# mpkuse/solve_keyframe_pose_graph

Hardware: AMD Instinct MI355X
Metric: LM iters/sec + final chi2 vs Ceres, 100k-pose/300k-edge SE(3) graph (higher is better)
Workload: dtype f64

## Files before the change

### solve_keyframe_pose_graph_amd/csrc/pgo_handle.hpp

```cpp
#pragma once
#include <hip/hip_runtime.h>

#include <chrono>
#include <cstdlib>
#include <cstring>
#include <memory>
#include <string>
#include <thread>
#include <vector>

#include "pgo.h"
#include "pgo_internal.hpp"
#include "pgo_comm.hpp"
#include "pgo_mg_host.hpp"

#pragma GCC visibility push(hidden)
namespace pgo {

inline double now_s() { return std::chrono::duration<double>(std::chrono::steady_clock::now().time_since_epoch()).count(); }

inline bool debug_hooks_enabled() { static const bool on = []() { const char* e = std::getenv("PGO_ENABLE_DEBUG_HOOKS"); return e && e[0] == '1' && e[1] == 0; }(); return on; }
inline bool debug_poison() { static const bool on = []() { const char* e = std::getenv("PGO_DEBUG_POISON"); return debug_hooks_enabled() && e && e[0] == '1' && e[1] == 0; }(); return on; }
inline bool debug_break_coarse() { if (!debug_hooks_enabled()) return false; const char* e = std::getenv("PGO_DEBUG_BREAK_COARSE"); return e && e[0] == '1' && e[1] == 0; }

inline int debug_graph_after() {
    static const int v = []() {
        const char* e = std::getenv("PGO_DEBUG_GRAPH_AFTER");
        if (!debug_hooks_enabled() || !e) return 192;
        char* end = nullptr; const long n = std::strtol(e, &end, 10);
        return (end && *end == 0 && n >= 2 && n <= 1000000 && (n & 1) == 0) ? (int)n : 192;
    }();
    return v;
}

template <class T>
struct DBuf {
    T* p = nullptr;
    size_t cap = 0;
    DBuf() = default;
    DBuf(const DBuf&) = delete;
    DBuf& operator=(const DBuf&) = delete;
    ~DBuf() { if (p) (void)hipFree(p); }
    hipError_t ensure(size_t n) {
        if (n <= cap) return hipSuccess;
        if (p) { (void)hipFree(p); p = nullptr; cap = 0; }
        const size_t want = n + n / 8 + 64;
        hipError_t e = hipMalloc((void**)&p, want * sizeof(T));
        if (e == hipSuccess) cap = want;
        if (e == hipSuccess && debug_poison()) { e = hipMemset(p, 0xFF, want * sizeof(T)); if (e == hipSuccess) e = hipDeviceSynchronize(); }
        return e;
    }
};

struct EventPair {
    hipEvent_t e0 = nullptr, e1 = nullptr;
    hipError_t create() { hipError_t e = hipEventCreate(&e0); if (e == hipSuccess) e = hipEventCreate(&e1); return e; }
    ~EventPair() { if (e0) (void)hipEventDestroy(e0); if (e1) (void)hipEventDestroy(e1); }
};

struct HostClass {
    std::vector<int32_t> c1, c2, sw;
    std::vector<double> meas;
    int64_t size() const { return (int64_t)c1.size(); }
};

struct MgPrepared;
struct MgPreparedFree { void operator()(MgPrepared* Q) const; };
using MgImage = std::unique_ptr<MgPrepared, MgPreparedFree>;

struct LevelPlanDev { const int32_t* send_idx = nullptr; const int32_t* recv_idx = nullptr; const pgo_mg::ExchangePlan* plan = nullptr; };
struct SetupPlanDev { const int32_t* val_send = nullptr; const int32_t* val_dst = nullptr; const int32_t* val_sum_ptr = nullptr; const int32_t* val_sum_src = nullptr;
                      const int32_t* ps_send = nullptr; const int32_t* ps_recv = nullptr; const int32_t* rv_send = nullptr; const int32_t* rv_recv = nullptr; };
struct OwnRange { int64_t row0 = 0, row1 = 0, blk0 = 0, blk1 = 0, ps0 = 0, ps1 = 0, w0 = 0, w1 = 0, rT0 = 0, rT1 = 0; };

struct MgJob {
    enum Kind { none, fresh, regroup };
    Kind kind = none;
    std::thread thread;
    MgImage out;
    int rc = 0;
    MgImage old;
};

struct MgState {
    DBuf<double> f64; DBuf<int32_t> i32; DBuf<int64_t> i64;
    MgDev M{}; MgLevelDev levels[MG_MAX_LEVELS];
    bool fine = false; MgLevelDev fineF{}, fineT{};
    int fine_auto = -1;
    bool built = false, active = false;
    pgo_mg::BuildCache cache;
    std::vector<double> sw_built;
    int regroups = 0;
    uint64_t geometry_epoch = 0;
    MgJob job;
    std::vector<LevelPlanDev> lvl_plan;
    std::vector<pgo_mg::ExchangePlan> plans;
    std::vector<uint8_t> dist;
    pgo_mg::SetupPlans setup; int first_whole = 0;
    int32_t fw_row0 = 0, fw_row1 = 0; int64_t fw_blk0 = 0, fw_blk1 = 0;
    std::vector<SetupPlanDev> su_plan;
    std::vector<OwnRange> own;
    int levels_distributed = 0; int64_t rows_total = 0, rows_own = 0, blocks_total = 0, blocks_own = 0;
    bool fresh_pending() const { return job.kind == MgJob::fresh; }
};

struct CoarseState {
    DBuf<double> d_ccen, d_cd, d_cAc, d_crc, d_cscr;
    DBuf<float> d_cAcf;
    DBuf<int64_t> d_cblk_ptr, d_ccontrib;
    DBuf<int32_t> d_cblk_ab, d_cagg_free, d_cinfo;
    CoarseDev K{};
    bool built = false, active = false;
    int mode = 0;
    int retests = 0; bool skip_all = false; double drop_radius = 0.0;
    int backoff = 0, skip = 0;
    int keep_streak = 0;
    uint64_t geometry_epoch = 0;
};

struct OwnedStream {
    hipStream_t s = nullptr;
    OwnedStream() = default;
    OwnedStream(const OwnedStream&) = delete;
    OwnedStream& operator=(const OwnedStream&) = delete;
    ~OwnedStream() { if (s) (void)hipStreamDestroy(s); }
    operator hipStream_t() const { return s; }
};

struct PcgState {
    struct Poll { int32_t flags[4]; double scal[4]; };
    Poll* poll = nullptr; hipEvent_t poll_ev[2] = {nullptr, nullptr};
    struct CapturedChunk { hipGraphExec_t exec = nullptr; int len = 0; uint64_t epoch = 0; double scale = 0.0; bool sr = false; };
    CapturedChunk cg_chunk[3];
    hipGraphExec_t cg_graph = nullptr;
    uint64_t build_epoch = 1; bool cg_graph_failed = false;
    double cg_predicted = 0.0;
    double cg_prev_equiv = 0.0, cg_prev_radius = 0.0;
    int mg_switch_at = 400;
    int cg_extra = 0;
    bool mg_failed = false;
    bool mg_start_deferred = false;
    PcgState() = default;
    PcgState(const PcgState&) = delete;
    PcgState& operator=(const PcgState&) = delete;
    hipError_t create() {
        hipError_t e = hipHostMalloc((void**)&poll, 3 * sizeof(Poll), hipHostMallocDefault);
        if (e == hipSuccess) e = hipEventCreateWithFlags(&poll_ev[0], hipEventDisableTiming);
        if (e == hipSuccess) e = hipEventCreateWithFlags(&poll_ev[1], hipEventDisableTiming);
        if (e == hipSuccess) std::memset(poll, 0, 3 * sizeof(Poll));
        return e;
    }
    ~PcgState() {
        for (CapturedChunk& cc : cg_chunk) if (cc.exec) (void)hipGraphExecDestroy(cc.exec);
        if (poll) (void)hipHostFree(poll);
        for (hipEvent_t e : poll_ev) if (e) (void)hipEventDestroy(e);
    }
};

}
#pragma GCC visibility pop

using namespace pgo;

struct pgo_problem {
    pgo_options opt;
    int device = 0;
    std::string err;

    HostClass rel, swe;
    std::vector<PriorDev> priors;
    std::vector<int32_t> constant_nodes;
    bool graph_dirty = true, priors_dirty = true;

    int64_t N = 0, S = 0, N_global = 0;
    bool local_ids = false;
    std::vector<int32_t> l2g, g2l;
    std::vector<uint8_t> h_touched_any;
    std::vector<double> h_own;
    std::vector<double> h_init_q, h_init_t;
    std::vector<uint64_t> h_touch_mask;
    std::vector<int32_t> h_owner;
    pgo_mg::FinePlan fine_plan;
    DBuf<int32_t> d_l2g, d_fp_send, d_fp_shloc, d_fp_sumptr, d_fp_sumsrc;
    DBuf<double> d_own, d_xsend[2], d_xrecv, d_xscal;
    int64_t n_sh_mine = 0, n_sh_global = 0;
    int64_t st_exchanges = 0, st_allreduces = 0, st_pcg_iterations = 0; double st_bytes_neighbour = 0.0, st_bytes_allreduce = 0.0;
    DBuf<int32_t> d_rc1, d_rc2, d_sc1, d_sc2, d_sidx, d_bsr_col;
    DBuf<double> d_rmeas, d_smeas;
    DBuf<int4> d_rwin, d_swin;
    DBuf<PriorDev> d_prior;
    DBuf<int64_t> d_inc_rowptr, d_inc, d_bsr_rowptr;
    DBuf<uint8_t> d_node_free;
    DBuf<double> d_Jr, d_Js, d_Jp;
    DBuf<double> d_Hd_g;
    DBuf<double> d_Hoff, d_c, d_hss, d_gs;
    DBuf<double> d_scale_p, d_scale_s, d_diag_p, d_diag_s, d_a_inv;
    DBuf<double> d_val, d_Dtot_b;
    DBuf<float> d_Lf;
    DBuf<double> d_cgvec;
    DBuf<double> d_part;
    DBuf<double> d_cgpart;
    DBuf<int32_t> d_flags;
    DBuf<double> d_scal;
    DBuf<double> d_pose[2], d_swv[2], d_delta_s, d_io;
    DBuf<double> d_tmp;
    DBuf<double> d_vio;
    DBuf<int32_t> d_vio_idx; DBuf<double> d_vio_meas;
    CoarseState coarse;
    uint64_t lin_epoch = 0;
    MgState mg;
    uint64_t hoff_epoch = 0;
    int64_t n_vio = 0;
    DBuf<uint32_t> d_einc;
    DBuf<uint32_t> d_einc_slot;
    DBuf<ushort4> d_node_rng;
    DBuf<int64_t> d_tile_inc0;
    DBuf<int32_t> d_einc_other, d_tile_node0, d_tile_sw0, d_node_prior;
    DBuf<double2> d_rec;
    DBuf<double> d_lam;
    MfDev F{};
    bool built_mf = false;
    int64_t mf_pair_lanes = 0, mf_rel_side_lanes = 0, mf_sw_lanes = 0;
    int cur = 0;
    int64_t n_part = MAX_PARTIALS;
    std::vector<uint8_t> h_node_free, h_sw_used;
    int64_t nnzb = 0;

    GraphDev G{};
    LinDev L{};
    ScaleDev Sc{};
    CgDev C{};

    bool in_solve = false, scale_ready = false, terminated = false, have_prev_step = false;
    double radius = 0, decrease_factor = 2, x_cost = 0, x_norm = 0, gmax = 0;
    bool reuse_diagonal = false;
    int iteration = 0, invalid = 0;
    double t_begin = 0, t_device0 = 0;
    pgo_summary sum;

    std::unique_ptr<pgo_comm::Comm> comm;
    int rank() const { return comm ? comm->rank() : 0; }
    int world() const { return comm ? comm->world() : 1; }

    OwnedStream st;
    PcgState pcg;
    double last_rho = 1.0;
};


#define HIPCHK(p, expr) PGO_HIPCHK((p)->err, expr)

#pragma GCC visibility push(hidden)
namespace pgo {

int allreduce(pgo_problem* p, double* buf, size_t n, int op );
int host_allreduce(pgo_problem* p, std::vector<double>& v, int op);
int exchange_rows(pgo_problem* p, double* a1, int k1, double* a2, int k2, const int32_t* stop = nullptr);
int exchange_level(pgo_problem* p, int l, double* v1, double* v2, const int32_t* stop, const double* dinv);
int exchange_blocks_copy(pgo_problem* p, const pgo_mg::ExchangePlan& X, const int32_t* send_idx, const int32_t* recv_idx, double* arr, int K);
int exchange_blocks_sum(pgo_problem* p, const pgo_mg::BlockPlan& B, const SetupPlanDev& D, double* arr);
int ensure_exchange_buffers(pgo_problem* p);

int build_two_level_aggregates(pgo_problem* p);
void two_level_solve_begin(pgo_problem* p);
void two_level_solve_end(pgo_problem* p);
int build_system(pgo_problem* p, bool* ok);
bool single_reduction(const pgo_problem* p);
struct PcgForm {
    enum Rec { ranks, sr, sr_coarse, classic_mf, classic_csr, classic_coarse };
    enum Post { none, mg_cycle, mg_restricted, two_level };
    Rec rec; Post post;
    int fused_parts;
    bool single_red() const { return rec == sr || rec == sr_coarse; }
    bool fused_coarse() const { return rec == sr_coarse || rec == classic_coarse; }
    bool mg() const { return post == mg_cycle || post == mg_restricted; }
    int precond() const { return mg() ? 2 : (fused_coarse() || post == two_level) ? 1 : 0; }
};
PcgForm choose_form(const pgo_problem* p, bool this_rank_only = false);
void pcg_matvec(pgo_problem* p, const PcgForm& f, int k, double tol2);
int pcg_update(pgo_problem* p, const PcgForm& f, int k);
int pcg_precond(pgo_problem* p, const PcgForm& f, int k);
int pcg_iteration(pgo_problem* p, const PcgForm& f, int k, double tol2);
int pcg_start(pgo_problem* p, const PcgForm& f, bool warm, double tol2);
struct CgResult { int iterations; bool breakdown; double rel_residual; bool converged; };
struct PcgPhase { double tol; int resume = -1; bool warm = false; bool switch_now = false; int max_iterations = 0; };
int run_pcg(pgo_problem* p, CgResult* res, const PcgPhase& ph);
int finish_system(pgo_problem* p, CgResult* cg, bool evaluated, int* precond_used);

bool wants_multigrid(const pgo_problem* p);
void mg_drop_pending(pgo_problem* p);
bool mg_start_fresh(pgo_problem* p, const double* sw_now);
int build_multigrid(pgo_problem* p, const double* sw_now);
int mg_fresh_install(pgo_problem* p);
int regroup_if_moved(pgo_problem* p, const double* sv, bool in_solve);
int regroup_start(pgo_problem* p);
int build_mg(pgo_problem* p);
int mg_operators(pgo_problem* p, int32_t* fail, bool hoff_valid, bool kernels_only, double t_build0);
bool mg_exchange_at(pgo_problem* p, int point, int lv, int* plan, double** v1, double** v2, const double** dinv);
int mg_apply_ranks(pgo_problem* p, bool inside_iteration);
double mg_cs(const pgo_problem* p);
double mg_scale(const pgo_problem* p);
const MgLevelDev* mg_fine_view(const pgo_problem* p);

}
#pragma GCC visibility pop
```

### solve_keyframe_pose_graph_amd/csrc/pgo_internal.hpp

```cpp
#pragma once
#include <hip/hip_runtime.h>
#include <stdint.h>

#include "pgo_device_math.hpp"

#define PGO_HIPCHK(err, expr)                                                                      \
    do {                                                                                           \
        hipError_t e__ = (expr);                                                                   \
        if (e__ != hipSuccess) {                                                                   \
            (err) = std::string(#expr) + ": " + hipGetErrorString(e__);                            \
            return e__ == hipErrorOutOfMemory ? PGO_ERR_OUT_OF_MEMORY : PGO_ERR_HIP;               \
        }                                                                                          \
    } while (0)

namespace pgo {

constexpr int TILE = 64;
constexpr int REL_DOUBLES = 78;
constexpr int SW_DOUBLES = 86;
constexpr int K1_WAVES = 4;
constexpr int WIN_MAX = 72;
constexpr int WIN_STRIDE = 80;
constexpr int MAX_PARTIALS = 1024;
constexpr int CG_MAX_GRID = 1024;
constexpr int RZ_STRIDE = CG_MAX_GRID + MAX_PARTIALS;
constexpr int PQ_SLOTS = CG_MAX_GRID;
constexpr int PRIOR_DOUBLES = 42;
constexpr int MF_BLOCK = 256;
constexpr int MF_MAX_NODES = 42;
constexpr int MF_SLOTS = 384;
constexpr int MF_MAX_GRID = 1024;
constexpr int MF_PLANES = 8;

struct PriorDev {
    double Rf[9];
    double tf[3];
    double qf[4];
    double w;
    int32_t node;
    int32_t pad_;
};

struct EdgeClassDev {
    const int32_t* c1;
    const int32_t* c2;
    const double* meas;
    const int32_t* swidx;
    const int4* win;
    double* J;
    int64_t E, Epad;
    int32_t tiles;
};

struct GraphDev {
    int64_t N, S;
    EdgeClassDev rel, sw;
    const PriorDev* prior; int32_t n_prior; double* Jp;
    const int64_t* inc_rowptr; const int64_t* inc;
    const uint8_t* node_free;
    const double* own;
    const int64_t* bsr_rowptr; const int32_t* bsr_col; int64_t nnzb;
};

struct MfDev {
    const uint32_t* einc;
    const int32_t* einc_other;
    const uint32_t* einc_slot;
    const int64_t* tile_inc0;
    const int32_t* tile_sw0;
    const int32_t* tile_node0;
    const ushort4* node_rng;
    const int32_t* node_prior;
    double2* rec;
    double* lam;
    int64_t ninc, ninc_pad;
    int32_t tiles;
};

struct LinDev {
    double* Hd; double* g; double* Hoff; double* c; double* hss; double* gs;
};

struct ScaleDev {
    double* scale_p;
    double* scale_s;
    double* diag_p;
    double* diag_s;
    double* a_inv;
};

struct CoarseDev {
    int32_t n_agg, nc;
    int32_t m;
    int32_t n_blk;
    double* cen;
    double* d;
    double* Ac;
    double* rc;
    double* yc;
    const int64_t* blk_ptr;
    const int32_t* blk_ab;
    const int64_t* contrib;
    const int32_t* agg_free;
    float* Acf;
};

constexpr int MG_MAX_LEVELS = 12;
constexpr int MG_TILE_ROWS = 32;
struct MgLevelDev {
    int32_t n, n_next, tiles, n_ps;
    int64_t nnzb;
    const int64_t* rowptr; const int32_t* col; double* val;
    const int64_t* g_ptr; const int64_t* g_ent;
    double* Dinv;
    double* pos; double* d;
    const int32_t* parent; const int32_t* agg_ptr; const int4* tile_info; const int2* tile_rows;
    double* r; double* x; double* xt; double* xf;
    float* valf;
    int32_t smoothed, n_w;
    int32_t seg_shift, pad3_;
    const int32_t* ps_rowptr; const int32_t* ps_col; const int32_t* w_rowptr; const int32_t* w_col; const int64_t* psT_ptr; const int64_t* psT_ent;
    double* ps_val; double* w_val;
    double* t; double* u; double* y; const double* zero;
    double* dlump;
    const int32_t* row_of; const int32_t* tr_of;
    const int32_t* ps_row; const int32_t* w_row;
    float* rt_valf; float* r_valf;
    const int2* rt_rows; const int2* rT_rows; const int32_t* rT_col; const int32_t* rT_of_w; const int32_t* ps_of_w;
    int32_t rT_tiles, rT_seg_shift;
    int32_t tile0, tiles_own, rT_row0, rT_row1;
    int32_t su_row0, su_row1, su_ps0, su_ps1, su_w0, su_w1, n_su_prod, pad4_;
    int64_t su_blk0, su_blk1;
    const int32_t* su_prod;
};
struct MgDev {
    int32_t n_levels;
    int32_t n1;
    const int32_t* agg0;
    const int32_t* mem0_ptr; const int32_t* mem0;
    double* d0;
    const int4* blk_tab;
    const double* inv_cnt;
    int32_t a0, a1;
    const int32_t* g0_slots; int32_t n_g0, pad_;
};
constexpr int MG_BLOCK0 = 64;

struct CgDev {
    double* val; float* Lf; double* Dtot; double* b;
    double* x; double* r; double* r2; double* z; double* p; double* p2; double* q;
    double* part_pq;
    double* part_rz;
    int32_t extra_rz;
    int32_t pad_;
    double* scal;
    int32_t* flags;
};

void launch_k1(const GraphDev& G, const double* pose8, const double* sw, bool want_jacobian, double* partials , int* n_partials, hipStream_t st);
void launch_prior(const GraphDev& G, const double* pose8, bool want_jacobian, double* partial_cost , hipStream_t st);
void launch_k2(const GraphDev& G, const LinDev& L, bool want_offdiag, hipStream_t st, const MfDev* F = nullptr );
void launch_scale_init(const GraphDev& G, const LinDev& L, const ScaleDev& Sc, int jacobi_scaling, hipStream_t st);
void launch_lm_diag(const GraphDev& G, const LinDev& L, const ScaleDev& Sc, double min_diag, double max_diag, hipStream_t st);
void launch_build_rows(const GraphDev& G, const LinDev& L, const ScaleDev& Sc, const CgDev& C, double radius, int add_lambda, double* lam_out , hipStream_t st);
void launch_mf_compact(const GraphDev& G, const MfDev& F, const double* pose8, const double* sw, hipStream_t st);
void launch_mf_spmv(const GraphDev& G, const MfDev& F, const ScaleDev& Sc, const CgDev& C, int k, double tol2, hipStream_t st);
void launch_mf_apply(const GraphDev& G, const MfDev& F, const ScaleDev& Sc, const CgDev& C, const double* x, double* y, hipStream_t st);
void launch_mf_apply_dot(const GraphDev& G, const MfDev& F, const ScaleDev& Sc, const CgDev& C, const double* x, double* y, hipStream_t st);
void launch_invert_rows(const GraphDev& G, const CgDev& C, int32_t* fail_flag, hipStream_t st);
void launch_cg_init(const GraphDev& G, const CgDev& C, int warm , double tol2, hipStream_t st);
int launch_cg_init_vectors(const GraphDev& G, const CgDev& C, int warm, hipStream_t st);
void launch_cg_init_scalars(const CgDev& C, int nparts, int nparts_bb, double tol2, hipStream_t st);
void launch_cg_set_tolerance(const CgDev& C, double tol2, hipStream_t st);
void launch_cg_poll(const CgDev& C, int32_t* host_flags, double* host_scal, hipStream_t st);
void launch_cg_spmv(const GraphDev& G, const CgDev& C, int k, double tol2, hipStream_t st);
void launch_cg_update(const GraphDev& G, const CgDev& C, int k, int n_pq_partials, hipStream_t st);
void launch_mf_apply_dot_live(const GraphDev& G, const MfDev& F, const ScaleDev& Sc, const CgDev& C, hipStream_t st);
void launch_cg_update_sr(const GraphDev& G, const CgDev& C, int k, int first, int n_pq_partials, hipStream_t st);
void launch_mf_apply_dot_live_coarse(const GraphDev& G, const MfDev& F, const ScaleDev& Sc, const CgDev& C, const CoarseDev& K, int pending, hipStream_t st);
void launch_cg_update_restrict_sr(const GraphDev& G, const CgDev& C, const CoarseDev& K, int k, int first, int pending, int n_pq_partials, hipStream_t st);
int cg_grid_size(const GraphDev& G);
int mf_grid_size(const MfDev& F);
void launch_apply_operator(const GraphDev& G, const CgDev& C, const double* x, double* y, hipStream_t st);
void launch_model_change(const GraphDev& G, const LinDev& L, const ScaleDev& Sc, const double* delta_p, double* delta_s, double* partials, int* n_partials, hipStream_t st);
void launch_plus(const GraphDev& G, const double* pose8, const double* sw, const double* delta_p, const double* delta_s,
                 double* pose8_out, double* sw_out, double* part_step2, double* part_sw_step2, int* n_partials, hipStream_t st);
void launch_state_norms(const GraphDev& G, const LinDev& L, const double* pose8, const double* sw,
                        double* part_xnorm2, double* part_sw_xnorm2, double* part_gmax, int* n_partials, hipStream_t st);
void launch_reduce(const double* partials, int n, int op , double* out, hipStream_t st);
void launch_manifold_plus(int64_t n, const double* quat, const double* t, const double* delta, double* quat_out, double* t_out, hipStream_t st);
void launch_pack_pose(const double* quat, const double* t, double* pose8, int64_t N, hipStream_t st);
void launch_unpack_pose(const double* pose8, double* quat, double* t, int64_t N, hipStream_t st);
void launch_unpack_k1(const GraphDev& G, int kind, int64_t first, int64_t count, double* r, double* J1, double* J2, double* Js, hipStream_t st);
void launch_gather_rows(double* buf, const double* a1, int k1, const double* a2, int k2, int64_t n, const int32_t* idx, const int32_t* stop, hipStream_t st);
void launch_scatter_rows(const double* buf, double* a1, int k1, double* a2, int k2, int64_t n, const int32_t* idx, const int32_t* stop, hipStream_t st);
void launch_scatter_rows_dinv(const double* buf, double* r, double* x, const double* Dinv, int64_t n, const int32_t* idx, const int32_t* stop, hipStream_t st);
void launch_sum_rows(const double* buf, double* a1, int k1, double* a2, int k2, int64_t n_sh, const int32_t* sh_loc, const int32_t* sum_ptr, const int32_t* sum_src, const int32_t* stop, hipStream_t st);
struct LocalPeers { const double* src[16]; int64_t off[16]; int64_t cnt[16]; int n; };
void launch_local_reduce(double* out, const LocalPeers& P, int64_t n, int op, hipStream_t st);
void launch_local_copy(double* recv, const LocalPeers& P, hipStream_t st);
void launch_coarse_geometry(const GraphDev& G, const CoarseDev& K, const double* pose8, hipStream_t st);
void launch_coarse_assemble(const GraphDev& G, const LinDev& L, const ScaleDev& Sc, const CgDev& C, const CoarseDev& K, hipStream_t st);
void launch_coarse_symmetrize(const CoarseDev& K, hipStream_t st);
void launch_coarse_shift(const CoarseDev& K, double eps, hipStream_t st);
void launch_coarse_invert(const CoarseDev& K, double* scratch , int32_t* fail, hipStream_t st);
void launch_coarse_negate(const CoarseDev& K, hipStream_t st);
void launch_coarse_apply(const GraphDev& G, const CgDev& C, const CoarseDev& K, const double* r, double* z, double* part_rz, bool inside_iteration, hipStream_t st);
int coarse_group_keyframes(const CoarseDev& K);
int coarse_update_grid(const GraphDev& G, const CoarseDev& K);
int coarse_solve_grid(const CoarseDev& K);
void launch_mf_spmv_coarse(const GraphDev& G, const MfDev& F, const ScaleDev& Sc, const CgDev& C, const CoarseDev& K, int k, double tol2, int nparts, int pending, hipStream_t st);
void launch_cg_update_restrict(const GraphDev& G, const CgDev& C, const CoarseDev& K, int k, int n_pq_partials, hipStream_t st);
void launch_coarse_solve_dot(const CoarseDev& K, const int32_t* stop, double* part, hipStream_t st);
void launch_cgcg_dots(const GraphDev& G, const CgDev& C, hipStream_t st);
void launch_cg_reduce2_live(const CgDev& C, const double* pa, int na, const double* pb, int nb, double* out, hipStream_t st);
void launch_cgcg_update(const GraphDev& G, const CgDev& C, int k, int first, hipStream_t st, const double* xq = nullptr, const int32_t* sh_of = nullptr, const double* two = nullptr);
void launch_cgcg_scalars_init(const CgDev& C, const double* bb_src, double tol2, hipStream_t st);
void launch_scatter_owned_pose(const double* quat, const double* t, int64_t n, const int32_t* l2g, const double* own, double* gquat, double* gt, hipStream_t st);
void launch_vio_odometry(int64_t n, const int32_t* c1, const int32_t* c2, const double* vio, int yaw_weight, double* meas8, hipStream_t st);
void launch_vio_initial_guess(int64_t u_begin, int64_t count, const double* left, const int32_t* left_of_node, const double* vio, double* quat, double* t, hipStream_t st);

void launch_mg_geometry(const GraphDev& G, const MgDev& M, const MgLevelDev* levels, const double* pose8, hipStream_t st);
void launch_mg_geometry0_sum(const GraphDev& G, const MgDev& M, const MgLevelDev* levels, const double* pose8, hipStream_t st);
void launch_mg_geometry_finish(const GraphDev& G, const MgDev& M, const MgLevelDev* levels, const double* pose8, hipStream_t st);
void launch_mg_assemble(const GraphDev& G, const LinDev& L, const ScaleDev& Sc, const CgDev& C, const MgDev& M, const MgLevelDev* levels, const CoarseDev& K, double omega, int32_t* fail, hipStream_t st, double prolong_scale = 0.0, bool hoff_valid = false);
void launch_mg_galerkin0(const GraphDev& G, const LinDev& L, const ScaleDev& Sc, const CgDev& C, const MgDev& M, const MgLevelDev* levels, hipStream_t st, bool hoff_valid = false);
void launch_k2_offdiag(const GraphDev& G, const LinDev& L, hipStream_t st);
void launch_mg_assemble_fine(const GraphDev& G, const LinDev& L, const ScaleDev& Sc, const CgDev& C, const MgLevelDev& F, const MgLevelDev& T, const MgLevelDev& L1, double omega, int32_t* fail, hipStream_t st,
                             double prolong_scale, bool hoff_valid, const double* pose8 = nullptr );
void launch_mg_assemble_rest(const MgDev& M, const MgLevelDev* levels, const CoarseDev& K, double omega, int32_t* fail, hipStream_t st, double prolong_scale = 0.0 ,
                             int first_level = 0 );
void launch_mg_level_inverses(const MgLevelDev& A, double omega, int32_t* fail, hipStream_t st);
void launch_mg_level_power(const MgLevelDev& A, double omega, hipStream_t st);
void launch_mg_power_init(const MgLevelDev& A, hipStream_t st);
void launch_mg_power_step(const MgLevelDev& A, const double* v, double* w, double omega, hipStream_t st);
void launch_mg_power_sums(const MgLevelDev& A, const double* a, const double* b, const int32_t* fail, double* out3, hipStream_t st);
void launch_mg_power_finish(const double* in3, int32_t* fail, double* lam, hipStream_t st);
void launch_mg_level_rescale(const MgLevelDev& A, const double* lam, double omega, hipStream_t st);
void launch_mg_transition_ps(const MgLevelDev& A, double prolong_scale, hipStream_t st);
void launch_mg_transition_w(const MgLevelDev& A, hipStream_t st);
void launch_mg_transition_product(const MgLevelDev& A, const MgLevelDev& B, hipStream_t st);
void launch_mg_level_galerkin(const MgLevelDev& A, const MgLevelDev& B, hipStream_t st);
void launch_mg_dense_top(const MgDev& M, const MgLevelDev* levels, const CoarseDev& K, hipStream_t st);
struct MgExchangeHook { void* ctx; int (*fn)(void* ctx, int point, int level); };
void launch_mg_apply(const GraphDev& G, const CgDev& C, const MgDev& M, const MgLevelDev* levels, const CoarseDev& K, const double* r, double* z, double* part_rz, double scale, bool inside_iteration, hipStream_t st,
                     bool restricted = false , double prolong_scale = 0.0 ,
                     const MgLevelDev* fine = nullptr ,
                     const MgExchangeHook* hook = nullptr , int* hook_rc = nullptr);
void launch_cg_update_mg(const GraphDev& G, const CgDev& C, const MgDev& M, const MgLevelDev* levels, const CoarseDev& K, int k, int n_pq_partials, hipStream_t st);
void launch_cg_update_mg_sr(const GraphDev& G, const CgDev& C, const MgDev& M, const MgLevelDev* levels, const CoarseDev& K, int k, int first, int n_pq_partials, hipStream_t st);

double k1_algorithmic_bytes(const GraphDev& G, bool want_jacobian);

}
```

### solve_keyframe_pose_graph_amd/csrc/pgo_mg_kernels.hpp

```cpp

__device__ __forceinline__ int bsr_idx(int row, int col) { return (row >> 1) * 12 + col * 2 + (row & 1); }

__device__ __forceinline__ void mg_row_accumulate(int64_t b, int64_t e, const int32_t* __restrict__ col, const double* __restrict__ val,
                                                  const double* __restrict__ x, int c, double* acc) {
    int64_t k = b;
    for (; k + 4 <= e; k += 4) spmv_chunk<4, false>(col + k, val + (size_t)k * 36, c, x, nullptr, 0.0, acc);
    if (k + 2 <= e) { spmv_chunk<2, false>(col + k, val + (size_t)k * 36, c, x, nullptr, 0.0, acc); k += 2; }
    if (k < e) spmv_chunk<1, false>(col + k, val + (size_t)k * 36, c, x, nullptr, 0.0, acc);
}

template <int U>
__device__ __forceinline__ void mg_chunk_f32(const int32_t* __restrict__ colp, const float* __restrict__ valp, int c, const double* __restrict__ x, double* acc) {
    int32_t col[U];
    float2 v[U][3];
    double xx[U];
#pragma unroll
    for (int u = 0; u < U; ++u) col[u] = colp[u];
#pragma unroll
    for (int u = 0; u < U; ++u) {
        const float2* vp = reinterpret_cast<const float2*>(valp + (size_t)u * 36) + c;
        v[u][0] = vp[0]; v[u][1] = vp[6]; v[u][2] = vp[12];
    }
#pragma unroll
    for (int u = 0; u < U; ++u) xx[u] = x[(size_t)col[u] * 6 + c];
// ... 186 lines not shown
#pragma unroll
            for (int u = 0; u < CH; ++u) if (u < n) acc += coarse_entry(Hs[wv][u], ds[wv][u], ds[wv][u] + 3, r, c);
        }
        __builtin_amdgcn_wave_barrier();
    }
    if (own) A.val[(size_t)slot * 36 + bsr_idx(r, c)] = acc;
}
__global__ __launch_bounds__(256) void mg_galerkin_kernel(MgLevelDev A, MgLevelDev B) {
    constexpr int CH = 8;
    __shared__ double Hs[4][CH][36];
    __shared__ double ds[4][CH][6];
    const int wv = wave_in_block(), lane = threadIdx.x & 63;
    const int64_t slot = wave_in_grid() + B.su_blk0;
    if (slot >= B.su_blk1) return;
    const int r = lane / 6, c = lane - r * 6;
    const bool own = lane < 36;
    const int srow = 2 * (lane / 12) + (lane & 1), scol = (lane % 12) >> 1;
    const int du = lane / 6, dm = lane - du * 6;
    double acc = 0.0;
    const int64_t kend = B.g_ptr[slot + 1];
    for (int64_t k0 = B.g_ptr[slot]; k0 < kend; k0 += CH) {
        const int n = (int)(kend - k0 < CH ? kend - k0 : CH);
        if (du < n) {
            const int64_t e = B.g_ent[k0 + du];
            const int64_t node = dm < 3 ? (e >> 32) : (int64_t)A.col[e & 0xffffffffll];
            ds[wv][du][dm] = A.d[(size_t)node * 3 + (dm < 3 ? dm : dm - 3)];
        }
        double h[CH];
#pragma unroll
        for (int u = 0; u < CH; ++u) {
            const int64_t fs = B.g_ent[k0 + u < kend ? k0 + u : kend - 1] & 0xffffffffll;
            h[u] = own ? A.val[(size_t)fs * 36 + lane] : 0.0;
        }
        if (own) {
#pragma unroll
            for (int u = 0; u < CH; ++u) Hs[wv][u][srow * 6 + scol] = h[u];
        }
        __builtin_amdgcn_wave_barrier();
        if (own) {
#pragma unroll
            for (int u = 0; u < CH; ++u) if (u < n) acc += coarse_entry(Hs[wv][u], ds[wv][u], ds[wv][u] + 3, r, c);
        }
        __builtin_amdgcn_wave_barrier();
    }
    if (own) B.val[(size_t)slot * 36 + bsr_idx(r, c)] = acc;
}
__global__ __launch_bounds__(256) void mg_dinv_kernel(MgLevelDev A, double omega, int32_t* __restrict__ fail, int skip_orphans ,
                                                      const double* __restrict__ diag = nullptr) {
    const int i = blockIdx.x * blockDim.x + threadIdx.x + A.su_row0;
    if (i >= A.su_row1) return;
    if (skip_orphans && A.parent[i] < 0) { double* out = A.Dinv + (size_t)i * 36; for (int e = 0; e < 36; ++e) out[e] = 0.0; return; }
    const double* v = diag ? diag + (size_t)i * 36 : A.val + (size_t)A.rowptr[i] * 36;
    double Lm[36];
    bool ok = true;
    for (int attempt = 0; attempt < 2; ++attempt) {
    ok = true;
#pragma unroll
    for (int j = 0; j < 6; ++j) {
        double d = v[bsr_idx(j, j)];
#pragma unroll
        for (int k = 0; k < 6; ++k) if (k < j) d -= Lm[j * 6 + k] * Lm[j * 6 + k];
        ok = ok && (d > 0.0);
        d = sqrt(d);
        Lm[j * 6 + j] = 1.0 / d;
#pragma unroll
        for (int r = 0; r < 6; ++r) if (r > j) {
            double s = v[bsr_idx(r, j)];
#pragma unroll
            for (int k = 0; k < 6; ++k) if (k < j) s -= Lm[r * 6 + k] * Lm[j * 6 + k];
            Lm[r * 6 + j] = s * Lm[j * 6 + j];
        }
    }
    if (ok || !diag || attempt == 1) break;
    v = A.val + (size_t)A.rowptr[i] * 36;
    }
    if (!ok) atomicOr(fail, 1);
    double* out = A.Dinv + (size_t)i * 36;
#pragma unroll
    for (int e = 0; e < 6; ++e) {
        double y[6], z[6];
#pragma unroll
        for (int r = 0; r < 6; ++r) {
            double s = r == e ? 1.0 : 0.0;
#pragma unroll
            for (int k = 0; k < 6; ++k) if (k < r) s -= Lm[r * 6 + k] * y[k];
            y[r] = s * Lm[r * 6 + r];
        }
#pragma unroll
        for (int r = 5; r >= 0; --r) {
            double s = y[r];
#pragma unroll
            for (int k = 0; k < 6; ++k) if (k > r) s -= Lm[k * 6 + r] * z[k];
            z[r] = s * Lm[r * 6 + r];
        }
#pragma unroll
        for (int r = 0; r < 6; ++r) out[r * 6 + e] = omega * z[r];
    }
}
__global__ __launch_bounds__(256) void mg_dense_scatter_kernel(MgLevelDev A, CoarseDev K) {
    const int64_t t = (int64_t)blockIdx.x * blockDim.x + threadIdx.x;
    if (t >= (int64_t)A.n * 36) return;
    const int i = (int)(t / 36), l = (int)(t - (int64_t)i * 36);
    const int row = 2 * (l / 12) + (l & 1), col = (l % 12) >> 1;
    for (int64_t k = A.rowptr[i]; k < A.rowptr[i + 1]; ++k)
        K.Ac[(size_t)(i * 6 + row) * K.nc + (size_t)A.col[k] * 6 + col] = A.val[(size_t)k * 36 + l];
}
__device__ __forceinline__ double mg_pblock(const double* __restrict__ d, int r, int c) {
    if (r < 3 || c >= 3) return r == c ? 1.0 : 0.0;
    const int a = r - 3;
    if (a == c) return 0.0;
    const int o = 3 - a - c;
    const double sgn = ((a + 1) % 3 == c) ? 1.0 : -1.0;
    return sgn * 2.0 * d[o];
}
template <bool FILT>
__global__ __launch_bounds__(256) void mg_ps_kernel(MgLevelDev A, double cs) {
    __shared__ double acc_s[4][36];
    const int wv = wave_in_block(), lane = threadIdx.x & 63;
    const int64_t slot = wave_in_grid() + A.su_ps0;
    if (slot >= A.su_ps1) return;
    const bool own = lane < 36;
    const int r = own ? lane / 6 : 0, c = own ? lane % 6 : 0;
    const int i = A.ps_row[slot], a = A.ps_col[slot];
    double acc = 0.0;
    for (int64_t k = A.rowptr[i]; k < A.rowptr[i + 1]; ++k) {
        const int j = A.col[k];
        if (A.parent[j] != a) continue;
        if (FILT && (A.g_ent[k] & 7) >= 3) continue;
        if (own) {
            const double* dj = A.d + (size_t)j * 3;
            const double* blk = (FILT && k == A.rowptr[i]) ? A.dlump + (size_t)i * 36 : A.val + (size_t)k * 36;
#pragma unroll
            for (int m = 0; m < 6; ++m) acc += blk[bsr_idx(r, m)] * mg_pblock(dj, m, c);
        }
    }
    if (own) acc_s[wv][lane] = acc;
    __builtin_amdgcn_wave_barrier();
    if (own) {
        double v = A.parent[i] == a ? mg_pblock(A.d + (size_t)i * 3, r, c) : 0.0;
        const double* Dk = A.Dinv + (size_t)i * 36 + r * 6;
#pragma unroll
        for (int m = 0; m < 6; ++m) v -= cs * Dk[m] * acc_s[wv][m * 6 + c];
        A.ps_val[(size_t)slot * 36 + lane] = v;
    }
}
constexpr int MG_SETUP_CHUNK = 8;
__global__ __launch_bounds__(256) void mg_w_kernel(MgLevelDev A) {
    __shared__ double pb[4][MG_SETUP_CHUNK][36], ab[4][MG_SETUP_CHUNK][36];
    const int wv = wave_in_block(), lane = threadIdx.x & 63;
    const int64_t slot = wave_in_grid() + A.su_w0;
    if (slot >= A.su_w1) return;
    const bool own = lane < 36;
    const int r = own ? lane / 6 : 0, c = own ? lane % 6 : 0;
    const int i = A.w_row[slot], b = A.w_col[slot];
    double acc = 0.0;
    const int64_t kend = A.rowptr[i + 1];
    for (int64_t k0 = A.rowptr[i]; k0 < kend; k0 += MG_SETUP_CHUNK) {
        const int n = (int)(kend - k0 < MG_SETUP_CHUNK ? kend - k0 : MG_SETUP_CHUNK);
        int j[MG_SETUP_CHUNK], p0[MG_SETUP_CHUNK], p1[MG_SETUP_CHUNK], ps[MG_SETUP_CHUNK];
#pragma unroll
        for (int u = 0; u < MG_SETUP_CHUNK; ++u) j[u] = u < n ? A.col[k0 + u] : 0;
#pragma unroll
        for (int u = 0; u < MG_SETUP_CHUNK; ++u) { p0[u] = u < n ? A.ps_rowptr[j[u]] : 0; p1[u] = u < n ? A.ps_rowptr[j[u] + 1] : 0; }
        int cand[MG_SETUP_CHUNK];
#pragma unroll
        for (int u = 0; u < MG_SETUP_CHUNK; ++u) cand[u] = (p0[u] + lane < p1[u]) ? A.ps_col[p0[u] + lane] : -1;
#pragma unroll
        for (int u = 0; u < MG_SETUP_CHUNK; ++u) {
            unsigned long long hit = __ballot(cand[u] == b);
            ps[u] = hit ? p0[u] + __ffsll((long long)hit) - 1 : -1;
            for (int base = p0[u] + 64; ps[u] < 0 && base < p1[u]; base += 64) {
                hit = __ballot(base + lane < p1[u] && A.ps_col[base + lane] == b);
                if (hit) ps[u] = base + __ffsll((long long)hit) - 1;
            }
        }
#pragma unroll
        for (int u = 0; u < MG_SETUP_CHUNK; ++u) if (ps[u] >= 0 && own) pb[wv][u][lane] = A.ps_val[(size_t)ps[u] * 36 + lane];
#pragma unroll
        for (int u = 0; u < MG_SETUP_CHUNK; ++u) if (ps[u] >= 0 && own) ab[wv][u][lane] = A.val[(size_t)(k0 + u) * 36 + lane];
        __builtin_amdgcn_wave_barrier();
#pragma unroll
        for (int u = 0; u < MG_SETUP_CHUNK; ++u) {
            if (ps[u] >= 0 && own) {
#pragma unroll
                for (int m = 0; m < 6; ++m) acc += ab[wv][u][bsr_idx(r, m)] * pb[wv][u][m * 6 + c];
            }
        }
        __builtin_amdgcn_wave_barrier();
    }
    if (own) A.w_val[(size_t)slot * 36 + lane] = acc;
}
__global__ __launch_bounds__(256) void mg_rt_kernel(MgLevelDev A) {
    const int lane = threadIdx.x & 63;
    const int64_t k = wave_in_grid() + A.su_w0;
    if (k >= A.su_w1 || lane >= 36) return;
    const int r = lane / 6, c = lane % 6;
    const int i = A.w_row[k];
    const int32_t ps = A.ps_of_w[k];
    const int32_t tr = A.rT_of_w[k];
    double v = ps >= 0 ? A.ps_val[(size_t)ps * 36 + lane] : 0.0;
    const double* Dk = A.Dinv + (size_t)i * 36 + r * 6;
    const double* W = A.w_val + (size_t)k * 36;
#pragma unroll
    for (int m = 0; m < 6; ++m) v -= Dk[m] * W[m * 6 + c];
    const float f = (float)v;
    A.rt_valf[(size_t)k * 36 + bsr_idx(r, c)] = f;
    A.r_valf[(size_t)tr * 36 + bsr_idx(c, r)] = f;
}
__global__ __launch_bounds__(256) void mg_psTw_kernel(MgLevelDev A, MgLevelDev B) {
    __shared__ double pa[4][MG_SETUP_CHUNK][36], wb[4][MG_SETUP_CHUNK][36];
    const int wv = wave_in_block(), lane = threadIdx.x & 63;
    int64_t slot = wave_in_grid();
    if (slot >= (A.su_prod ? (int64_t)A.n_su_prod : B.nnzb)) return;
    if (A.su_prod) slot = A.su_prod[slot];
    const bool own = lane < 36;
    const int r = own ? lane / 6 : 0, c = own ? lane % 6 : 0;
    const int a = B.row_of[slot], b = B.col[slot];
    double acc = 0.0;
    const int64_t eend = A.psT_ptr[a + 1];
    for (int64_t e0 = A.psT_ptr[a]; e0 < eend; e0 += MG_SETUP_CHUNK) {
        const int n = (int)(eend - e0 < MG_SETUP_CHUNK ? eend - e0 : MG_SETUP_CHUNK);
        int64_t ent[MG_SETUP_CHUNK];
        int w0[MG_SETUP_CHUNK], w1[MG_SETUP_CHUNK], ws[MG_SETUP_CHUNK], cand[MG_SETUP_CHUNK];
#pragma unroll
        for (int u = 0; u < MG_SETUP_CHUNK; ++u) ent[u] = u < n ? A.psT_ent[e0 + u] : 0;
#pragma unroll
        for (int u = 0; u < MG_SETUP_CHUNK; ++u) { const int i = (int)(ent[u] >> 32); const bool in = u < n && i >= A.su_row0 && i < A.su_row1; w0[u] = in ? A.w_rowptr[i] : 0; w1[u] = in ? A.w_rowptr[i + 1] : 0; }
#pragma unroll
        for (int u = 0; u < MG_SETUP_CHUNK; ++u) cand[u] = (w0[u] + lane < w1[u]) ? A.w_col[w0[u] + lane] : -1;
#pragma unroll
        for (int u = 0; u < MG_SETUP_CHUNK; ++u) {
            unsigned long long hit = __ballot(cand[u] == b);
            ws[u] = hit ? w0[u] + __ffsll((long long)hit) - 1 : -1;
            for (int base = w0[u] + 64; ws[u] < 0 && base < w1[u]; base += 64) {
                hit = __ballot(base + lane < w1[u] && A.w_col[base + lane] == b);
                if (hit) ws[u] = base + __ffsll((long long)hit) - 1;
            }
        }
#pragma unroll
        for (int u = 0; u < MG_SETUP_CHUNK; ++u)
            if (ws[u] >= 0 && own) { pa[wv][u][lane] = A.ps_val[(size_t)(ent[u] & 0xffffffffll) * 36 + lane]; wb[wv][u][lane] = A.w_val[(size_t)ws[u] * 36 + lane]; }
        __builtin_amdgcn_wave_barrier();
#pragma unroll
        for (int u = 0; u < MG_SETUP_CHUNK; ++u) {
            if (ws[u] >= 0 && own) {
#pragma unroll
                for (int m = 0; m < 6; ++m) acc += pa[wv][u][m * 6 + r] * wb[wv][u][m * 6 + c];
            }
        }
        __builtin_amdgcn_wave_barrier();
    }
    if (own) B.val[(size_t)slot * 36 + bsr_idx(r, c)] = acc;
}
__device__ __forceinline__ void mg_smooth_step_tile(const MgLevelDev& A, int tile, const double* __restrict__ in_r, const double* __restrict__ in_x, double* __restrict__ out_w,
                                                    const double* __restrict__ add1, const double* __restrict__ add2, double* __restrict__ out, double cs, const int32_t* __restrict__ stop,
                                                    double* xch , double* tb ) {
    const int stopped = stop ? *stop : 0;
    const int q6 = threadIdx.x / 6, c = threadIdx.x % 6;
    const int li = q6 & ((MG_TILE_ROWS >> A.seg_shift) - 1), sg = q6 >> (5 - A.seg_shift);
    const int4 ti = A.tile_info[tile];
    const int2 rb = A.tile_rows[tile * MG_TILE_ROWS + li];
    if (stopped) return;
    const int i0 = ti.z, i1 = ti.w;
    const int row = i0 + li;
    const bool rowlive = row < i1;
    const bool live = rowlive && sg == 0;
    double rv = 0.0, av = 0.0;
    double Dk[6] = {0.0, 0.0, 0.0, 0.0, 0.0, 0.0};
    if (live) {
        if (in_r) rv = in_r[(size_t)row * 6 + c];
        if (add1) av += add1[(size_t)row * 6 + c];
        if (add2) av += add2[(size_t)row * 6 + c];
        const double2* Dp = reinterpret_cast<const double2*>(A.Dinv + (size_t)row * 36 + c * 6);
        const double2 u0 = Dp[0], u1 = Dp[1], u2 = Dp[2];
        Dk[0] = u0.x; Dk[1] = u0.y; Dk[2] = u1.x; Dk[3] = u1.y; Dk[4] = u2.x; Dk[5] = u2.y;
    }
    double acc[6] = {0.0, 0.0, 0.0, 0.0, 0.0, 0.0};
    MG_ROW_PRODUCT(tile, in_x);
    double* mine = xch + (size_t)threadIdx.x * 7;
#pragma unroll
    for (int q = 0; q < 6; ++q) mine[q] = acc[q];
    __syncthreads();
    double w = 0.0;
    if (live) {
        w = rv - mg_gather_row(xch, li, c, A.seg_shift);
        tb[threadIdx.x] = w;
        if (out_w) out_w[(size_t)row * 6 + c] = w;
    }
    __syncthreads();
    if (live) {
        const double* ta = tb + (threadIdx.x - c);
        double x = 0.0;
#pragma unroll
        for (int j = 0; j < 6; ++j) x += Dk[j] * ta[j];
        out[(size_t)row * 6 + c] = av + cs * x;
    }
}
__global__ __launch_bounds__(CG_BLOCK) void mg_smooth_step_kernel(MgLevelDev A, const double* __restrict__ in_r, const double* __restrict__ in_x, double* __restrict__ out_w,
                                                                   const double* __restrict__ add1, const double* __restrict__ add2, double* __restrict__ out, double cs, const int32_t* __restrict__ stop) {
    __shared__ double xch[CG_BLOCK * 7];
    __shared__ double tb[CG_BLOCK];
    mg_smooth_step_tile(A, (int)blockIdx.x + A.tile0, in_r, in_x, out_w, add1, add2, out, cs, stop, xch, tb);
}
__global__ __launch_bounds__(CG_BLOCK) void mg_sdown_kernel(MgLevelDev A, double* __restrict__ r_next, double* __restrict__ x_next, const double* __restrict__ Dinv_next, const int32_t* __restrict__ stop) {
    __shared__ double xch[CG_BLOCK * 7];
    __shared__ double tb[CG_BLOCK];
    if ((int)blockIdx.x < A.tiles_own) { mg_smooth_step_tile(A, (int)blockIdx.x + A.tile0, A.r, A.x, nullptr, A.x, nullptr, A.y, 1.0, stop, xch, tb); return; }
    const int stopped = stop ? *stop : 0;
    const int tile = (int)blockIdx.x - A.tiles_own;
    const int ss = A.rT_seg_shift, rpt = MG_TILE_ROWS >> ss;
    const int q6 = threadIdx.x / 6, c = threadIdx.x % 6;
    const int li = q6 & (rpt - 1), sg = q6 >> (5 - ss);
    const int2 rb = A.rT_rows[tile * MG_TILE_ROWS + li];
    const int row = A.rT_row0 + tile * rpt + li;
    const bool live = row < A.rT_row1 && sg == 0;
    double Dk[6] = {0.0, 0.0, 0.0, 0.0, 0.0, 0.0};
    if (live && x_next) {
        const double2* Dp = reinterpret_cast<const double2*>(Dinv_next + (size_t)row * 36 + c * 6);
        const double2 u0 = Dp[0], u1 = Dp[1], u2 = Dp[2];
        Dk[0] = u0.x; Dk[1] = u0.y; Dk[2] = u1.x; Dk[3] = u1.y; Dk[4] = u2.x; Dk[5] = u2.y;
    }
    if (stopped) return;
    double acc[6] = {0.0, 0.0, 0.0, 0.0, 0.0, 0.0};
    if (row < A.rT_row1) { int kb, ke; mg_split_row(rb, sg, ss, kb, ke); mg_row_accumulate_f32(kb, ke, A.rT_col, A.r_valf, A.r, c, acc); }
    double* mine = xch + (size_t)threadIdx.x * 7;
#pragma unroll
    for (int q = 0; q < 6; ++q) mine[q] = acc[q];
    __syncthreads();
    double sum = 0.0;
    if (live) { sum = mg_gather_row(xch, li, c, ss); r_next[(size_t)row * 6 + c] = sum; }
    if (!x_next) return;
    tb[threadIdx.x] = sum;
    __syncthreads();
    if (live) {
        const double* ra = tb + (threadIdx.x - c);
        double x = 0.0;
#pragma unroll
        for (int j = 0; j < 6; ++j) x += Dk[j] * ra[j];
        x_next[(size_t)row * 6 + c] = x;
    }
}

template <bool HOFF>
__global__ __launch_bounds__(256) void mg_fine_blocks_kernel(GraphDev G, LinDev L, ScaleDev Sc, CgDev C, MgLevelDev F) {
    const int lane = threadIdx.x & 63;
    const int64_t k = wave_in_grid();
    if (k >= F.nnzb) return;
    const int r = lane / 6, c = lane - r * 6;
    const bool own = lane < 36;
    const double h = fine_block_value<HOFF>(G, L, Sc, C, F.g_ent[k], lane, r, c, own);
    if (own) F.val[(size_t)k * 36 + bsr_idx(r, c)] = h;
}
__global__ __launch_bounds__(256) void mg_fine_lump_kernel(MgLevelDev F, const double* __restrict__ pose8) {
    __shared__ double cs_[4][36];
    const int wv = wave_in_block(), lane = threadIdx.x & 63;
    const int64_t i = wave_in_grid();
    if (i >= F.n) return;
    const bool own = lane < 36;
    const int r = own ? lane / 6 : 0, c = own ? lane % 6 : 0;
    const int64_t k0 = F.rowptr[i], k1 = F.rowptr[i + 1];
    double acc = 0.0;
    if (F.parent[i] >= 0) {
        const double* ti = pose8 + (size_t)i * 8 + 4;
        for (int64_t k = k0 + 1; k < k1; ++k) {
            if ((F.g_ent[k] & 7) < 3) continue;
            const int j = F.col[k];
            if (F.parent[j] < 0 || j == (int)i) continue;
            if (own) {
                const double* tj = pose8 + (size_t)j * 8 + 4;
                const double d[3] = {tj[0] - ti[0], tj[1] - ti[1], tj[2] - ti[2]};
#pragma unroll
                for (int m = 0; m < 6; ++m) acc += F.val[(size_t)k * 36 + bsr_idx(r, m)] * mg_pblock(d, m, c);
            }
        }
    }
    if (own) cs_[wv][lane] = acc;
    __builtin_amdgcn_wave_barrier();
    if (own) F.dlump[(size_t)i * 36 + bsr_idx(r, c)] = F.val[(size_t)k0 * 36 + bsr_idx(r, c)] + 0.5 * (cs_[wv][r * 6 + c] + cs_[wv][c * 6 + r]);
}
__global__ __launch_bounds__(256) void mg_ps_f32_kernel(MgLevelDev T) {
    const int lane = threadIdx.x & 63;
    const int64_t k = wave_in_grid();
    if (k >= T.n_ps || lane >= 36) return;
    const int r = lane / 6, c = lane % 6;
    const float f = (float)T.ps_val[(size_t)k * 36 + lane];
    T.rt_valf[(size_t)k * 36 + bsr_idx(r, c)] = f;
    T.r_valf[(size_t)T.rT_of_w[k] * 36 + bsr_idx(c, r)] = f;
}
__global__ __launch_bounds__(CG_BLOCK) void mg_prolong0s_kernel(GraphDev G, MgLevelDev T, const double* __restrict__ x1, const double* __restrict__ rv, double* __restrict__ zv,
                                                                 double* __restrict__ part_rz, double scale, const int32_t* __restrict__ stop) {
    __shared__ double red[CG_BLOCK / 64];
    if (stop && *stop) return;
    const int64_t pairs = G.N * 3;
    double acc = 0.0;
    for (int64_t i = (int64_t)blockIdx.x * CG_BLOCK + threadIdx.x; i < pairs; i += (int64_t)gridDim.x * CG_BLOCK) {
        const int64_t n = i / 3;
        const int j = (int)(i - n * 3);
        const int k0 = T.ps_rowptr[n], k1 = T.ps_rowptr[n + 1];
        if (k1 <= k0) continue;
        double a0 = 0.0, a1 = 0.0;
        for (int k = k0; k < k1; ++k) {
            const float4* vp = reinterpret_cast<const float4*>(T.rt_valf + (size_t)k * 36 + j * 12);
            const float4 v0 = vp[0], v1 = vp[1], v2 = vp[2];
            const double2* xp = reinterpret_cast<const double2*>(x1 + (size_t)T.ps_col[k] * 6);
            const double2 xa = xp[0], xb = xp[1], xc = xp[2];
            a0 += (double)v0.x * xa.x + (double)v0.z * xa.y + (double)v1.x * xb.x + (double)v1.z * xb.y + (double)v2.x * xc.x + (double)v2.z * xc.y;
            a1 += (double)v0.y * xa.x + (double)v0.w * xa.y + (double)v1.y * xb.x + (double)v1.w * xb.y + (double)v2.y * xc.x + (double)v2.w * xc.y;
        }
        a0 *= scale; a1 *= scale;
        double2* zp = reinterpret_cast<double2*>(zv) + i;
        const double2 r = reinterpret_cast<const double2*>(rv)[i];
        double2 z = *zp;
        z.x += a0; z.y += a1;
        *zp = z;
        acc += r.x * a0 + r.y * a1;
    }
    const double s = block_sum(acc, red);
    if (threadIdx.x == 0) part_rz[blockIdx.x] += s;
}

__global__ void mg_power_init_kernel(double* __restrict__ v, double* __restrict__ w, int n6, int lo6, int hi6) {
    const int i = blockIdx.x * blockDim.x + threadIdx.x;
    if (i >= n6) return;
    v[i] = (i >= lo6 && i < hi6) ? 1.0 + 0.5 * sin(0.7 * (double)i) : 0.0;
    w[i] = 0.0;
}
__global__ __launch_bounds__(1024) void mg_power_ratio_kernel(const double* __restrict__ a, const double* __restrict__ b, int lo6, int hi6, double* __restrict__ lam) {
    __shared__ double red[32];
    double sa = 0.0, sb = 0.0;
    for (int i = lo6 + threadIdx.x; i < hi6; i += blockDim.x) { sa += a[i] * a[i]; sb += b[i] * b[i]; }
    sa = wave_sum(sa); sb = wave_sum(sb);
    if ((threadIdx.x & 63) == 0) { red[threadIdx.x >> 6] = sa; red[16 + (threadIdx.x >> 6)] = sb; }
    __syncthreads();
    if (threadIdx.x == 0) {
        double ta = 0.0, tb = 0.0;
        for (int k = 0; k < 16; ++k) { ta += red[k]; tb += red[16 + k]; }
        *lam = ta > 0.0 ? sqrt(tb / ta) : 0.0;
    }
}
__global__ __launch_bounds__(256) void mg_rescale_dinv_kernel(MgLevelDev A, const double* __restrict__ lam, double omega, double limit, double target) {
    const double wl = omega * lam[0];
    if (!(wl > limit)) return;
    const double f = target / wl;
    const int64_t i = (int64_t)blockIdx.x * blockDim.x + threadIdx.x + (int64_t)A.su_row0 * 36;
    if (i < (int64_t)A.su_row1 * 36) A.Dinv[i] *= f;
}
void launch_mg_level_power(const MgLevelDev& A, double omega, hipStream_t st) {
    const int n6 = A.n * 6;
    double* v = A.x; double* w = A.xt; double* lam = A.xf;
    MgLevelDev S = A;
    const bool part = A.su_row0 != 0 || A.su_row1 != A.n;
    if (!part) { S.tile0 = 0; S.tiles_own = A.tiles; }
    hipLaunchKernelGGL(mg_power_init_kernel, dim3((unsigned)((n6 + 255) / 256)), dim3(256), 0, st, v, w, n6, A.su_row0 * 6, A.su_row1 * 6);
    for (int it = 0; it < 8; ++it) {
        if (S.tiles_own > 0) hipLaunchKernelGGL(mg_smooth_step_kernel, dim3((unsigned)S.tiles_own), dim3(CG_BLOCK), 0, st, S, (const double*)nullptr, (const double*)v, (double*)nullptr, (const double*)nullptr, (const double*)nullptr, w, -1.0 / omega, (const int32_t*)nullptr);
        double* tmp = v; v = w; w = tmp;
    }
    hipLaunchKernelGGL(mg_power_ratio_kernel, dim3(1), dim3(1024), 0, st, (const double*)w, (const double*)v, A.su_row0 * 6, A.su_row1 * 6, lam);
}
void launch_mg_level_rescale(const MgLevelDev& A, const double* lam, double omega, hipStream_t st) {
    const int64_t cnt = (int64_t)(A.su_row1 - A.su_row0) * 36;
    if (cnt > 0) hipLaunchKernelGGL(mg_rescale_dinv_kernel, dim3((unsigned)((cnt + 255) / 256)), dim3(256), 0, st, A, lam, omega, 1.75, 1.5);
}
void launch_mg_level_inverses(const MgLevelDev& A, double omega, int32_t* fail, hipStream_t st) {
    const int rows = A.su_row1 - A.su_row0;
    const int64_t blocks = A.su_blk1 - A.su_blk0;
    if (rows > 0) hipLaunchKernelGGL(mg_dinv_kernel, dim3((unsigned)((rows + 255) / 256)), dim3(256), 0, st, A, omega, fail, 0, (const double*)nullptr);
    if (blocks > 0) hipLaunchKernelGGL(mg_val_f32_kernel, dim3((unsigned)((blocks + 3) / 4)), dim3(256), 0, st, A);
}
void launch_mg_transition_ps(const MgLevelDev& A, double prolong_scale, hipStream_t st) {
    const int cnt = A.su_ps1 - A.su_ps0;
    if (cnt > 0) hipLaunchKernelGGL(mg_ps_kernel<false>, dim3((unsigned)((cnt + 3) / 4)), dim3(256), 0, st, A, prolong_scale);
}
void launch_mg_transition_w(const MgLevelDev& A, hipStream_t st) {
    const int cnt = A.su_w1 - A.su_w0;
    if (cnt <= 0) return;
    hipLaunchKernelGGL(mg_w_kernel, dim3((unsigned)((cnt + 3) / 4)), dim3(256), 0, st, A);
    if (A.rt_valf) hipLaunchKernelGGL(mg_rt_kernel, dim3((unsigned)((cnt + 3) / 4)), dim3(256), 0, st, A);
}
void launch_mg_transition_product(const MgLevelDev& A, const MgLevelDev& B, hipStream_t st) {
    const int64_t cnt = A.su_prod ? (int64_t)A.n_su_prod : B.nnzb;
    if (cnt > 0) hipLaunchKernelGGL(mg_psTw_kernel, dim3((unsigned)((cnt + 3) / 4)), dim3(256), 0, st, A, B);
}
void launch_mg_level_galerkin(const MgLevelDev& A, const MgLevelDev& B, hipStream_t st) {
    const int64_t cnt = B.su_blk1 - B.su_blk0;
    if (cnt > 0) hipLaunchKernelGGL(mg_galerkin_kernel, dim3((unsigned)((cnt + 3) / 4)), dim3(256), 0, st, A, B);
}
void launch_mg_power_init(const MgLevelDev& A, hipStream_t st) {
    const int n6 = A.n * 6;
    hipLaunchKernelGGL(mg_power_init_kernel, dim3((unsigned)((n6 + 255) / 256)), dim3(256), 0, st, A.x, A.xt, n6, A.su_row0 * 6, A.su_row1 * 6);
}
void launch_mg_power_step(const MgLevelDev& A, const double* v, double* w, double omega, hipStream_t st) {
    if (A.tiles_own > 0) hipLaunchKernelGGL(mg_smooth_step_kernel, dim3((unsigned)A.tiles_own), dim3(CG_BLOCK), 0, st, A, (const double*)nullptr, v, (double*)nullptr, (const double*)nullptr, (const double*)nullptr, w, -1.0 / omega, (const int32_t*)nullptr);
}
__global__ __launch_bounds__(1024) void mg_power_sums_kernel(const double* __restrict__ a, const double* __restrict__ b, int lo6, int hi6, const int32_t* __restrict__ fail, double* __restrict__ out3) {
    __shared__ double red[32];
    double sa = 0.0, sb = 0.0;
    for (int i = lo6 + threadIdx.x; i < hi6; i += blockDim.x) { sa += a[i] * a[i]; sb += b[i] * b[i]; }
    sa = wave_sum(sa); sb = wave_sum(sb);
    if ((threadIdx.x & 63) == 0) { red[threadIdx.x >> 6] = sa; red[16 + (threadIdx.x >> 6)] = sb; }
    __syncthreads();
    if (threadIdx.x == 0) {
        double ta = 0.0, tb = 0.0;
        for (int k = 0; k < 16; ++k) { ta += red[k]; tb += red[16 + k]; }
        out3[0] = ta; out3[1] = tb; out3[2] = *fail != 0 ? 1.0 : 0.0;
    }
}
__global__ void mg_power_finish_kernel(const double* __restrict__ in3, int32_t* __restrict__ fail, double* __restrict__ lam) { if (in3[2] != 0.0) *fail = 1; *lam = in3[0] > 0.0 ? sqrt(in3[1] / in3[0]) : 0.0; }
void launch_mg_power_sums(const MgLevelDev& A, const double* a, const double* b, const int32_t* fail, double* out3, hipStream_t st) {
    hipLaunchKernelGGL(mg_power_sums_kernel, dim3(1), dim3(1024), 0, st, a, b, A.su_row0 * 6, A.su_row1 * 6, fail, out3);
}
void launch_mg_power_finish(const double* in3, int32_t* fail, double* lam, hipStream_t st) { hipLaunchKernelGGL(mg_power_finish_kernel, dim3(1), dim3(1), 0, st, in3, fail, lam); }

void launch_mg_galerkin0(const GraphDev& G, const LinDev& L, const ScaleDev& Sc, const CgDev& C, const MgDev& M, const MgLevelDev* levels, hipStream_t st, bool hoff_valid) {
    const int64_t cnt = M.g0_slots ? (int64_t)M.n_g0 : levels[0].nnzb;
    if (cnt <= 0) return;
    if (hoff_valid) hipLaunchKernelGGL((mg_galerkin0_kernel<true>), dim3((unsigned)((cnt + 3) / 4)), dim3(256), 0, st, G, L, Sc, C, M, levels[0]);
    else hipLaunchKernelGGL((mg_galerkin0_kernel<false>), dim3((unsigned)((cnt + 3) / 4)), dim3(256), 0, st, G, L, Sc, C, M, levels[0]);
}
void launch_mg_assemble(const GraphDev& G, const LinDev& L, const ScaleDev& Sc, const CgDev& C, const MgDev& M, const MgLevelDev* levels, const CoarseDev& K, double omega, int32_t* fail, hipStream_t st, double prolong_scale, bool hoff_valid) {
    launch_mg_galerkin0(G, L, Sc, C, M, levels, st, hoff_valid);
    launch_mg_assemble_rest(M, levels, K, omega, fail, st, prolong_scale);
}
void launch_mg_dense_top(const MgDev& M, const MgLevelDev* levels, const CoarseDev& K, hipStream_t st) {
    const MgLevelDev& T = levels[M.n_levels - 1];
    (void)hipMemsetAsync(K.Ac, 0, (size_t)K.nc * K.nc * sizeof(double), st);
    if (K.nc > 6 * K.n_agg) hipLaunchKernelGGL(coarse_pad_identity_kernel, dim3((unsigned)((K.nc - 6 * K.n_agg + 63) / 64)), dim3(64), 0, st, K);
    hipLaunchKernelGGL(mg_dense_scatter_kernel, dim3((unsigned)(((int64_t)T.n * 36 + 255) / 256)), dim3(256), 0, st, T, K);
}
void launch_mg_assemble_rest(const MgDev& M, const MgLevelDev* levels, const CoarseDev& K, double omega, int32_t* fail, hipStream_t st, double prolong_scale, int first_level) {
    for (int l = first_level; l < M.n_levels; ++l) {
        if (l > first_level) {
            const MgLevelDev& A = levels[l - 1];
            if (A.smoothed) { launch_mg_transition_ps(A, prolong_scale, st); launch_mg_transition_w(A, st); launch_mg_transition_product(A, levels[l], st); }
            else launch_mg_level_galerkin(A, levels[l], st);
        }
        if (l + 1 < M.n_levels) {
            launch_mg_level_inverses(levels[l], omega, fail, st);
            launch_mg_level_power(levels[l], omega, st);
            launch_mg_level_rescale(levels[l], levels[l].xf, omega, st);
        }
    }
    launch_mg_dense_top(M, levels, K, st);
}
void launch_mg_assemble_fine(const GraphDev& G, const LinDev& L, const ScaleDev& Sc, const CgDev& C, const MgLevelDev& F, const MgLevelDev& T, const MgLevelDev& L1, double omega, int32_t* fail, hipStream_t st,
                             double prolong_scale, bool hoff_valid, const double* pose8) {
    if (hoff_valid) hipLaunchKernelGGL((mg_fine_blocks_kernel<true>), dim3((unsigned)((F.nnzb + 3) / 4)), dim3(256), 0, st, G, L, Sc, C, F);
    else hipLaunchKernelGGL((mg_fine_blocks_kernel<false>), dim3((unsigned)((F.nnzb + 3) / 4)), dim3(256), 0, st, G, L, Sc, C, F);
    if (F.dlump && pose8) {
        hipLaunchKernelGGL(mg_fine_lump_kernel, dim3((unsigned)((F.n + 3) / 4)), dim3(256), 0, st, F, pose8);
        hipLaunchKernelGGL(mg_dinv_kernel, dim3((unsigned)((F.n + 255) / 256)), dim3(256), 0, st, F, omega, fail, 1, (const double*)F.dlump);
        hipLaunchKernelGGL(mg_ps_kernel<true>, dim3((unsigned)((F.n_ps + 3) / 4)), dim3(256), 0, st, F, prolong_scale);
    } else {
        hipLaunchKernelGGL(mg_dinv_kernel, dim3((unsigned)((F.n + 255) / 256)), dim3(256), 0, st, F, omega, fail, 1, (const double*)nullptr);
        hipLaunchKernelGGL(mg_ps_kernel<false>, dim3((unsigned)((F.n_ps + 3) / 4)), dim3(256), 0, st, F, prolong_scale);
    }
    hipLaunchKernelGGL(mg_w_kernel, dim3((unsigned)((F.n_w + 3) / 4)), dim3(256), 0, st, F);
    hipLaunchKernelGGL(mg_psTw_kernel, dim3((unsigned)((L1.nnzb + 3) / 4)), dim3(256), 0, st, F, L1);
    hipLaunchKernelGGL(mg_ps_f32_kernel, dim3((unsigned)((T.n_ps + 3) / 4)), dim3(256), 0, st, T);
}

__global__ __launch_bounds__(CG_BLOCK) void mg_restrict0_kernel(MgDev M, const double* __restrict__ rv, double* __restrict__ r_out, double* __restrict__ x_out,
                                                                 const double* __restrict__ Dinv, const int32_t* __restrict__ stop, const double* __restrict__ own = nullptr ) {
    __shared__ double rb[CG_BLOCK];
    const int stopped = stop ? *stop : 0;
    const int a = M.a0 + blockIdx.x * MG_TILE_ROWS + threadIdx.x / 6, k = threadIdx.x % 6;
    const bool live = a < M.a1;
    int m0 = 0, m1 = 0;
    if (live) { m0 = M.mem0_ptr[a]; m1 = M.mem0_ptr[a + 1]; }
    if (stopped) return;
    double s = 0.0;
    if (live) {
        if (own) for (int m = m0; m < m1; ++m) { const int i = M.mem0[m]; s += own[i] * mg_restrict_comp(rv + (size_t)i * 6, M.d0 + (size_t)i * 3, k); }
        else for (int m = m0; m < m1; ++m) { const int i = M.mem0[m]; s += mg_restrict_comp(rv + (size_t)i * 6, M.d0 + (size_t)i * 3, k); }
        r_out[(size_t)a * 6 + k] = s;
    }
    if (!x_out) return;
    rb[threadIdx.x] = s;
    __syncthreads();
    if (live) {
        const double* Dk = Dinv + (size_t)a * 36 + k * 6;
        const double* ra = rb + (threadIdx.x - k);
        double x = 0.0;
#pragma unroll
        for (int j = 0; j < 6; ++j) x += Dk[j] * ra[j];
        x_out[(size_t)a * 6 + k] = x;
    }
}
#ifdef PGO_MG_TIMELINE
__device__ unsigned long long pgo_mg_tl[4 * 1024 * 8];
#define MG_TL(slot) do { __builtin_amdgcn_s_waitcnt(0); if (threadIdx.x == 0 && A.pad3_ < 4 && blockIdx.x < 1024) pgo_mg_tl[((size_t)A.pad3_ * 1024 + blockIdx.x) * 8 + (slot)] = wall_clock64(); } while (0)
extern "C" int pgo_debug_mg_timeline(unsigned long long* out, int n) {
    return (int)hipMemcpyFromSymbol(out, HIP_SYMBOL(pgo_mg_tl), (size_t)n * sizeof(unsigned long long), 0, hipMemcpyDeviceToHost);
}
#else
#define MG_TL(slot) do {} while (0)
#endif
__global__ __launch_bounds__(CG_BLOCK) void mg_down_kernel(MgLevelDev A, double* __restrict__ r_next, double* __restrict__ x_next, const double* __restrict__ Dinv_next,
                                                            const int32_t* __restrict__ stop) {
    __shared__ double xch[CG_BLOCK * 7];
    __shared__ double tb[CG_BLOCK];
    __shared__ double cb[CG_BLOCK];
    MG_TL(0);
    const int stopped = stop ? *stop : 0;
    const int q6 = threadIdx.x / 6, c = threadIdx.x % 6;
    const int li = q6 & ((MG_TILE_ROWS >> A.seg_shift) - 1), sg = q6 >> (5 - A.seg_shift);
    const int tile_d = (int)blockIdx.x + A.tile0;
    const int4 ti = A.tile_info[tile_d];
    const int2 rb = A.tile_rows[tile_d * MG_TILE_ROWS + li];
    MG_TL(1);
    if (stopped) return;
    const int a0 = ti.x, na = ti.y - ti.x, i0 = ti.z, i1 = ti.w;
    const int row = i0 + li;
    const bool rowlive = row < i1;
    const bool live = rowlive && sg == 0;
    const bool lagg = threadIdx.x < na * 6;
    const int a = a0 + li;
    double rv = 0.0, d0 = 0.0, d1 = 0.0, d2 = 0.0;
    int m0 = 0, m1 = 0;
    double Dk[6] = {0.0, 0.0, 0.0, 0.0, 0.0, 0.0};
    if (live) { rv = A.r[(size_t)row * 6 + c]; d0 = A.d[(size_t)row * 3]; d1 = A.d[(size_t)row * 3 + 1]; d2 = A.d[(size_t)row * 3 + 2]; }
    if (lagg) {
        m0 = A.agg_ptr[a]; m1 = A.agg_ptr[a + 1];
        if (x_next) {
            const double2* Dp = reinterpret_cast<const double2*>(Dinv_next + (size_t)a * 36 + c * 6);
            const double2 u0 = Dp[0], u1 = Dp[1], u2 = Dp[2];
            Dk[0] = u0.x; Dk[1] = u0.y; Dk[2] = u1.x; Dk[3] = u1.y; Dk[4] = u2.x; Dk[5] = u2.y;
        }
    }
    MG_TL(2);
    double acc[6] = {0.0, 0.0, 0.0, 0.0, 0.0, 0.0};
    MG_ROW_PRODUCT(blockIdx.x, A.x);
    MG_TL(3);
    double* mine = xch + (size_t)threadIdx.x * 7;
#pragma unroll
    for (int q = 0; q < 6; ++q) mine[q] = acc[q];
    __syncthreads();
    if (live) tb[threadIdx.x] = rv - mg_gather_row(xch, li, c, A.seg_shift);
    __syncthreads();
    MG_TL(4);
    if (live) {
        const double d[3] = {d0, d1, d2};
        cb[threadIdx.x] = mg_restrict_comp(tb + (size_t)li * 6, d, c);
    }
    __syncthreads();
    double s = 0.0;
    if (lagg) {
        for (int m = m0; m < m1; ++m) s += cb[(m - i0) * 6 + c];
        r_next[(size_t)a * 6 + c] = s;
    }
    MG_TL(5);
    if (!x_next) return;
    tb[threadIdx.x] = s;
    __syncthreads();
    if (lagg) {
        const double* ra = tb + (threadIdx.x - c);
        double x = 0.0;
#pragma unroll
        for (int j = 0; j < 6; ++j) x += Dk[j] * ra[j];
        x_next[(size_t)a * 6 + c] = x;
    }
    MG_TL(6);
}
__global__ __launch_bounds__(384) void mg_dense_solve_kernel(CoarseDev K, MgLevelDev Below, int has_below, double scale, const int32_t* __restrict__ stop) {
    __shared__ double ys[6];
    const int stopped = stop ? *stop : 0;
    const int a = blockIdx.x;
    const int q = threadIdx.x >> 6, lane = threadIdx.x & 63;
    const double2* __restrict__ x = reinterpret_cast<const double2*>(K.rc);
    const float4* __restrict__ Ar = reinterpret_cast<const float4*>(K.Acf + (size_t)(a * 6 + q) * K.nc);
    const int n4 = K.nc >> 2;
    double s = 0.0;
    if (lane < n4) { const float4 u = Ar[lane]; const double2 v = x[2 * lane], w = x[2 * lane + 1]; s = (double)u.x * v.x + (double)u.y * v.y + (double)u.z * w.x + (double)u.w * w.y; }
    if (stopped) return;
#pragma unroll 4
    for (int j = lane + 64; j < n4; j += 64) { const float4 u = Ar[j]; const double2 v = x[2 * j], w = x[2 * j + 1]; s += (double)u.x * v.x + (double)u.y * v.y + (double)u.z * w.x + (double)u.w * w.y; }
    s = wave_sum(s);
    if (lane == 0) { ys[q] = s; K.yc[a * 6 + q] = s; }
    if (!has_below) return;
    __syncthreads();
    double y[6];
#pragma unroll
    for (int k = 0; k < 6; ++k) y[k] = ys[k];
    const int c0 = Below.agg_ptr[a], c1 = Below.agg_ptr[a + 1];
    for (int idx = threadIdx.x; idx < (c1 - c0) * 6; idx += 384) {
        const int i = c0 + idx / 6, k = idx % 6;
        Below.xt[(size_t)i * 6 + k] = Below.x[(size_t)i * 6 + k] + scale * mg_prolong_comp(y, Below.d + (size_t)i * 3, k);
    }
}
template <bool FINE>
__global__ __launch_bounds__(CG_BLOCK) void mg_up_kernel(MgLevelDev A, MgLevelDev Below, int has_below, double scale, const int32_t* __restrict__ stop,
                                                          MgDev M, const double* __restrict__ rfine, double* __restrict__ zfine, double* __restrict__ part_extra,
                                                          const double* __restrict__ xnext = nullptr) {
    __shared__ double xch[CG_BLOCK * 7];
    __shared__ double tb[CG_BLOCK];
    __shared__ double xb[CG_BLOCK];
    const int stopped = stop ? *stop : 0;
    const int q6 = threadIdx.x / 6, c = threadIdx.x % 6;
    const int li = q6 & ((MG_TILE_ROWS >> A.seg_shift) - 1), sg = q6 >> (5 - A.seg_shift);
    double acc2 = 0.0;
    for (int tile = A.tile0 + (int)blockIdx.x; tile < A.tile0 + A.tiles_own; tile += gridDim.x) {
    const int4 ti = A.tile_info[tile];
    const bool expl = xnext != nullptr;
    const int2 rb = expl ? A.rt_rows[tile * MG_TILE_ROWS + li] : A.tile_rows[tile * MG_TILE_ROWS + li];
    if (stopped) return;
    const int i0 = ti.z, i1 = ti.w;
    const int row = i0 + li;
    const bool rowlive = row < i1;
    const bool live = rowlive && sg == 0;
    double rv = 0.0, xv = 0.0;
    double Dk[6] = {0.0, 0.0, 0.0, 0.0, 0.0, 0.0};
    int c0 = 0, c1 = 0;
    if (live) {
        rv = A.r[(size_t)row * 6 + c]; xv = expl ? A.y[(size_t)row * 6 + c] : A.xt[(size_t)row * 6 + c];
        if (!expl) {
            const double2* Dp = reinterpret_cast<const double2*>(A.Dinv + (size_t)row * 36 + c * 6);
            const double2 u0 = Dp[0], u1 = Dp[1], u2 = Dp[2];
            Dk[0] = u0.x; Dk[1] = u0.y; Dk[2] = u1.x; Dk[3] = u1.y; Dk[4] = u2.x; Dk[5] = u2.y;
        }
    }
    if (has_below) { c0 = Below.agg_ptr[i0]; c1 = Below.agg_ptr[i1]; }
    const int idx0 = threadIdx.x;
    int ch = 0, chk = 0, chp = 0; double chx = 0.0, chd[3] = {0.0, 0.0, 0.0};
    const bool first = has_below && idx0 < (c1 - c0) * 6;
    if (first) {
        ch = c0 + idx0 / 6; chk = idx0 % 6;
        chp = Below.parent[ch]; chx = Below.x[(size_t)ch * 6 + chk];
        chd[0] = Below.d[(size_t)ch * 3]; chd[1] = Below.d[(size_t)ch * 3 + 1]; chd[2] = Below.d[(size_t)ch * 3 + 2];
    }
    constexpr int FT = FINE ? (MG_TILE_ROWS * 8 * 3 + CG_BLOCK - 1) / CG_BLOCK : 1;
    int fn[FT], fa[FT]; double fd[FT][3]; double2 fz[FT];
    int fcnt = 0;
    if (FINE) {
        const int e0 = M.mem0_ptr[i0];
        fcnt = (M.mem0_ptr[i1] - e0) * 3;
#pragma unroll
        for (int tt = 0; tt < FT; ++tt) {
            const int idx = threadIdx.x + tt * CG_BLOCK;
            fn[tt] = -1;
            if (idx < fcnt) {
                const int n = M.mem0[e0 + idx / 3], j = idx % 3;
                fn[tt] = n * 3 + j; fa[tt] = M.agg0[n] - i0;
                fd[tt][0] = M.d0[(size_t)n * 3]; fd[tt][1] = M.d0[(size_t)n * 3 + 1]; fd[tt][2] = M.d0[(size_t)n * 3 + 2];
                fz[tt] = reinterpret_cast<const double2*>(zfine)[(size_t)n * 3 + j];
            }
        }
    }
    double acc[6] = {0.0, 0.0, 0.0, 0.0, 0.0, 0.0};
    if (expl) { if (rowlive) { int kb, ke; mg_split_row(rb, sg, A.seg_shift, kb, ke); mg_row_accumulate_f32(kb, ke, A.w_col, A.rt_valf, xnext, c, acc); } }
    else MG_ROW_PRODUCT(tile, A.xt);
    double* mine = xch + (size_t)threadIdx.x * 7;
#pragma unroll
    for (int q = 0; q < 6; ++q) mine[q] = acc[q];
    __syncthreads();
    if (expl) {
        if (live) {
            const double x = xv + scale * mg_gather_row(xch, li, c, A.seg_shift);
            A.xf[(size_t)row * 6 + c] = x;
            xb[threadIdx.x] = x;
        }
    } else {
        if (live) tb[threadIdx.x] = rv - mg_gather_row(xch, li, c, A.seg_shift);
        __syncthreads();
        if (live) {
            const double* ta = tb + (threadIdx.x - c);
            double x = xv;
#pragma unroll
            for (int j = 0; j < 6; ++j) x += Dk[j] * ta[j];
            A.xf[(size_t)row * 6 + c] = x;
            xb[threadIdx.x] = x;
        }
    }
    if (FINE) {
        __syncthreads();
        if (live) acc2 += scale * rv * xb[threadIdx.x];
#pragma unroll
        for (int tt = 0; tt < FT; ++tt) {
            if (fn[tt] < 0) continue;
            const int j = fn[tt] % 3;
            const double* y = xb + (size_t)fa[tt] * 6;
            const double b0 = scale * mg_prolong_comp(y, fd[tt], 2 * j), b1 = scale * mg_prolong_comp(y, fd[tt], 2 * j + 1);
            reinterpret_cast<double2*>(zfine)[fn[tt]] = make_double2(fz[tt].x + b0, fz[tt].y + b1);
        }
        __syncthreads();
        continue;
    }
    if (!has_below) return;
    __syncthreads();
    if (first) Below.xt[(size_t)ch * 6 + chk] = chx + scale * mg_prolong_comp(xb + (size_t)(chp - i0) * 6, chd, chk);
    for (int idx = threadIdx.x + CG_BLOCK; idx < (c1 - c0) * 6; idx += CG_BLOCK) {
        const int i = c0 + idx / 6, k = idx % 6;
        const double* y = xb + (size_t)(Below.parent[i] - i0) * 6;
        Below.xt[(size_t)i * 6 + k] = Below.x[(size_t)i * 6 + k] + scale * mg_prolong_comp(y, Below.d + (size_t)i * 3, k);
    }
    }
    if (FINE) {
        __shared__ double red[CG_BLOCK / 64];
        const double s2 = block_sum(acc2, red);
        if (threadIdx.x == 0) part_extra[blockIdx.x] = s2;
    }
}
__global__ __launch_bounds__(CG_BLOCK) void mg_prolong0_kernel(GraphDev G, MgDev M, const double* __restrict__ y1, const double* __restrict__ rv, double* __restrict__ zv,
                                                                double* __restrict__ part_rz, double scale, const int32_t* __restrict__ stop) {
    __shared__ double red[CG_BLOCK / 64];
    if (stop && *stop) return;
    const int64_t pairs = G.N * 3;
    double acc = 0.0;
    for (int64_t i = (int64_t)blockIdx.x * CG_BLOCK + threadIdx.x; i < pairs; i += (int64_t)gridDim.x * CG_BLOCK) {
        const int64_t n = i / 3;
        const int j = (int)(i - n * 3);
        const int a = M.agg0[n];
        if (a < 0) continue;
        const double* y = y1 + (size_t)a * 6;
        const double* d = M.d0 + (size_t)n * 3;
        const double a0 = scale * mg_prolong_comp(y, d, 2 * j), a1 = scale * mg_prolong_comp(y, d, 2 * j + 1);
        double2* zp = reinterpret_cast<double2*>(zv) + i;
        const double2 r = reinterpret_cast<const double2*>(rv)[i];
        double2 z = *zp;
        z.x += a0; z.y += a1;
        *zp = z;
        const double w = G.own ? G.own[n] : 1.0;
        acc += w * (r.x * a0 + r.y * a1);
    }
    const double s = block_sum(acc, red);
    if (threadIdx.x == 0) part_rz[blockIdx.x] += s;
}

#ifdef PGO_SR_MG_NO_BOUNDS
#define PGO_SR_MG_WAVES 1
#else
#define PGO_SR_MG_WAVES 3
#endif
template <bool SR>
__global__ __launch_bounds__(CG_BLOCK, SR ? PGO_SR_MG_WAVES : 1) void cg_update_mg_kernel(GraphDev G, CgDev C, MgDev M, double* __restrict__ r1_out, double* __restrict__ x1_out, const double* __restrict__ Dinv1,
                                                                 int parity, int nparts_pq, int nparts, int first) {
    static_assert(CG_BLOCK / 3 == MG_BLOCK0, "one workgroup trip of the vector update = one run of the slot table");
    __shared__ double red[2 * (CG_BLOCK / 64) + 1];
    const double2* __restrict__ rin = reinterpret_cast<const double2*>(SR ? C.r : (parity ? C.r2 : C.r));
    double2* __restrict__ rout = reinterpret_cast<double2*>(SR ? C.r : (parity ? C.r : C.r2));
    const double2* __restrict__ pcur = reinterpret_cast<const double2*>(SR ? C.p : (parity ? C.p2 : C.p));
    const double2* __restrict__ qv = reinterpret_cast<const double2*>(C.q);
    double2* __restrict__ xv = reinterpret_cast<double2*>(C.x);
    double2* __restrict__ zv = reinterpret_cast<double2*>(C.z);
    double2* __restrict__ pout = reinterpret_cast<double2*>(C.p);
    double2* __restrict__ sv = reinterpret_cast<double2*>(C.p2);
    double2 u0 = make_double2(0.0, 0.0), s0 = u0;
    constexpr int KF = CG_BLOCK / 3;
    const int t = threadIdx.x;
    const int64_t pairs = G.N * 3;
    const int64_t stride = (int64_t)gridDim.x * CG_BLOCK;
    const int64_t trips = (pairs + stride - 1) / stride;
    const int c6 = t % 6;
    double2 r0, q0, p0, x0; double d0, d1, d2; float4 lf0, lf1; int4 tab0, tab1; double Dk0[6], Dk1[6];
    auto load_trip = [&](int64_t run) {
        const int64_t base = run * CG_BLOCK, i = base + t;
        r0 = make_double2(0.0, 0.0); q0 = r0; p0 = r0; x0 = r0; d0 = d1 = d2 = 0.0;
        if (SR) { u0 = r0; s0 = r0; }
        lf0 = make_float4(0.f, 0.f, 0.f, 0.f); lf1 = lf0; tab0 = make_int4(-1, -1, -1, 0); tab1 = tab0;
        if (base < pairs) {
            tab0 = M.blk_tab[(size_t)run * MG_BLOCK0 + t / 6];
            tab1 = M.blk_tab[(size_t)run * MG_BLOCK0 + (t + CG_BLOCK) / 6];
        }
        if (i < pairs) {
            r0 = rin[i]; q0 = qv[i]; p0 = pcur[i]; x0 = xv[i];
            if (SR) { u0 = zv[i]; s0 = sv[i]; }
            const double* d = M.d0 + (size_t)(i / 3) * 3; d0 = d[0]; d1 = d[1]; d2 = d[2];
        }
        const int64_t first_node = base / 3;
        const float4* lp = reinterpret_cast<const float4*>(C.Lf + (size_t)first_node * LF_STRIDE);
        if (first_node + t / 6 < G.N) lf0 = lp[t];
        if (first_node + (t + CG_BLOCK) / 6 < G.N) lf1 = lp[t + CG_BLOCK];
#pragma unroll
        for (int jj = 0; jj < 6; ++jj) { Dk0[jj] = 0.0; Dk1[jj] = 0.0; }
        if (x1_out) {
            if (tab0.x >= 0) { const double2* Dp = reinterpret_cast<const double2*>(Dinv1 + (size_t)tab0.x * 36 + c6 * 6); const double2 u0 = Dp[0], u1 = Dp[1], u2 = Dp[2]; Dk0[0] = u0.x; Dk0[1] = u0.y; Dk0[2] = u1.x; Dk0[3] = u1.y; Dk0[4] = u2.x; Dk0[5] = u2.y; }
            if (tab1.x >= 0) { const double2* Dp = reinterpret_cast<const double2*>(Dinv1 + (size_t)tab1.x * 36 + c6 * 6); const double2 u0 = Dp[0], u1 = Dp[1], u2 = Dp[2]; Dk1[0] = u0.x; Dk1[1] = u0.y; Dk1[2] = u1.x; Dk1[3] = u1.y; Dk1[4] = u2.x; Dk1[5] = u2.y; }
        }
    };
    load_trip((int64_t)blockIdx.x);
    double alpha = 0.0, beta = 0.0;
    if (SR) { if (!sr_head(C, parity, first, nparts_pq, nparts, red, alpha, beta)) return; }
    else {
        double pq, rz;
        if (block_total2_done(C.flags, C.part_pq, nparts_pq, C.part_rz + parity * RZ_STRIDE, nparts + C.extra_rz, red, pq, rz)) return;
        if (!(pq > 0.0)) {
            if (blockIdx.x == 0 && threadIdx.x == 0) C.flags[1] = 1;
            if (threadIdx.x == 0) C.part_rz[(parity ^ 1) * RZ_STRIDE + blockIdx.x] = 0.0;
            return;
        }
        alpha = rz / pq;
    }
    __shared__ double2 rnew[CG_BLOCK];
    __shared__ double2 btr[CG_BLOCK];
    __shared__ double rs[2 * CG_BLOCK];
    __shared__ __attribute__((aligned(16))) float lfs[KF * LF_STRIDE];
    static_assert(KF * LF_STRIDE / 4 == 2 * CG_BLOCK, "two 16-B loads per lane stage a trip's factors");
    double acc = 0.0;
    for (int64_t it = 0; it < trips; ++it) {
        const int64_t run = it * gridDim.x + blockIdx.x;
        const int64_t base = run * CG_BLOCK;
        const int64_t i = base + t;
        const bool live = i < pairs;
        double2 rr = make_double2(0.0, 0.0);
        if (live) {
            if (SR) {
                p0.x = u0.x + beta * p0.x; p0.y = u0.y + beta * p0.y;
                s0.x = q0.x + beta * s0.x; s0.y = q0.y + beta * s0.y;
                rr = make_double2(r0.x - alpha * s0.x, r0.y - alpha * s0.y);
                x0.x += alpha * p0.x; x0.y += alpha * p0.y;
                pout[i] = p0; sv[i] = s0;
            } else {
                rr = make_double2(r0.x - alpha * q0.x, r0.y - alpha * q0.y);
                x0.x += alpha * p0.x; x0.y += alpha * p0.y;
            }
            rout[i] = rr; xv[i] = x0;
        }
        reinterpret_cast<float4*>(lfs)[t] = lf0; reinterpret_cast<float4*>(lfs)[t + CG_BLOCK] = lf1;
        rnew[t] = rr;
        const double e0 = d0, e1 = d1, e2 = d2;
        const int4 tb0 = tab0, tb1 = tab1;
        __syncthreads();
        {
            const int j = t % 3;
            const double* r6 = reinterpret_cast<const double*>(rnew + (t - j));
            double2 b;
            if (j == 0) b = make_double2(r6[0] + 2.0 * (e1 * r6[5] - e2 * r6[4]), r6[1] + 2.0 * (e2 * r6[3] - e0 * r6[5]));
            else if (j == 1) b = make_double2(r6[2] + 2.0 * (e0 * r6[4] - e1 * r6[3]), r6[3]);
            else b = make_double2(r6[4], r6[5]);
            btr[t] = b;
            if (live) {
                const double2 z = lf_apply_pair(lfs + (t / 3) * LF_STRIDE, r6, j);
                zv[i] = z;
                acc += rr.x * z.x + rr.y * z.y;
            }
        }
        __syncthreads();
        double sum2[2];
#pragma unroll
        for (int round = 0; round < 2; ++round) {
            const int4 tb = round ? tb1 : tb0;
            double sum = 0.0;
            if (tb.x >= 0) {
                const double* col = reinterpret_cast<const double*>(btr) + c6;
                const uint32_t lo = (uint32_t)tb.y, hi = (uint32_t)tb.z;
#pragma unroll
                for (int m = 0; m < 8; ++m) {
                    const uint32_t kf = ((m < 4 ? lo >> (8 * m) : hi >> (8 * (m - 4))) & 0xffu);
                    if (kf != 0xffu) sum += col[kf * 6];
                }
                r1_out[(size_t)tb.x * 6 + c6] = sum;
            }
            sum2[round] = sum;
            rs[round * CG_BLOCK + t] = sum;
        }
        if (x1_out) {
            __syncthreads();
#pragma unroll
            for (int round = 0; round < 2; ++round) {
                const int4 tb = round ? tb1 : tb0;
                if (tb.x >= 0) {
                    const double* ra = rs + round * CG_BLOCK + (t - c6);
                    double x = 0.0;
#pragma unroll
                    for (int jj = 0; jj < 6; ++jj) x += (round ? Dk1[jj] : Dk0[jj]) * ra[jj];
                    x1_out[(size_t)tb.x * 6 + c6] = x;
                }
            }
        }
        (void)sum2;
        if (it + 1 < trips) { load_trip(run + gridDim.x); __syncthreads(); }
    }
    const double s = block_sum(acc, red);
    if (threadIdx.x == 0) C.part_rz[(parity ^ 1) * RZ_STRIDE + blockIdx.x] = s;
}
void launch_cg_update_mg(const GraphDev& G, const CgDev& C, const MgDev& M, const MgLevelDev* levels, const CoarseDev& K, int k, int n_pq_partials, hipStream_t st) {
    const int g = cg_grid(G);
    if (M.n_levels == 1) hipLaunchKernelGGL(cg_update_mg_kernel<false>, dim3(g), dim3(CG_BLOCK), 0, st, G, C, M, K.rc, (double*)nullptr, (const double*)nullptr, k & 1, n_pq_partials, g, 0);
    else hipLaunchKernelGGL(cg_update_mg_kernel<false>, dim3(g), dim3(CG_BLOCK), 0, st, G, C, M, levels[0].r, levels[0].x, (const double*)levels[0].Dinv, k & 1, n_pq_partials, g, 0);
}
void launch_cg_update_mg_sr(const GraphDev& G, const CgDev& C, const MgDev& M, const MgLevelDev* levels, const CoarseDev& K, int k, int first, int n_pq_partials, hipStream_t st) {
    const int g = cg_grid(G);
    if (M.n_levels == 1) hipLaunchKernelGGL(cg_update_mg_kernel<true>, dim3(g), dim3(CG_BLOCK), 0, st, G, C, M, K.rc, (double*)nullptr, (const double*)nullptr, k & 1, n_pq_partials, g, first);
    else hipLaunchKernelGGL(cg_update_mg_kernel<true>, dim3(g), dim3(CG_BLOCK), 0, st, G, C, M, levels[0].r, levels[0].x, (const double*)levels[0].Dinv, k & 1, n_pq_partials, g, first);
}
void launch_mg_apply(const GraphDev& G, const CgDev& C, const MgDev& M, const MgLevelDev* levels, const CoarseDev& K, const double* r, double* z, double* part_rz, double scale, bool inside_iteration, hipStream_t st,
                     bool restricted, double prolong_scale, const MgLevelDev* fine ,
                     const MgExchangeHook* hook, int* hook_rc) {
    const int32_t* stop = inside_iteration ? C.flags : nullptr;
    const int nl = M.n_levels;
    const unsigned g1 = (unsigned)((std::max(M.a1 - M.a0, 0) + MG_TILE_ROWS - 1) / MG_TILE_ROWS);
    bool hook_failed = false;
    auto xchg = [&](int point, int level) { if (hook && !hook_failed) { const int rc = hook->fn(hook->ctx, point, level); if (rc != 0) { hook_failed = true; if (hook_rc) *hook_rc = rc; } } };
    if (restricted) {}
    else if (fine) {
        MgLevelDev T = *fine; T.tiles = 0; T.tiles_own = 0; T.r = const_cast<double*>(r);
        if (nl == 1) hipLaunchKernelGGL(mg_sdown_kernel, dim3((unsigned)T.rT_tiles), dim3(CG_BLOCK), 0, st, T, K.rc, (double*)nullptr, (const double*)nullptr, stop);
        else hipLaunchKernelGGL(mg_sdown_kernel, dim3((unsigned)T.rT_tiles), dim3(CG_BLOCK), 0, st, T, levels[0].r, levels[0].x, (const double*)levels[0].Dinv, stop);
    }
    else if (g1 == 0) {}
    else if (nl == 1) hipLaunchKernelGGL(mg_restrict0_kernel, dim3(g1), dim3(CG_BLOCK), 0, st, M, r, K.rc, (double*)nullptr, (const double*)nullptr, stop);
    else hipLaunchKernelGGL(mg_restrict0_kernel, dim3(g1), dim3(CG_BLOCK), 0, st, M, r, levels[0].r, levels[0].x, (const double*)levels[0].Dinv, stop);
    for (int l = 1; l < nl; ++l) {
        MgLevelDev A = levels[l - 1];
        xchg(0, l);
        if (hook_failed) return;
        if (A.smoothed && A.rt_valf) {
            const unsigned g = (unsigned)(A.tiles_own + A.rT_tiles);
            if (g == 0) continue;
            if (l + 1 == nl) hipLaunchKernelGGL(mg_sdown_kernel, dim3(g), dim3(CG_BLOCK), 0, st, A, K.rc, (double*)nullptr, (const double*)nullptr, stop);
            else hipLaunchKernelGGL(mg_sdown_kernel, dim3(g), dim3(CG_BLOCK), 0, st, A, levels[l].r, levels[l].x, (const double*)levels[l].Dinv, stop);
            continue;
        }
        if (A.tiles_own == 0) continue;
        if (A.smoothed) {
            hipLaunchKernelGGL(mg_smooth_step_kernel, dim3((unsigned)A.tiles_own), dim3(CG_BLOCK), 0, st, A, (const double*)A.r, (const double*)A.x, A.t, (const double*)nullptr, (const double*)nullptr, A.u, prolong_scale, stop);
            A.r = A.t; A.x = A.u;
        }
        if (l + 1 == nl) hipLaunchKernelGGL(mg_down_kernel, dim3((unsigned)A.tiles_own), dim3(CG_BLOCK), 0, st, A, K.rc, (double*)nullptr, (const double*)nullptr, stop);
        else hipLaunchKernelGGL(mg_down_kernel, dim3((unsigned)A.tiles_own), dim3(CG_BLOCK), 0, st, A, levels[l].r, levels[l].x, (const double*)levels[l].Dinv, stop);
    }
    auto below_of = [&](int idx) { MgLevelDev B = levels[idx]; if (B.smoothed) B.x = const_cast<double*>(B.zero); return B; };
    auto expl_at = [&](int idx) { return idx >= 0 && levels[idx].smoothed && levels[idx].rt_valf != nullptr; };
    xchg(0, nl);
    if (hook_failed) return;
    hipLaunchKernelGGL(mg_dense_solve_kernel, dim3((unsigned)K.n_agg), dim3(384), 0, st, K, nl >= 2 ? below_of(nl - 2) : levels[0], nl >= 2 && !expl_at(nl - 2) ? 1 : 0, scale, stop);
    const bool fused = C.extra_rz > 0;
    const unsigned g0 = (unsigned)cg_grid(G);
    for (int l = nl - 1; l >= 1; --l) {
        MgLevelDev A = levels[l - 1];
        xchg(1, l);
        if (hook_failed) return;
        if (A.tiles_own == 0) continue;
        if (expl_at(l - 1)) {
            const double* xn = l + 1 == nl ? (const double*)K.yc : (const double*)levels[l].xf;
            if (l == 1 && fused) hipLaunchKernelGGL(mg_up_kernel<true>, dim3((unsigned)(A.tiles_own < MAX_PARTIALS ? A.tiles_own : MAX_PARTIALS)), dim3(CG_BLOCK), 0, st, A, A, 0, scale, stop, M, r, z, part_rz + g0, xn);
            else hipLaunchKernelGGL(mg_up_kernel<false>, dim3((unsigned)A.tiles_own), dim3(CG_BLOCK), 0, st, A, l >= 2 ? below_of(l - 2) : levels[0], l >= 2 && !expl_at(l - 2) ? 1 : 0, scale, stop, M, r, z, part_rz, xn);
            continue;
        }
        if (A.smoothed) {
            hipLaunchKernelGGL(mg_smooth_step_kernel, dim3((unsigned)A.tiles_own), dim3(CG_BLOCK), 0, st, A, (const double*)nullptr, (const double*)A.xt, (double*)nullptr, (const double*)A.x, (const double*)A.xt, A.y, prolong_scale, stop);
            A.xt = A.y;
        }
        if (l == 1 && fused) hipLaunchKernelGGL(mg_up_kernel<true>, dim3((unsigned)(A.tiles_own < MAX_PARTIALS ? A.tiles_own : MAX_PARTIALS)), dim3(CG_BLOCK), 0, st, A, A, 0, scale, stop, M, r, z, part_rz + g0, (const double*)nullptr);
        else hipLaunchKernelGGL(mg_up_kernel<false>, dim3((unsigned)A.tiles_own), dim3(CG_BLOCK), 0, st, A, l >= 2 ? below_of(l - 2) : levels[0], l >= 2 && !expl_at(l - 2) ? 1 : 0, scale, stop, M, r, z, part_rz, (const double*)nullptr);
    }
    xchg(2, 1);
    if (hook_failed) return;
    if (fine) hipLaunchKernelGGL(mg_prolong0s_kernel, dim3(g0), dim3(CG_BLOCK), 0, st, G, *fine, (const double*)(nl == 1 ? K.yc : levels[0].xf), r, z, part_rz, scale, stop);
    else if (!fused) hipLaunchKernelGGL(mg_prolong0_kernel, dim3(g0), dim3(CG_BLOCK), 0, st, G, M, (const double*)(nl == 1 ? K.yc : levels[0].xf), r, z, part_rz, scale, stop);
}
```

### solve_keyframe_pose_graph_amd/csrc/pgo_pcg.hip

```cpp
#include <algorithm>
#include <cmath>
#include <cstdio>
#include <cstdlib>
#include <cstring>
#include <vector>

#include "pgo_handle.hpp"

namespace pgo {

int build_two_level_aggregates(pgo_problem* p) {
    CoarseState& c = p->coarse;
    const int64_t N = p->N, Er = p->rel.size(), Es = p->swe.size();
    const int32_t* g2l = p->local_ids ? p->g2l.data() : nullptr;
    auto L = [g2l](int32_t g) -> int32_t { return g2l ? g2l[g] : g; };
    int n_agg = p->opt.coarse_aggregates;
    const int half = std::min(n_agg / 2, 256);
    if (N <= half) n_agg = (int)N;
    else n_agg = (int)std::min<int64_t>(n_agg, std::max<int64_t>(N / 8, half));
    if (n_agg >= 2 && !p->local_ids && (N + n_agg - 1) / n_agg <= 1024) {
        const int m = (int)((N + n_agg - 1) / n_agg);
        n_agg = (int)((N + m - 1) / m);
        std::vector<int32_t> agg_free((size_t)n_agg, 0);
        for (int64_t n = 0; n < N; ++n) if (p->h_node_free[n]) agg_free[n / m]++;
        std::vector<std::pair<int64_t, int64_t>> ent;
        ent.reserve((size_t)N + 2 * (size_t)(Er + Es));
        for (int64_t n = 0; n < N; ++n) if (p->h_node_free[n]) ent.push_back({(int64_t)(n / m) * n_agg + n / m, (n << 3) | 0});
        auto edge = [&](int64_t e, int32_t c1, int32_t c2, int kind_fwd) {
            if (!p->h_node_free[c1] || !p->h_node_free[c2]) return;
            const int64_t a = c1 / m, b = c2 / m;
            if (a < b) ent.push_back({a * n_agg + b, (e << 3) | kind_fwd});
            else if (a > b) ent.push_back({b * n_agg + a, (e << 3) | (kind_fwd + 1)});
            else { ent.push_back({a * n_agg + a, (e << 3) | kind_fwd}); ent.push_back({a * n_agg + a, (e << 3) | (kind_fwd + 1)}); }
        };
        for (int64_t e = 0; e < Er; ++e) edge(e, L(p->rel.c1[e]), L(p->rel.c2[e]), 1);
        for (int64_t e = 0; e < Es; ++e) edge(e, L(p->swe.c1[e]), L(p->swe.c2[e]), 3);
        for (int a = 0; a < n_agg; ++a) if (agg_free[a] == 0) ent.push_back({(int64_t)a * n_agg + a, -1});
        std::stable_sort(ent.begin(), ent.end(), [](const std::pair<int64_t, int64_t>& x, const std::pair<int64_t, int64_t>& y) { return x.first < y.first; });
        std::vector<int64_t> blk_ptr, contrib;
        std::vector<int32_t> blk_ab;
        int64_t prev = -1;
        for (const auto& kv : ent) {
            if (kv.first != prev) { blk_ptr.push_back((int64_t)contrib.size()); blk_ab.push_back((int32_t)(kv.first / n_agg)); blk_ab.push_back((int32_t)(kv.first % n_agg)); prev = kv.first; }
            if (kv.second >= 0) contrib.push_back(kv.second);
        }
        blk_ptr.push_back((int64_t)contrib.size());
        const int n_blk = (int)blk_ab.size() / 2;
        const int nc = (6 * n_agg + 63) / 64 * 64;
        HIPCHK(p, c.d_ccen.ensure((size_t)n_agg * 3)); HIPCHK(p, c.d_cd.ensure((size_t)N * 3)); HIPCHK(p, c.d_cAc.ensure((size_t)nc * nc)); HIPCHK(p, c.d_cAcf.ensure((size_t)nc * nc));
        HIPCHK(p, c.d_crc.ensure((size_t)nc * 2)); HIPCHK(p, c.d_cscr.ensure((size_t)nc * 64 + 4096)); HIPCHK(p, hipMemsetAsync(c.d_crc.p, 0, (size_t)nc * 2 * sizeof(double), p->st)); HIPCHK(p, c.d_cblk_ptr.ensure(blk_ptr.size())); HIPCHK(p, c.d_ccontrib.ensure(std::max<size_t>(contrib.size(), 1)));
        HIPCHK(p, c.d_cblk_ab.ensure(blk_ab.size())); HIPCHK(p, c.d_cagg_free.ensure(n_agg)); HIPCHK(p, c.d_cinfo.ensure(4));
        HIPCHK(p, hipMemcpyAsync(c.d_cblk_ptr.p, blk_ptr.data(), blk_ptr.size() * sizeof(int64_t), hipMemcpyHostToDevice, p->st));
        if (!contrib.empty()) HIPCHK(p, hipMemcpyAsync(c.d_ccontrib.p, contrib.data(), contrib.size() * sizeof(int64_t), hipMemcpyHostToDevice, p->st));
        HIPCHK(p, hipMemcpyAsync(c.d_cblk_ab.p, blk_ab.data(), blk_ab.size() * sizeof(int32_t), hipMemcpyHostToDevice, p->st));
        HIPCHK(p, hipMemcpyAsync(c.d_cagg_free.p, agg_free.data(), n_agg * sizeof(int32_t), hipMemcpyHostToDevice, p->st));
        HIPCHK(p, hipStreamSynchronize(p->st));
        c.K = CoarseDev{n_agg, nc, m, n_blk, c.d_ccen.p, c.d_cd.p, c.d_cAc.p, c.d_crc.p, c.d_crc.p + nc, c.d_cblk_ptr.p, c.d_cblk_ab.p, c.d_ccontrib.p, c.d_cagg_free.p, c.d_cAcf.p};
        c.built = true;
    }
    return PGO_OK;
}

static int build_coarse(pgo_problem* p) {
    CoarseState& c = p->coarse;
    c.active = false;
    const double t_coarse0 = now_s();
    if (!c.built || p->opt.coarse_aggregates <= 0) return PGO_OK;
    if (c.mode == 2) {
        if (c.retests >= 2 || c.skip_all || !(p->radius >= 9.0 * c.drop_radius)) return PGO_OK;
        ++c.retests; c.mode = 0;
    }
    if (!(c.K.m <= 64 || (p->radius >= p->opt.coarse_min_radius && c.K.m <= 1024))) return PGO_OK;
    if (c.geometry_epoch != p->lin_epoch) {
        launch_coarse_geometry(p->G, c.K, p->d_pose[p->cur].p, p->st);
        c.geometry_epoch = p->lin_epoch;
    }
    launch_coarse_assemble(p->G, p->L, p->Sc, p->C, c.K, p->st);
    int32_t* fail = c.d_cinfo.p;
    HIPCHK(p, hipMemsetAsync(fail, 0, sizeof(int32_t), p->st));
    launch_coarse_invert(c.K, c.d_cscr.p, fail, p->st);
    if (debug_break_coarse()) launch_coarse_negate(c.K, p->st);
    int32_t h = 1;
    HIPCHK(p, hipMemcpyAsync(&h, fail, sizeof(h), hipMemcpyDeviceToHost, p->st));
    HIPCHK(p, hipStreamSynchronize(p->st));
    c.active = h == 0;
    if (p->opt.verbosity > 1) std::fprintf(stderr, "[pgo] coarse operator assembled and inverted in %.3f ms (since the start of build_coarse)\n", (now_s() - t_coarse0) * 1e3);
    if (p->opt.verbosity > 0) std::fprintf(stderr, "[pgo] coarse space: %d aggregates of %d keyframes, %d blocks, radius %.1e: %s\n", c.K.n_agg, c.K.m, c.K.n_blk, p->radius, h == 0 ? "on" : "coarse operator not positive definite -> off");
    return PGO_OK;
}
void two_level_solve_begin(pgo_problem* p) {
    CoarseState& c = p->coarse;
    c.retests = 0; c.drop_radius = 0.0;
    if (c.skip > 0) { c.mode = 2; c.skip_all = true; --c.skip; }
    else { c.mode = (c.keep_streak % 4 != 0) ? 1 : 0; c.skip_all = false; }
}
void two_level_solve_end(pgo_problem* p) {
    CoarseState& c = p->coarse;
    if (c.mode == 2 && !c.skip_all) { c.backoff = std::min(2 * c.backoff + 1, 15); c.skip = c.backoff; }
    if (c.mode == 1) ++c.keep_streak; else if (c.mode == 2 && !c.skip_all) c.keep_streak = 0;
}

int build_system(pgo_problem* p, bool* ok) {
    PcgState& s = p->pcg;
    int rc;
    HIPCHK(p, hipMemsetAsync(p->d_flags.p + 4, 0, sizeof(int32_t), p->st));
    launch_build_rows(p->G, p->L, p->Sc, p->C, p->radius, 1 , p->built_mf ? p->d_lam.p : nullptr, p->st);
    if ((rc = exchange_rows(p, p->C.Dtot, 36, p->C.b, 6)) != PGO_OK) return rc;
    launch_invert_rows(p->G, p->C, p->d_flags.p + 4, p->st);
    int32_t fail = 0;
    HIPCHK(p, hipMemcpyAsync(&fail, p->d_flags.p + 4, sizeof(int32_t), hipMemcpyDeviceToHost, p->st));
    HIPCHK(p, hipStreamSynchronize(p->st));
    if (p->local_ids) {
        std::vector<double> f(1, fail ? 1.0 : 0.0);
        if ((rc = host_allreduce(p, f, 2)) != PGO_OK) return rc;
        fail = f[0] != 0.0;
    }
    *ok = fail == 0;
    p->mg.active = false; s.mg_failed = false; p->C.extra_rz = 0; s.mg_start_deferred = false;
    s.cg_predicted = (s.cg_prev_radius > 0.0 && p->radius > 0.0) ? s.cg_prev_equiv * std::sqrt(p->radius / s.cg_prev_radius) : 0.0;
    if (*ok && p->mg.built) {
        const double predicted = s.cg_predicted;
        const double start_factor = 1.75, wait_factor = 2.0;
        s.mg_switch_at = p->opt.mg_switch_iterations;
        if (predicted > 0.0 && predicted < start_factor * (double)p->opt.mg_switch_iterations) s.mg_switch_at = std::max(p->opt.mg_switch_iterations, (int)(wait_factor * predicted));
        const bool hard = p->opt.mg_switch_iterations <= 0 || predicted >= start_factor * (double)p->opt.mg_switch_iterations;
        const bool rejection_likely = p->reuse_diagonal || p->last_rho < 0.8;
        s.mg_start_deferred = hard && rejection_likely && p->opt.mg_switch_iterations > 0 && p->opt.cg_early_tolerance > p->opt.cg_rel_tolerance;
        if (s.mg_start_deferred) {
            const int prelude = 72;
            s.mg_switch_at = std::min(s.mg_switch_at, prelude);
        }
        if (hard && !s.mg_start_deferred && (rc = build_mg(p)) != PGO_OK) return rc;
    }
    else if (*ok && (rc = build_coarse(p)) != PGO_OK) return rc;
    return PGO_OK;
}
bool single_reduction(const pgo_problem* p) {
    const bool two_level = p->coarse.active && !p->mg.active;
    constexpr int64_t SINGLE_REDUCTION_MAX_KEYFRAMES = 150000;
    return p->opt.cg_single_reduction != 0 && !p->local_ids && p->built_mf && p->opt.cg_rel_tolerance >= 1e-11 && p->N_global <= SINGLE_REDUCTION_MAX_KEYFRAMES &&
           (!two_level || coarse_group_keyframes(p->coarse.K) > 0);
}
PcgForm choose_form(const pgo_problem* p, bool this_rank_only) {
    PcgForm f{PcgForm::classic_csr, PcgForm::none, 0};
    const bool mg = p->mg.active, two_level = p->coarse.active && !mg;
    const bool fused_coarse = !p->local_ids && two_level && p->built_mf && coarse_group_keyframes(p->coarse.K) > 0;
    if (p->local_ids && !this_rank_only) f.rec = PcgForm::ranks;
    else if (fused_coarse) f.rec = single_reduction(p) ? PcgForm::sr_coarse : PcgForm::classic_coarse;
    else if (single_reduction(p)) f.rec = PcgForm::sr;
    else if (p->built_mf) f.rec = PcgForm::classic_mf;
    if (fused_coarse) f.fused_parts = coarse_update_grid(p->G, p->coarse.K);
    else if (mg) f.post = f.rec != PcgForm::ranks && p->mg.M.blk_tab != nullptr ? PcgForm::mg_restricted : PcgForm::mg_cycle;
    else if (two_level) f.post = PcgForm::two_level;
    return f;
}
void pcg_matvec(pgo_problem* p, const PcgForm& f, int k, double tol2) {
    if (f.rec == PcgForm::ranks && p->built_mf) launch_mf_apply_dot(p->G, p->F, p->Sc, p->C, p->C.z, p->C.q, p->st);
    else if (f.rec == PcgForm::ranks) { launch_apply_operator(p->G, p->C, p->C.z, p->C.q, p->st); launch_cgcg_dots(p->G, p->C, p->st); }
    else if (f.rec == PcgForm::sr) launch_mf_apply_dot_live(p->G, p->F, p->Sc, p->C, p->st);
    else if (f.rec == PcgForm::sr_coarse) launch_mf_apply_dot_live_coarse(p->G, p->F, p->Sc, p->C, p->coarse.K, k > 0 ? 1 : 0, p->st);
    else if (f.rec == PcgForm::classic_coarse) launch_mf_spmv_coarse(p->G, p->F, p->Sc, p->C, p->coarse.K, k, tol2, f.fused_parts, k > 0 ? 1 : 0, p->st);
    else if (f.rec == PcgForm::classic_mf) launch_mf_spmv(p->G, p->F, p->Sc, p->C, k, tol2, p->st);
    else launch_cg_spmv(p->G, p->C, k, tol2, p->st);
}
int pcg_update(pgo_problem* p, const PcgForm& f, int k) {
    const int first = k == 0 ? 1 : 0, n_pq = p->built_mf ? mf_grid_size(p->F) : cg_grid_size(p->G);
    const bool restricted = f.post == PcgForm::mg_restricted;
    const MgState& m = p->mg;
    if (f.rec == PcgForm::ranks) {
        int rc;
        launch_cg_reduce2_live(p->C, p->C.part_pq, n_pq, p->C.part_rz, cg_grid_size(p->G), p->d_xscal.p, p->st);
        if ((rc = exchange_rows(p, p->C.q, 6, nullptr, 0, p->C.flags)) != PGO_OK || (rc = allreduce(p, p->d_xscal.p, 2, 0)) != PGO_OK) return rc;
        launch_cgcg_update(p->G, p->C, k, first, p->st, nullptr, nullptr, p->d_xscal.p);
        ++p->st_pcg_iterations;
    } else if (f.rec == PcgForm::sr_coarse) launch_cg_update_restrict_sr(p->G, p->C, p->coarse.K, k, first, k > 0 ? 1 : 0, n_pq, p->st);
    else if (f.rec == PcgForm::classic_coarse) launch_cg_update_restrict(p->G, p->C, p->coarse.K, k, n_pq, p->st);
    else if (f.rec == PcgForm::sr && restricted) launch_cg_update_mg_sr(p->G, p->C, m.M, m.levels, p->coarse.K, k, first, n_pq, p->st);
    else if (f.rec == PcgForm::sr) launch_cg_update_sr(p->G, p->C, k, first, n_pq, p->st);
    else if (restricted) launch_cg_update_mg(p->G, p->C, m.M, m.levels, p->coarse.K, k, n_pq, p->st);
    else launch_cg_update(p->G, p->C, k, n_pq, p->st);
    return PGO_OK;
}
int pcg_precond(pgo_problem* p, const PcgForm& f, int k) {
    double* const part_rz = p->C.part_rz + (size_t)((k & 1) ^ 1) * RZ_STRIDE;
    const double* const r = f.single_red() || (k & 1) ? p->C.r : p->C.r2;
    if (f.fused_coarse()) launch_coarse_solve_dot(p->coarse.K, p->C.flags, part_rz + f.fused_parts, p->st);
    else if (f.mg() && f.rec == PcgForm::ranks) return mg_apply_ranks(p, true);
    else if (f.mg()) launch_mg_apply(p->G, p->C, p->mg.M, p->mg.levels, p->coarse.K, r, p->C.z, part_rz, mg_scale(p), true, p->st, f.post == PcgForm::mg_restricted, mg_cs(p), mg_fine_view(p));
    else if (f.post == PcgForm::two_level) launch_coarse_apply(p->G, p->C, p->coarse.K, r, p->C.z, part_rz, true, p->st);
    return PGO_OK;
}
int pcg_start(pgo_problem* p, const PcgForm& f, bool warm, double tol2) {
    int rc;
    if (warm) {
        if (p->built_mf) launch_mf_apply(p->G, p->F, p->Sc, p->C, p->C.x, p->C.q, p->st);
        else launch_apply_operator(p->G, p->C, p->C.x, p->C.q, p->st);
        if ((rc = exchange_rows(p, p->C.q, 6, nullptr, 0)) != PGO_OK) return rc;
    }
    if (f.rec == PcgForm::ranks) {
        const int g = launch_cg_init_vectors(p->G, p->C, warm ? 1 : 0, p->st);
        if (f.mg() && (rc = mg_apply_ranks(p, false)) != PGO_OK) return rc;
        double* bb = p->C.scal + 12;
        launch_reduce(p->C.part_pq, g, 0, bb, p->st);
        if ((rc = allreduce(p, bb, 1, 0)) != PGO_OK) return rc;
        launch_cgcg_scalars_init(p->C, bb, tol2, p->st);
    } else if (f.precond() == 0) {
        launch_cg_init(p->G, p->C, warm ? 1 : 0, tol2, p->st);
    } else {
        int g = launch_cg_init_vectors(p->G, p->C, warm ? 1 : 0, p->st);
        const int g_bb = g;
        if (f.mg()) launch_mg_apply(p->G, p->C, p->mg.M, p->mg.levels, p->coarse.K, p->C.r, p->C.z, p->C.part_rz, mg_scale(p), false, p->st, false, mg_cs(p), mg_fine_view(p));
        else launch_coarse_apply(p->G, p->C, p->coarse.K, p->C.r, p->C.z, p->C.part_rz, false, p->st);
        if (f.fused_coarse()) {
            HIPCHK(p, hipMemsetAsync(p->C.part_rz + g, 0, (size_t)(f.fused_parts + p->C.extra_rz - g) * sizeof(double), p->st));
            g = f.fused_parts;
        }
        launch_cg_init_scalars(p->C, g, g_bb, tol2, p->st);
    }
    return PGO_OK;
}
int pcg_iteration(pgo_problem* p, const PcgForm& f, int k, double tol2) {
    int rc;
    pcg_matvec(p, f, k, tol2);
    if ((rc = pcg_update(p, f, k)) != PGO_OK) return rc;
    return pcg_precond(p, f, k);
}

namespace {

int chunk_length(const pgo_problem* p, const PcgForm& f) {
    int e = std::max(2, p->opt.cg_check_every) & ~1;
    if (f.precond() == 1) e = std::min(e, f.fused_coarse() ? 24 : 12);
    if (!f.mg()) return e;
    const MgState& m = p->mg;
    int n_sm = 0;
    for (int l = 0; l < m.M.n_levels; ++l) n_sm += (m.levels[l].smoothed && !m.levels[l].rt_valf) ? 1 : 0;
    if (f.rec == PcgForm::ranks) return std::min(e, std::max(2, (72 / (6 * m.M.n_levels + 12)) & ~1));
    return std::max(2, (72 / (2 * m.M.n_levels + 3 + 2 * n_sm)) & ~1);
}
struct EndGame {
    bool on = false, tight = false, have = false; int next = 0, k0 = 0; double rz0 = 0.0;
    void snapshot(pgo_problem* p) { if (on) launch_cg_poll(p->C, p->pcg.poll[2].flags, p->pcg.poll[2].scal, p->st); have = false; }
    void update(const pgo_problem* p, int slot, int k, int every, double tol2) {
        if (!on) return;
        const PcgState::Poll* poll = p->pcg.poll;
        const int kk = poll[slot].flags[2]; const double rz = poll[slot].scal[1], bb = poll[slot].scal[0];
        if (!have) { k0 = poll[2].flags[2]; rz0 = poll[2].scal[1]; have = true; }
        tight = false; next = every;
        if (rz > 0.0 && bb > 0.0 && rz0 > 0.0 && kk > k0 && rz < rz0) {
            const double lr = std::log(rz / rz0) / (double)(kk - k0);
            const double need = std::log(tol2 * bb / rz);
            const double left = need < 0.0 ? need / lr - (double)(k - kk) : 0.0;
            if (left < 2.0 * (double)every) {
                tight = true;
                const int want = (int)std::ceil(std::max(left, 0.0) * 1.15 + 4.0);
                next = std::max(2, std::min(every, (want + 1) & ~1));
            }
        }
        if (kk > k0) { k0 = kk; rz0 = rz; }
    }
};
struct PcgRun {
    PcgForm f; double tol2; int cap; bool want_graph; int every = 2, k = 0, n_chunks = 0, waited = -1; EndGame eg;
    int ex_k0 = -1; double ex_rz0 = 0.0;
};
void ensure_graph(pgo_problem* p, const PcgRun& R, bool may_capture) {
    PcgState& s = p->pcg;
    PcgState::CapturedChunk& cc = s.cg_chunk[R.f.precond()];
    const bool sr = R.f.single_red();
    if (!R.want_graph || s.cg_graph_failed || (cc.exec != nullptr && cc.epoch == s.build_epoch && cc.len == R.every && cc.scale == mg_scale(p) && cc.sr == sr)) { s.cg_graph = R.want_graph && !s.cg_graph_failed ? cc.exec : nullptr; return; }
    if (!may_capture) { s.cg_graph = nullptr; return; }
    if (cc.exec) { (void)hipGraphExecDestroy(cc.exec); cc.exec = nullptr; }
    hipGraph_t gr = nullptr;
    bool ok = hipStreamBeginCapture(p->st, hipStreamCaptureModeThreadLocal) == hipSuccess;
    if (ok) {
        for (int j = 0; j < R.every; ++j) (void)pcg_iteration(p, R.f, 2 + j, R.tol2);
        ok = hipStreamEndCapture(p->st, &gr) == hipSuccess && gr != nullptr;
    }
    const double t_inst = now_s();
    if (ok) ok = hipGraphInstantiate(&cc.exec, gr, nullptr, nullptr, 0) == hipSuccess;
    if (p->opt.verbosity > 1) std::fprintf(stderr, "[pgo] PCG chunk of %d iterations (preconditioner %d) captured, instantiated in %.2f ms\n", R.every, R.f.precond(), (now_s() - t_inst) * 1e3);
    if (gr) (void)hipGraphDestroy(gr);
    if (!ok) { cc.exec = nullptr; s.cg_graph_failed = true; (void)hipGetLastError(); }
    else { cc.epoch = s.build_epoch; cc.len = R.every; cc.scale = mg_scale(p); cc.sr = sr; }
    s.cg_graph = cc.exec;
}
int enqueue_poll(pgo_problem* p, int slot) {
    PcgState& s = p->pcg;
#ifdef PGO_POLL_BY_COPY
    HIPCHK(p, hipMemcpyAsync(s.poll[slot].flags, p->C.flags, 3 * sizeof(int32_t), hipMemcpyDeviceToHost, p->st));
    HIPCHK(p, hipMemcpyAsync(s.poll[slot].scal, p->C.scal, 3 * sizeof(double), hipMemcpyDeviceToHost, p->st));
#else
    launch_cg_poll(p->C, s.poll[slot].flags, s.poll[slot].scal, p->st);
#endif
    HIPCHK(p, hipEventRecord(s.poll_ev[slot], p->st));
    return PGO_OK;
}
bool may_switch_to_mg(const pgo_problem* p) { return p->mg.built && !p->mg.active && !p->pcg.mg_failed; }

void switch_estimate(pgo_problem* p, PcgRun& R, int slot) {
    const pgo_options& o = p->opt;
    PcgState& s = p->pcg;
    if (!may_switch_to_mg(p) || s.mg_start_deferred || o.mg_switch_iterations <= 0 || R.k >= s.mg_switch_at) return;
    const int kk = s.poll[slot].flags[2]; const double rz = s.poll[slot].scal[1], bb = s.poll[slot].scal[0];
    if (!(rz > 0.0 && bb > 0.0)) return;
    if (R.ex_k0 < 0) { if (kk >= 24) { R.ex_k0 = kk; R.ex_rz0 = rz; } }
    else if (kk >= 96 && kk > R.ex_k0) {
        const double lr = std::log(rz / R.ex_rz0) / (double)(kk - R.ex_k0);
        const double need = std::log(o.cg_rel_tolerance * o.cg_rel_tolerance * bb / rz);
        const double total = lr < 0.0 ? (double)kk + need / lr : 1e30;
        if (total >= 1.75 * (double)o.mg_switch_iterations && total >= 2.0 * (double)kk) s.mg_switch_at = std::min(s.mg_switch_at, R.k);
    }
}
int switch_to_mg(pgo_problem* p, PcgRun& R, int so_far) {
    int rc = build_mg(p);
    if (rc != PGO_OK) return rc;
    if (!p->mg.active) { p->pcg.mg_failed = true; return PGO_OK; }
    p->pcg.cg_extra += so_far;
    R.f = choose_form(p);
    if ((rc = pcg_start(p, R.f, true, R.tol2)) != PGO_OK) return rc;
    R.k = 0; R.n_chunks = 0; R.waited = -1; R.every = chunk_length(p, R.f);
    R.eg.tight = false; R.eg.next = R.every; R.eg.have = false; R.eg.snapshot(p);
    ensure_graph(p, R, true);
    return PGO_OK;
}

}

int run_pcg(pgo_problem* p, CgResult* res, const PcgPhase& ph) {
    const pgo_options& o = p->opt;
    PcgState& s = p->pcg;
    PcgRun R{choose_form(p), ph.tol * ph.tol, ph.max_iterations > 0 ? ph.max_iterations : o.cg_max_iterations};
    const bool multi = R.f.rec == PcgForm::ranks;
    int rc;
    if (R.f.fused_coarse()) p->C.extra_rz = coarse_solve_grid(p->coarse.K);
    else if (!p->mg.active) p->C.extra_rz = 0;
    if (ph.resume >= 0) launch_cg_set_tolerance(p->C, R.tol2, p->st);
    else if ((rc = pcg_start(p, R.f, ph.warm, R.tol2)) != PGO_OK) return rc;
    R.k = ph.resume >= 0 ? ph.resume : 0;
    R.every = chunk_length(p, R.f);
    R.want_graph = o.cg_use_graph && !s.cg_graph_failed && (!p->local_ids || (p->comm && p->comm->graph_capturable()));
    const int graph_after = debug_graph_after();
    ensure_graph(p, R, R.k >= graph_after);
    bool done = false;
    R.eg.on = o.cg_end_game != 0 && !multi;
    if (ph.switch_now && ph.resume >= 0 && may_switch_to_mg(p) && (rc = switch_to_mg(p, R, ph.resume)) != PGO_OK) return rc;
    R.eg.next = R.every;
    if (ph.resume >= 0 || R.k == 0) R.eg.snapshot(p);
    while (R.k < R.cap && !done) {
        if (R.eg.tight && R.n_chunks > 0 && R.waited < R.n_chunks - 1) {
            HIPCHK(p, hipEventSynchronize(s.poll_ev[(R.n_chunks - 1) & 1]));
            R.waited = R.n_chunks - 1;
            if (s.poll[R.waited & 1].flags[0]) { done = true; break; }
            R.eg.update(p, R.waited & 1, R.k, R.every, R.tol2);
        }
        const int first_short = R.eg.on && R.n_chunks == 0 && ph.tol >= 5e-3 ? std::min(R.every, 8) : R.every;
        const int chunk = std::min(R.eg.tight ? R.eg.next : first_short, R.cap - R.k);
        if (R.want_graph && !s.cg_graph_failed && !s.cg_graph && R.k >= graph_after && (R.k & 1) == 0) ensure_graph(p, R, true);
        if (R.k >= 2 && chunk == R.every && R.want_graph && s.cg_graph && (R.k & 1) == 0) {
            HIPCHK(p, hipGraphLaunch(s.cg_graph, p->st));
            R.k += R.every;
        } else {
            const int n = R.k == 0 ? std::min(2, chunk) : ((R.k & 1) ? 1 : chunk);
            const bool startup = R.k == 0 || (R.k & 1);
            for (int j = 0; j < n; ++j, ++R.k) if ((rc = pcg_iteration(p, R.f, R.k, R.tol2)) != PGO_OK) return rc;
            if (startup && R.k < R.cap) continue;
        }
        if ((rc = enqueue_poll(p, R.n_chunks & 1)) != PGO_OK) return rc;
        const int check = (R.n_chunks < 2 || R.eg.tight) ? R.n_chunks : R.n_chunks - 1;
        if (check > R.waited) {
            HIPCHK(p, hipEventSynchronize(s.poll_ev[check & 1]));
            R.waited = check;
            if (s.poll[check & 1].flags[0]) done = true;
            else R.eg.update(p, check & 1, R.k, R.every, R.tol2);
            if (!done) switch_estimate(p, R, check & 1);
        }
        ++R.n_chunks;
        if (!done && may_switch_to_mg(p) && R.k >= s.mg_switch_at && R.k < R.cap) {
            int32_t hflags[3] = {0, 0, 0};
            HIPCHK(p, hipMemcpyAsync(hflags, p->C.flags, sizeof(hflags), hipMemcpyDeviceToHost, p->st));
            HIPCHK(p, hipStreamSynchronize(p->st));
            if (hflags[0]) { done = true; (void)enqueue_poll(p, R.n_chunks & 1); ++R.n_chunks; break; }
            if ((rc = switch_to_mg(p, R, hflags[2])) != PGO_OK) return rc;
        }
    }
    int32_t hflags[3] = {0, 0, 0}; double hscal[3] = {0, 0, 0};
    if (R.n_chunks > 0) {
        HIPCHK(p, hipEventSynchronize(s.poll_ev[(R.n_chunks - 1) & 1]));
        std::memcpy(hflags, s.poll[(R.n_chunks - 1) & 1].flags, sizeof(hflags));
        std::memcpy(hscal, s.poll[(R.n_chunks - 1) & 1].scal, sizeof(hscal));
    } else {
        HIPCHK(p, hipMemcpyAsync(hflags, p->C.flags, sizeof(hflags), hipMemcpyDeviceToHost, p->st));
        HIPCHK(p, hipMemcpyAsync(hscal, p->C.scal, sizeof(hscal), hipMemcpyDeviceToHost, p->st));
        HIPCHK(p, hipStreamSynchronize(p->st));
    }
    res->converged = hflags[0] != 0 && hflags[1] == 0;
    if (!hflags[0] && !multi) {
        launch_cg_set_tolerance(p->C, 1e300, p->st);
        if (!R.f.single_red()) pcg_matvec(p, R.f, R.k, 1e300);
        else if ((rc = pcg_iteration(p, R.f, R.k, 1e300)) != PGO_OK) return rc;
        HIPCHK(p, hipMemcpyAsync(hflags, p->C.flags, sizeof(hflags), hipMemcpyDeviceToHost, p->st));
        HIPCHK(p, hipMemcpyAsync(hscal, p->C.scal, sizeof(hscal), hipMemcpyDeviceToHost, p->st));
        HIPCHK(p, hipStreamSynchronize(p->st));
    }
    res->iterations = hflags[2];
    res->breakdown = hflags[1] != 0;
    res->rel_residual = hscal[0] > 0 ? std::sqrt(std::max(0.0, hscal[1]) / hscal[0]) : 0.0;
    return PGO_OK;
}

int finish_system(pgo_problem* p, CgResult* cg, bool evaluated, int* precond_used) {
    const pgo_options& o = p->opt;
    CoarseState& c = p->coarse; PcgState& s = p->pcg;
    int rc;
    if (c.active && c.mode == 0 && !evaluated && !cg->breakdown && cg->converged) {
        HIPCHK(p, p->d_tmp.ensure((size_t)p->N * 6));
        HIPCHK(p, hipMemcpyAsync(p->d_tmp.p, p->C.x, (size_t)p->N * 6 * sizeof(double), hipMemcpyDeviceToDevice, p->st));
        c.active = false;
        CgResult plain{0, false, 0.0, false};
        if ((rc = run_pcg(p, &plain, PcgPhase{o.cg_rel_tolerance, -1, false, false, std::max(3 * cg->iterations, 2 * (std::max(2, o.cg_check_every) & ~1))})) != PGO_OK) return rc;
        if (plain.converged && !plain.breakdown) {
            if ((double)plain.iterations < 1.2 * (double)cg->iterations) c.retests = 2;
            c.mode = 2; cg->iterations += plain.iterations; c.drop_radius = p->radius;
        }
        else {
            c.mode = 1; c.active = true; c.backoff = 0;
            HIPCHK(p, hipMemcpyAsync(p->C.x, p->d_tmp.p, (size_t)p->N * 6 * sizeof(double), hipMemcpyDeviceToDevice, p->st));
            cg->iterations += plain.iterations;
        }
    }
    *precond_used = p->mg.active ? PGO_PRECOND_MULTIGRID : (c.active ? PGO_PRECOND_TWO_LEVEL : PGO_PRECOND_BLOCK_JACOBI);
    if (cg->breakdown && (p->mg.active || c.active) && !evaluated) {
        if (o.verbosity > 0) std::fprintf(stderr, "[pgo] %s: PCG breakdown at radius %.1e after %d iterations (preconditioner not positive definite) -> block-Jacobi for this system\n",
                                          p->mg.active ? "multigrid" : "two-level method", p->radius, cg->iterations);
        if (p->mg.active) { p->mg.active = false; s.mg_failed = true; }
        c.active = false;
        p->C.extra_rz = 0;
        s.cg_extra += cg->iterations;
        ++p->sum.pcg_retries;
        *precond_used = PGO_PRECOND_BLOCK_JACOBI | PGO_PRECOND_RETRIED;
        if ((rc = run_pcg(p, cg, PcgPhase{o.cg_rel_tolerance, -1, true})) != PGO_OK) return rc;
        if (cg->breakdown) { s.cg_extra += cg->iterations; if ((rc = run_pcg(p, cg, PcgPhase{o.cg_rel_tolerance})) != PGO_OK) return rc; }
    }
    if (!evaluated && !cg->breakdown) {
        const double equiv = p->mg.levels[0].smoothed ? 8.0 : 4.0;
        s.cg_prev_equiv = (double)s.cg_extra + (p->mg.active ? equiv : 1.0) * (double)cg->iterations; s.cg_prev_radius = p->radius;
    }
    return PGO_OK;
}

}
```

### solve_keyframe_pose_graph_amd/csrc/pgo_solver.hip

```cpp
#include <algorithm>
#include <cmath>
#include <cstdio>
#include <cstdlib>
#include <cstring>
#include <memory>
#include <string>
#include <vector>

#include "pgo_handle.hpp"

namespace {

enum { S_COST = 0, S_PRIOR_COST = 1, S_MODEL = 2, S_SW_STEP2 = 3, S_SW_XNORM2 = 4, S_GMAX = 5, S_STEP2 = 6, S_XNORM2 = 7, S_N = 8 };

int set_device(pgo_problem* p) { HIPCHK(p, hipSetDevice(p->device)); return PGO_OK; }

void meas_from_matrix(const double* T, double w, double* out8) {
    double R[9];
    for (int r = 0; r < 3; ++r) for (int c = 0; c < 3; ++c) R[r * 3 + c] = T[c * 4 + r];
    double q[4];
    eigen_matrix_to_quat(R, q);
    out8[0] = q[0]; out8[1] = q[1]; out8[2] = q[2]; out8[3] = q[3];
    out8[4] = T[12]; out8[5] = T[13]; out8[6] = T[14]; out8[7] = w;
}
// ... 1121 lines not shown
    if ((rc = set_device(p)) != PGO_OK) return rc;
    HIPCHK(p, p->d_tmp.ensure((size_t)count * 79));
    double* d1 = p->d_tmp.p; double* d2 = d1 + count * 36; double* ds = d2 + count * 36;
    launch_unpack_k1(p->G, kind, first, count, nullptr, d1, kind == 2 ? nullptr : d2, kind == 1 ? ds : nullptr, p->st);
    if (J1) HIPCHK(p, hipMemcpyAsync(J1, d1, count * 36 * sizeof(double), hipMemcpyDeviceToHost, p->st));
    if (J2 && kind != 2) HIPCHK(p, hipMemcpyAsync(J2, d2, count * 36 * sizeof(double), hipMemcpyDeviceToHost, p->st));
    if (dr_ds && kind == 1) HIPCHK(p, hipMemcpyAsync(dr_ds, ds, count * 7 * sizeof(double), hipMemcpyDeviceToHost, p->st));
    HIPCHK(p, hipStreamSynchronize(p->st));
    return PGO_OK;
}

int pgo_get_normal_blocks(pgo_problem* p, double* diag, double* grad, double* offdiag, double* sw_c, double* sw_hss, double* sw_gs) {
    if (!p) return PGO_ERR_INVALID_ARG;
    if (p->graph_dirty) { p->err = "no linearisation available"; return PGO_ERR_STATE; }
    int rc;
    if ((rc = set_device(p)) != PGO_OK) return rc;
    const int64_t Er = p->G.rel.E, Es = p->G.sw.E;
    if (diag && (rc = nodes_to_global(p, p->L.Hd, 36, diag)) != PGO_OK) return rc;
    if (grad && (rc = nodes_to_global(p, p->L.g, 6, grad)) != PGO_OK) return rc;
    if (offdiag && p->built_mf) {
        HIPCHK(p, p->d_Hoff.ensure((size_t)(p->G.rel.Epad + p->G.sw.Epad) * 36));
        p->L.Hoff = p->d_Hoff.p;
        launch_k2(p->G, p->L, true, p->st);
    }
    if (offdiag) {
        if (Er) HIPCHK(p, hipMemcpyAsync(offdiag, p->L.Hoff, Er * 36 * sizeof(double), hipMemcpyDeviceToHost, p->st));
        if (Es) HIPCHK(p, hipMemcpyAsync(offdiag + Er * 36, p->L.Hoff + (size_t)p->G.rel.Epad * 36, Es * 36 * sizeof(double), hipMemcpyDeviceToHost, p->st));
    }
    if (sw_c && Es) HIPCHK(p, hipMemcpyAsync(sw_c, p->L.c, Es * 12 * sizeof(double), hipMemcpyDeviceToHost, p->st));
    if (sw_hss && Es) HIPCHK(p, hipMemcpyAsync(sw_hss, p->L.hss, Es * sizeof(double), hipMemcpyDeviceToHost, p->st));
    if (sw_gs && Es) HIPCHK(p, hipMemcpyAsync(sw_gs, p->L.gs, Es * sizeof(double), hipMemcpyDeviceToHost, p->st));
    HIPCHK(p, hipStreamSynchronize(p->st));
    return PGO_OK;
}

int pgo_manifold_plus(pgo_problem* p, int64_t n, const double* quat, const double* t, const double* delta, double* quat_out, double* t_out) {
    if (!p || n < 0 || (n > 0 && (!quat || !delta || !quat_out))) return PGO_ERR_INVALID_ARG;
    if (n == 0) return PGO_OK;
    int rc;
    if ((rc = set_device(p)) != PGO_OK) return rc;
    const bool with_t = t != nullptr && t_out != nullptr;
    DBuf<double> d;
    HIPCHK(p, d.ensure((size_t)n * 20));
    double* dq = d.p; double* dd = dq + 4 * n; double* dqo = dd + 6 * n; double* dt = dqo + 4 * n; double* dto = dt + 3 * n;
    HIPCHK(p, hipMemcpyAsync(dq, quat, (size_t)n * 4 * sizeof(double), hipMemcpyHostToDevice, p->st));
    HIPCHK(p, hipMemcpyAsync(dd, delta, (size_t)n * 6 * sizeof(double), hipMemcpyHostToDevice, p->st));
    if (with_t) HIPCHK(p, hipMemcpyAsync(dt, t, (size_t)n * 3 * sizeof(double), hipMemcpyHostToDevice, p->st));
    launch_manifold_plus(n, dq, with_t ? dt : nullptr, dd, dqo, with_t ? dto : nullptr, p->st);
    HIPCHK(p, hipMemcpyAsync(quat_out, dqo, (size_t)n * 4 * sizeof(double), hipMemcpyDeviceToHost, p->st));
    if (with_t) HIPCHK(p, hipMemcpyAsync(t_out, dto, (size_t)n * 3 * sizeof(double), hipMemcpyDeviceToHost, p->st));
    HIPCHK(p, hipStreamSynchronize(p->st));
    return PGO_OK;
}

int pgo_apply_normal_operator(pgo_problem* p, const double* x, double* y) {
    if (!p || !x || !y) return PGO_ERR_INVALID_ARG;
    if (!p->in_solve) { p->err = "pgo_apply_normal_operator needs an open solve (pgo_solve_begin)"; return PGO_ERR_STATE; }
    int rc;
    if ((rc = set_device(p)) != PGO_OK) return rc;
    const pgo_options& o = p->opt;
    if (!p->reuse_diagonal) launch_lm_diag(p->G, p->L, p->Sc, o.min_lm_diagonal, o.max_lm_diagonal, p->st);
    bool ok = true;
    if ((rc = build_system(p, &ok)) != PGO_OK) return rc;
    HIPCHK(p, p->d_io.ensure((size_t)p->N * 12));
    double* xin = p->d_io.p; double* yout = p->d_io.p + (size_t)p->N * 6;
    if ((rc = nodes_from_global(p, x, 6, xin)) != PGO_OK) return rc;
    if (p->built_mf) launch_mf_apply(p->G, p->F, p->Sc, p->C, xin, yout, p->st);
    else launch_apply_operator(p->G, p->C, xin, yout, p->st);
    if ((rc = exchange_rows(p, yout, 6, nullptr, 0)) != PGO_OK) return rc;
    return nodes_to_global(p, yout, 6, y);
}

int pgo_comm_init(pgo_problem* p, int32_t rank, int32_t world, const uint8_t id[PGO_COMM_ID_BYTES]) {
    if (!p || !id || world < 1 || rank < 0 || rank >= world) return PGO_ERR_INVALID_ARG;
    return attach_comm(p, [&](std::unique_ptr<pgo_comm::Comm>& c) { return pgo_comm::make_rccl_comm(id, rank, world, p->st, c, p->err); });
}
int pgo_comm_init_custom(pgo_problem* p, int32_t rank, int32_t world, pgo_allreduce_fn fn, void* ctx) {
    if (!p || !fn || world < 1 || rank < 0 || rank >= world) return PGO_ERR_INVALID_ARG;
    return attach_comm(p, [&](std::unique_ptr<pgo_comm::Comm>& c) { c = pgo_comm::make_custom_comm(fn, ctx, rank, world, p->st); return PGO_OK; });
}
int pgo_comm_set_exchange(pgo_problem* p, pgo_exchange_fn fn) {
    return p && p->comm && p->comm->set_exchange(fn) ? PGO_OK : PGO_ERR_INVALID_ARG;
}
int pgo_comm_init_local(pgo_problem* p, int32_t rank, int32_t world, void* group) {
    if (!p || !group || rank < 0 || rank >= world) return PGO_ERR_INVALID_ARG;
    return attach_comm(p, [&](std::unique_ptr<pgo_comm::Comm>& c) { return pgo_comm::make_local_comm(group, rank, world, p->device, p->st, c, p->err); });
}
int pgo_get_sharding_stats(pgo_problem* p, pgo_sharding_stats* out) {
    if (!p || !out) return PGO_ERR_INVALID_ARG;
    std::memset(out, 0, sizeof(*out));
    out->world = p->world(); out->rank = p->rank();
    if (!p->local_ids || p->graph_dirty) return PGO_OK;
    out->keyframes_local = p->N;
    for (double w : p->h_own) if (w != 0.0) ++out->keyframes_owned;
    out->keyframes_shared = p->n_sh_mine; out->shared_global = p->n_sh_global;
    out->pcg_iterations = p->st_pcg_iterations; out->exchanges = p->st_exchanges; out->allreduces = p->st_allreduces;
    out->bytes_sent_neighbour = p->st_bytes_neighbour; out->bytes_allreduce = p->st_bytes_allreduce;
    const double fine = (double)p->fine_plan.x.n_send() * 48.0 + 16.0;
    out->bytes_sent_per_bj_iteration = fine; out->exchanges_per_bj_iteration = 1;
    out->bytes_round5_per_bj_iteration = (6.0 * (double)p->n_sh_global + 2.0) * 8.0;
    if (p->mg.built && !p->mg.fresh_pending() && p->mg.M.n_levels >= 1) {
        const int nl = p->mg.M.n_levels;
        out->mg_levels = nl; out->mg_levels_distributed = p->mg.levels_distributed;
        out->mg_rows_total = p->mg.rows_total; out->mg_rows_own = p->mg.rows_own; out->mg_blocks_total = p->mg.blocks_total; out->mg_blocks_own = p->mg.blocks_own;
        double bytes = fine; int nx = 1;
        auto count = [&](int point, int lv) { int plan; double* v1; double* v2; const double* dinv; if (mg_exchange_at(p, point, lv, &plan, &v1, &v2, &dinv) && p->mg.lvl_plan[(size_t)plan].plan) { bytes += (double)p->mg.lvl_plan[(size_t)plan].plan->n_send() * (v2 && !dinv ? 96.0 : 48.0); ++nx; } };
        for (int l = 1; l <= nl; ++l) count(0, l);
        for (int l = nl - 1; l >= 1; --l) count(1, l);
        count(2, 1);
        out->bytes_sent_per_mg_iteration = bytes; out->exchanges_per_mg_iteration = nx;
        out->bytes_round5_per_mg_iteration = (6.0 * (double)p->n_sh_global + 2.0 + 6.0 * (double)p->mg.M.n1) * 8.0;
        const int fw = p->mg.first_whole;
        for (int l = 0; l + 1 < nl; ++l) {
            const MgLevelDev& A = p->mg.levels[l];
            const int64_t all = A.nnzb + (A.smoothed ? (int64_t)A.n_ps + 2 * (int64_t)A.n_w : 0);
            const int64_t own = l < fw ? (A.su_blk1 - A.su_blk0) + (A.smoothed ? (int64_t)(A.su_ps1 - A.su_ps0) + 2 * (int64_t)(A.su_w1 - A.su_w0) : 0) : all;
            out->mg_setup_blocks_total += all; out->mg_setup_blocks_own += own;
        }
        out->bytes_allreduce_replicated_setup = (double)p->mg.levels[0].nnzb * 288.0;
        out->mg_setup_levels_own_rows = fw; out->mg_setup_exchanges = 1;
        if (fw > 0) {
            double sb = 0.0; int nx = 0;
            auto add = [&](const pgo_mg::ExchangePlan& X, double bytes_per_row) { if (!plan_is_empty(X)) { sb += (double)X.n_send() * bytes_per_row; ++nx; } };
            for (const pgo_mg::BlockPlan& B : p->mg.setup.val) add(B.x, 288.0);
            for (int l = 0; l < fw; ++l) {
                nx += 9; sb += 24.0;
                if ((size_t)l < p->mg.lvl_plan.size() && p->mg.lvl_plan[(size_t)l].plan) sb += 8.0 * (double)p->mg.lvl_plan[(size_t)l].plan->n_send() * 48.0;
                if (!p->mg.levels[l].smoothed) continue;
                if ((size_t)l < p->mg.lvl_plan.size() && p->mg.lvl_plan[(size_t)l].plan) add(*p->mg.lvl_plan[(size_t)l].plan, 288.0);
                add(p->mg.setup.ps[(size_t)l], 288.0); add(p->mg.setup.rv[(size_t)l], 144.0);
            }
            out->bytes_sent_per_mg_setup = sb; out->mg_setup_exchanges = nx;
        }
    }
    return PGO_OK;
}
int pgo_mg_level_norms(pgo_problem* p, int32_t level, double* out8) {
    if (!p || !out8) return PGO_ERR_INVALID_ARG;
    for (int k = 0; k < 8; ++k) out8[k] = 0.0;
    if (!p->mg.built || p->mg.fresh_pending() || level < 1 || level > p->mg.M.n_levels || (size_t)(level - 1) >= p->mg.own.size()) { p->err = "pgo_mg_level_norms: no such level (is a hierarchy installed?)"; return PGO_ERR_INVALID_ARG; }
    int rc;
    if ((rc = set_device(p)) != PGO_OK) return rc;
    const MgLevelDev& A = p->mg.levels[level - 1];
    const OwnRange& R = p->mg.own[(size_t)level - 1];
    HIPCHK(p, hipStreamSynchronize(p->st));
    auto sq64 = [&](const double* dev, int64_t first, int64_t count, double* out) -> int {
        if (!dev || count <= 0) return PGO_OK;
        std::vector<double> h((size_t)count);
        HIPCHK(p, hipMemcpy(h.data(), dev + first, (size_t)count * sizeof(double), hipMemcpyDeviceToHost));
        long double s = 0.0L; for (double v : h) s += (long double)v * v;
        *out = (double)s; return PGO_OK;
    };
    auto sq32 = [&](const float* dev, int64_t first, int64_t count, double* out) -> int {
        if (!dev || count <= 0) return PGO_OK;
        std::vector<float> h((size_t)count);
        HIPCHK(p, hipMemcpy(h.data(), dev + first, (size_t)count * sizeof(float), hipMemcpyDeviceToHost));
        long double s = 0.0L; for (float v : h) s += (long double)v * v;
        *out = (double)s; return PGO_OK;
    };
    const bool sparse = level < p->mg.M.n_levels;
    if ((rc = sq64(A.val, R.blk0 * 36, (R.blk1 - R.blk0) * 36, out8 + 0)) != PGO_OK) return rc;
    if (sparse) {
        if ((rc = sq32(A.valf, R.blk0 * 36, (R.blk1 - R.blk0) * 36, out8 + 1)) != PGO_OK) return rc;
        if ((rc = sq64(A.Dinv, R.row0 * 36, (R.row1 - R.row0) * 36, out8 + 2)) != PGO_OK) return rc;
        if (A.smoothed && A.rt_valf) {
            if ((rc = sq32(A.rt_valf, R.w0 * 36, (R.w1 - R.w0) * 36, out8 + 3)) != PGO_OK) return rc;
            if ((rc = sq32(A.r_valf, R.rT0 * 36, (R.rT1 - R.rT0) * 36, out8 + 4)) != PGO_OK) return rc;
        }
    } else if ((rc = sq64(p->coarse.K.Ac, 0, (int64_t)p->coarse.K.nc * p->coarse.K.nc, out8 + 5)) != PGO_OK) return rc;
    return PGO_OK;
}
int pgo_comm_destroy(pgo_problem* p) {
    if (!p) return PGO_ERR_INVALID_ARG;
    p->comm.reset();
    mg_drop_pending(p);
    p->graph_dirty = true;
    return PGO_OK;
}

int pgo_partition_edges(int32_t policy, int32_t world, int64_t n_nodes, const double* t_xyz, int64_t n_rel, const int32_t* rel_c1, const int32_t* rel_c2,
                        int64_t n_sw, const int32_t* sw_c1, const int32_t* sw_c2, int32_t* node_part, int32_t* rel_rank, int32_t* sw_rank) {
    if (world < 1 || n_nodes < 0 || n_rel < 0 || n_sw < 0 || (n_rel > 0 && (!rel_c1 || !rel_c2 || !rel_rank)) || (n_sw > 0 && (!sw_c1 || !sw_c2 || !sw_rank))) return PGO_ERR_INVALID_ARG;
    if (policy == PGO_PARTITION_CONTIGUOUS) {
        for (int cls = 0; cls < 2; ++cls) {
            const int64_t n = cls ? n_sw : n_rel; int32_t* out = cls ? sw_rank : rel_rank;
            for (int r = 0; r < world; ++r) for (int64_t e = (n * r) / world; e < (n * (r + 1)) / world; ++e) out[e] = r;
        }
        return PGO_OK;
    }
    if (policy != PGO_PARTITION_CHAIN && policy != PGO_PARTITION_SPATIAL) return PGO_ERR_INVALID_ARG;
    if (policy == PGO_PARTITION_SPATIAL && n_nodes > 0 && !t_xyz) return PGO_ERR_INVALID_ARG;
    for (int64_t e = 0; e < n_rel; ++e) if (rel_c1[e] < 0 || rel_c1[e] >= n_nodes || rel_c2[e] < 0 || rel_c2[e] >= n_nodes) return PGO_ERR_INVALID_ARG;
    for (int64_t e = 0; e < n_sw; ++e) if (sw_c1[e] < 0 || sw_c1[e] >= n_nodes || sw_c2[e] < 0 || sw_c2[e] >= n_nodes) return PGO_ERR_INVALID_ARG;
    std::vector<double> load((size_t)n_nodes, 0.0);
    for (int64_t e = 0; e < n_rel; ++e) load[std::max(rel_c1[e], rel_c2[e])] += 1.0;
    for (int64_t e = 0; e < n_sw; ++e) load[std::max(sw_c1[e], sw_c2[e])] += 1.0;
    for (double& v : load) v += 1e-3;
    std::vector<int32_t> part((size_t)n_nodes, 0);
    if (policy == PGO_PARTITION_CHAIN) {
        std::vector<double> c((size_t)n_nodes);
        double acc = 0.0;
        for (int64_t i = 0; i < n_nodes; ++i) { acc += load[i]; c[i] = acc; }
        for (int64_t i = 0; i < n_nodes; ++i) part[i] = (int32_t)std::min((c[i] - load[i]) * (double)world / acc, (double)(world - 1));
    } else {
        std::vector<int32_t> idx((size_t)n_nodes), tmp;
        for (int64_t i = 0; i < n_nodes; ++i) idx[i] = (int32_t)i;
        struct Job { int64_t b, e; int lo, hi; };
        std::vector<Job> stack{{0, n_nodes, 0, world}};
        while (!stack.empty()) {
            const Job j = stack.back(); stack.pop_back();
            if (j.hi - j.lo <= 1 || j.e - j.b <= 0) { for (int64_t k = j.b; k < j.e; ++k) part[idx[k]] = j.lo; continue; }
            const int mid = (j.lo + j.hi) / 2;
            double mn[3] = {1e300, 1e300, 1e300}, mx[3] = {-1e300, -1e300, -1e300};
            for (int64_t k = j.b; k < j.e; ++k) for (int a = 0; a < 3; ++a) { const double v = t_xyz[(size_t)idx[k] * 3 + a]; mn[a] = std::min(mn[a], v); mx[a] = std::max(mx[a], v); }
            int axis = 0;
            for (int a = 1; a < 3; ++a) if (mx[a] - mn[a] > mx[axis] - mn[axis]) axis = a;
            std::stable_sort(idx.begin() + j.b, idx.begin() + j.e, [&](int32_t x, int32_t y) { return t_xyz[(size_t)x * 3 + axis] < t_xyz[(size_t)y * 3 + axis]; });
            const int64_t len = j.e - j.b;
            std::vector<double> c((size_t)len);
            double acc = 0.0;
            for (int64_t k = 0; k < len; ++k) { acc += load[idx[j.b + k]]; c[k] = acc; }
            const double target = acc * (double)(mid - j.lo) / (double)(j.hi - j.lo);
            int64_t k = std::lower_bound(c.begin(), c.end(), target) - c.begin();
            if (len > 1) k = std::min(std::max<int64_t>(k, 1), len - 1); else k = len;
            stack.push_back({j.b + k, j.e, mid, j.hi});
            stack.push_back({j.b, j.b + k, j.lo, mid});
        }
    }
    for (int64_t e = 0; e < n_rel; ++e) rel_rank[e] = part[std::max(rel_c1[e], rel_c2[e])];
    for (int64_t e = 0; e < n_sw; ++e) sw_rank[e] = part[std::max(sw_c1[e], sw_c2[e])];
    if (node_part) std::copy(part.begin(), part.end(), node_part);
    return PGO_OK;
}

int pgo_time_kernel(pgo_problem* p, int32_t which, int32_t launches, double* avg_ms, double* algorithmic_bytes) {
    if (!p || launches <= 0 || !avg_ms) return PGO_ERR_INVALID_ARG;
    if (!p->in_solve) { p->err = "pgo_time_kernel needs an open solve (pgo_solve_begin)"; return PGO_ERR_STATE; }
    int rc;
    if ((rc = set_device(p)) != PGO_OK) return rc;
    EventPair ev;
    HIPCHK(p, ev.create());
    const hipEvent_t e0 = ev.e0, e1 = ev.e1;
    int np = 0;
    const int nxt = p->cur ^ 1;
    const GraphDev& G = p->G;
    double bytes = 0, best_ms = -1.0;
    if (which == 6 || which == 7 || which == 8) {
        if (!p->mg.built || !p->built_mf || (p->local_ids && which == 6)) { p->err = "pgo_time_kernel: this graph has no multigrid hierarchy (mg_min_keyframes) / several ranks: only the level kernels (7) can be timed"; return PGO_ERR_STATE; }
        const pgo_options& o = p->opt;
        if (!p->reuse_diagonal) launch_lm_diag(p->G, p->L, p->Sc, o.min_lm_diagonal, o.max_lm_diagonal, p->st);
        bool ok = true;
        if ((rc = build_system(p, &ok)) != PGO_OK) return rc;
        if (!p->mg.active && (rc = build_mg(p)) != PGO_OK) return rc;
        if (!p->mg.active) { p->err = "pgo_time_kernel: the multigrid operators of this system are not positive definite"; return PGO_ERR_NUMERIC; }
        if (!p->local_ids) { if ((rc = pcg_start(p, choose_form(p), false, 0.0)) != PGO_OK) return rc; }
        else { launch_cg_init_vectors(p->G, p->C, 0, p->st); if ((rc = mg_apply_ranks(p, false)) != PGO_OK) return rc; launch_cg_set_tolerance(p->C, 0.0, p->st); }
    }
    const int turns = (p->comm && (which == 7 || which == 8)) ? p->world() : 1;
    for (int turn = 0; turn < turns; ++turn) {
    if (turns > 1) { HIPCHK(p, hipStreamSynchronize(p->st)); if (!p->comm->barrier()) { p->err = "in-process communicator: a rank left during pgo_time_kernel"; return PGO_ERR_COMM; } if (turn != p->rank()) continue; }
    if (which == 5 && single_reduction(p)) {
        p->err = "pgo_time_kernel(5): the single-reduction update cannot be timed without its matvec; time the iteration (2) and the matvec (4) and subtract"; return PGO_ERR_STATE;
    }
    if (which == 2 || which == 4 || which == 5) {
        const pgo_options& o = p->opt;
        if (!p->reuse_diagonal) launch_lm_diag(p->G, p->L, p->Sc, o.min_lm_diagonal, o.max_lm_diagonal, p->st);
        bool ok = true;
        if ((rc = build_system(p, &ok)) != PGO_OK) return rc;
        p->mg.active = false; p->coarse.active = false; p->C.extra_rz = 0;
        launch_cg_init(p->G, p->C, 0, 0.0, p->st);
    }
    const double N = (double)G.N, E = (double)(G.rel.E + G.sw.E), Es = (double)G.sw.E;
    const int batches = turns > 1 ? 3 : 1;
    for (int rep = 0; rep < 1 + batches; ++rep) {
        const int n = rep == 0 ? 1 : launches;
        if (rep >= 1) HIPCHK(p, hipEventRecord(e0, p->st));
        for (int i = 0; i < n; ++i) {
            switch (which) {
                case 0: launch_k1(G, p->d_pose[p->cur].p, p->d_swv[p->cur].p, true, part(p, 0), &np, p->st); bytes = k1_algorithmic_bytes(G, true); break;
                case 1: launch_k2(G, p->L, !p->built_mf, p->st, p->built_mf ? &p->F : nullptr); bytes = (624.0 * G.rel.E + 688.0 * Es) + 288.0 * E + 336.0 * N + 112.0 * Es; break;
                case 2: case 4: case 5: {
                          const int kk = rep == 0 ? 0 : i + 1;
                          const PcgForm f = choose_form(p, true);
                          const bool sr = f.single_red();
                          if (which != 5) pcg_matvec(p, f, kk, 0.0);
                          if (which != 4 && (rc = pcg_update(p, f, kk)) != PGO_OK) return rc;
                          const double lanes_rel = (double)(p->mf_pair_lanes + p->mf_rel_side_lanes), lanes_sw = (double)p->mf_sw_lanes;
                          const double mv = p->built_mf ? lanes_rel * (128.0 + 12.0) + lanes_sw * (128.0 + 12.0 + 8.0) + N * ((sr ? 2.0 : 4.0) * 48.0 + 48.0 + 13.0)
                                                        : 288.0 * (N + 2.0 * E) + 4.0 * (N + 2.0 * E) + N * 4.0 * 48.0;
                          const double up = N * ((sr ? 11.0 : 7.0) * 48.0 + 96.0);
                          bytes = which == 2 ? mv + up : which == 4 ? mv : up;
                          break; }
                case 3: launch_k1(G, p->d_pose[nxt].p, p->d_swv[nxt].p, false, part(p, 5), &np, p->st); bytes = k1_algorithmic_bytes(G, false); break;
                case 6: case 7: {
                          const int kk = rep == 0 ? 0 : i + 1;
                          if (p->local_ids) {
                              launch_mg_apply(G, p->C, p->mg.M, p->mg.levels, p->coarse.K, p->C.r, p->C.z, p->C.part_rz, mg_scale(p), false, p->st, false, mg_cs(p), nullptr);
                              bytes = (double)p->mg.blocks_own * 148.0 + (double)p->mg.rows_own * (288.0 + 24.0 + 8.0 * 48.0 + 16.0) + (double)p->coarse.K.nc * (double)p->coarse.K.nc * 4.0 + (double)p->coarse.K.nc * 16.0;
                              break;
                          }
                          PcgForm f = choose_form(p);
                          const bool sr = f.single_red();
                          if (which == 6) { pcg_matvec(p, f, kk, 0.0); if ((rc = pcg_update(p, f, kk)) != PGO_OK) return rc; }
                          else f.post = PcgForm::mg_cycle;
                          if ((rc = pcg_precond(p, f, kk)) != PGO_OK) return rc;
                          const double lanes_rel = (double)(p->mf_pair_lanes + p->mf_rel_side_lanes), lanes_sw = (double)p->mf_sw_lanes;
                          const double fine = lanes_rel * (128.0 + 12.0) + lanes_sw * (128.0 + 12.0 + 8.0) + N * ((sr ? 2.0 : 4.0) * 48.0 + 48.0 + 13.0) + N * ((sr ? 11.0 : 7.0) * 48.0 + 96.0);
                          double cyc = N * (24.0 + 16.0 / 8.0 * 8.0)  + N * (2.0 * 48.0 + 24.0 + 4.0 + 4.0) ;
                          for (int l = 0; l + 1 < p->mg.M.n_levels; ++l) {
                              const MgLevelDev& A = p->mg.levels[l];
                              if (A.smoothed && A.rt_valf)
                                  cyc += (double)A.nnzb * (144.0 + 4.0) + 2.0 * (double)A.n_w * (144.0 + 4.0) + (double)A.n * (288.0 + 24.0 + 8.0 * 48.0 + 16.0) + (double)A.n_next * (288.0 + 2.0 * 48.0 + 8.0);
                              else
                              cyc += (A.smoothed ? 4.0 : 2.0) * (double)A.nnzb * (144.0 + 4.0) + (double)A.n * ((A.smoothed ? 4.0 : 2.0) * 288.0  + 24.0 + (A.smoothed ? 18.0 : 10.0) * 48.0 + 16.0);
                          }
                          cyc += (double)p->coarse.K.nc * (double)p->coarse.K.nc * 4.0 + (double)p->coarse.K.nc * 16.0;
                          bytes = which == 6 ? fine + cyc : cyc;
                          break; }
                case 8: {
                          const bool hoff_valid = !p->built_mf || p->hoff_epoch == p->lin_epoch;
                          if ((rc = mg_operators(p, p->coarse.d_cinfo.p, hoff_valid, true, -1.0)) != PGO_OK) return rc;
                          bytes = 0.0;
                          break; }
                default: return PGO_ERR_INVALID_ARG;
            }
        }
        if (rep >= 1) HIPCHK(p, hipEventRecord(e1, p->st));
        HIPCHK(p, hipStreamSynchronize(p->st));
        if (rep >= 1) { float msb = 0; HIPCHK(p, hipEventElapsedTime(&msb, e0, e1)); if (best_ms < 0.0 || (double)msb < best_ms) best_ms = (double)msb; }
    }
    }
    if (turns > 1 && !p->comm->barrier()) { p->err = "in-process communicator: a rank left during pgo_time_kernel"; return PGO_ERR_COMM; }
    if (which == 8) { p->mg.active = false; if ((rc = build_mg(p)) != PGO_OK) return rc; }
    *avg_ms = best_ms / launches;
    if (algorithmic_bytes) *algorithmic_bytes = bytes;
    return PGO_OK;
}
int pgo_time_linearize_kernel(pgo_problem* p, int32_t launches, double* avg_ms, double* bytes) { return pgo_time_kernel(p, 0, launches, avg_ms, bytes); }

int pgo_time_vio_odometry_kernel(pgo_problem* p, int32_t f_max, int32_t launches, double* avg_ms, double* algorithmic_bytes) {
    if (!p || launches <= 0 || !avg_ms || f_max < 1) return PGO_ERR_INVALID_ARG;
    if (p->n_vio < 2) { p->err = "no resident VIO poses"; return PGO_ERR_STATE; }
    int rc;
    if ((rc = set_device(p)) != PGO_OK) return rc;
    std::vector<int32_t> c;
    for (int64_t u = 0; u < p->n_vio; ++u) for (int f = 1; f <= f_max; ++f) if (u - f >= 0) c.push_back((int32_t)u);
    const int64_t n = (int64_t)c.size();
    for (int64_t u = 0; u < p->n_vio; ++u) for (int f = 1; f <= f_max; ++f) if (u - f >= 0) c.push_back((int32_t)(u - f));
    DBuf<int32_t> d_c; DBuf<double> d_meas;
    HIPCHK(p, d_c.ensure((size_t)2 * n)); HIPCHK(p, d_meas.ensure((size_t)8 * n));
    HIPCHK(p, hipMemcpyAsync(d_c.p, c.data(), (size_t)2 * n * sizeof(int32_t), hipMemcpyHostToDevice, p->st));
    EventPair ev;
    HIPCHK(p, ev.create());
    const hipEvent_t e0 = ev.e0, e1 = ev.e1;
    launch_vio_odometry(n, d_c.p, d_c.p + n, p->d_vio.p, 1, d_meas.p, p->st);
    HIPCHK(p, hipEventRecord(e0, p->st));
    for (int i = 0; i < launches; ++i) launch_vio_odometry(n, d_c.p, d_c.p + n, p->d_vio.p, 1, d_meas.p, p->st);
    HIPCHK(p, hipEventRecord(e1, p->st));
    HIPCHK(p, hipStreamSynchronize(p->st));
    float ms = 0;
    HIPCHK(p, hipEventElapsedTime(&ms, e0, e1));
    *avg_ms = (double)ms / launches;
    if (algorithmic_bytes) *algorithmic_bytes = 128.0 * (double)p->n_vio + (8.0 + 64.0) * (double)n;
    return PGO_OK;
}

int pgo_dense_spd_inverse(pgo_problem* p, int32_t n, const double* a, double* a_inv, int32_t launches, double* avg_ms) {
    if (!p || n <= 0 || !a || !a_inv || launches < 1) return PGO_ERR_INVALID_ARG;
    int rc;
    if ((rc = set_device(p)) != PGO_OK) return rc;
    const int nc = (n + 63) / 64 * 64;
    std::vector<double> h((size_t)nc * nc, 0.0);
    for (int i = 0; i < nc; ++i) {
        if (i < n) std::memcpy(&h[(size_t)i * nc], a + (size_t)i * n, (size_t)n * sizeof(double));
        else h[(size_t)i * nc + i] = 1.0;
    }
    DBuf<double> d_a, d_scr; DBuf<int32_t> d_fail;
    HIPCHK(p, d_a.ensure((size_t)nc * nc)); HIPCHK(p, d_scr.ensure((size_t)nc * 64 + 4096)); HIPCHK(p, d_fail.ensure(1));
    CoarseDev K{}; K.nc = nc; K.Ac = d_a.p;
    EventPair ev;
    HIPCHK(p, ev.create());
    const hipEvent_t e0 = ev.e0, e1 = ev.e1;
    float total = 0;
    for (int l = 0; l < launches; ++l) {
        HIPCHK(p, hipMemcpyAsync(d_a.p, h.data(), h.size() * sizeof(double), hipMemcpyHostToDevice, p->st));
        HIPCHK(p, hipMemsetAsync(d_fail.p, 0, sizeof(int32_t), p->st));
        HIPCHK(p, hipEventRecord(e0, p->st));
        launch_coarse_invert(K, d_scr.p, d_fail.p, p->st);
        HIPCHK(p, hipEventRecord(e1, p->st));
        HIPCHK(p, hipStreamSynchronize(p->st));
        float ms = 0;
        HIPCHK(p, hipEventElapsedTime(&ms, e0, e1));
        total += ms;
    }
    int32_t fail = 1;
    HIPCHK(p, hipMemcpy(&fail, d_fail.p, sizeof(fail), hipMemcpyDeviceToHost));
    HIPCHK(p, hipMemcpy(h.data(), d_a.p, h.size() * sizeof(double), hipMemcpyDeviceToHost));
    for (int i = 0; i < n; ++i) std::memcpy(a_inv + (size_t)i * n, &h[(size_t)i * nc], (size_t)n * sizeof(double));
    if (avg_ms) *avg_ms = (double)total / launches;
    if (fail) { p->err = "matrix is not numerically positive definite"; return PGO_ERR_NUMERIC; }
    return PGO_OK;
}

int pgo_device_synchronize(pgo_problem* p) {
    if (!p) return PGO_ERR_INVALID_ARG;
    int rc;
    if ((rc = set_device(p)) != PGO_OK) return rc;
    if ((rc = mg_fresh_install(p)) != PGO_OK) return rc;
    HIPCHK(p, hipStreamSynchronize(p->st));
    return PGO_OK;
}

const char* pgo_strerror(int code) {
    switch (code) {
        case PGO_OK: return "ok";
        case PGO_ERR_INVALID_ARG: return "invalid argument";
        case PGO_ERR_NO_DEVICE: return "no usable HIP device (libpgo has no CPU fallback)";
        case PGO_ERR_HIP: return "HIP runtime error";
        case PGO_ERR_OUT_OF_MEMORY: return "out of device memory";
        case PGO_ERR_STATE: return "call order violated";
        case PGO_ERR_COMM: return "RCCL error";
        case PGO_ERR_NUMERIC: return "non-finite value";
        default: return "unknown error";
    }
}
const char* pgo_last_error(const pgo_problem* p) { return p ? p->err.c_str() : ""; }
#ifndef PGO_SOURCE_SHA256
#define PGO_SOURCE_SHA256 "unknown (not built by _build.py)"
#endif
const char* pgo_build_info(void) { return "libpgo sources sha256:" PGO_SOURCE_SHA256; }

}
```

Baseline: 112.1.

## Split PCG update: move off-critical-path vector work into rider workgroups of MG cycle kernels

The single-reduction MG-restricted PCG update is split. A slimmer critical kernel now computes only the residual, s, and the restriction to the first coarse level. The direction/x update and the Jacobi z=L r application with its r·z partial are deferred to extra 'rider' workgroups appended to two coarse-level MG kernels, chosen as the ones with the fewest tiles. This shortens the serial update kernel and fills idle CUs during small coarse-level launches. The cost is extra complexity, a consistency check between the rider host list and the cycle's launches, and possible contention with the coarse-level work.

```diff
diff --git a/solve_keyframe_pose_graph_amd/csrc/pgo_handle.hpp b/solve_keyframe_pose_graph_amd/csrc/pgo_handle.hpp
--- a/solve_keyframe_pose_graph_amd/csrc/pgo_handle.hpp
+++ b/solve_keyframe_pose_graph_amd/csrc/pgo_handle.hpp
@@ -22,6 +22,21 @@
 inline bool debug_hooks_enabled() { static const bool on = []() { const char* e = std::getenv("PGO_ENABLE_DEBUG_HOOKS"); return e && e[0] == '1' && e[1] == 0; }(); return on; }
 inline bool debug_poison() { static const bool on = []() { const char* e = std::getenv("PGO_DEBUG_POISON"); return debug_hooks_enabled() && e && e[0] == '1' && e[1] == 0; }(); return on; }
 inline bool debug_break_coarse() { if (!debug_hooks_enabled()) return false; const char* e = std::getenv("PGO_DEBUG_BREAK_COARSE"); return e && e[0] == '1' && e[1] == 0; }
+
+inline bool debug_no_split_update() { static const bool on = []() { const char* e = std::getenv("PGO_DEBUG_NO_SPLIT_UPDATE"); return debug_hooks_enabled() && e && e[0] == '1' && e[1] == 0; }(); return on; }
+inline bool debug_split_hosts(int* a, int* b) {
+    static const int v = []() {
+        const char* e = std::getenv("PGO_DEBUG_SPLIT_HOSTS");
+        if (!debug_hooks_enabled() || !e) return -1;
+        char* end = nullptr; const long x = std::strtol(e, &end, 10);
+        if (!end || *end != ',' || x < 0 || x > 63) return -1;
+        const long y = std::strtol(end + 1, &end, 10);
+        return (end && *end == 0 && y >= x && y <= 63) ? (int)(x * 64 + y) : -1;
+    }();
+    if (v < 0) return false;
+    *a = v / 64; *b = v % 64;
+    return true;
+}
 
 inline int debug_graph_after() {
     static const int v = []() {
@@ -271,6 +286,7 @@
     enum Post { none, mg_cycle, mg_restricted, two_level };
     Rec rec; Post post;
     int fused_parts;
+    UpdSplit split;
     bool single_red() const { return rec == sr || rec == sr_coarse; }
     bool fused_coarse() const { return rec == sr_coarse || rec == classic_coarse; }
     bool mg() const { return post == mg_cycle || post == mg_restricted; }
diff --git a/solve_keyframe_pose_graph_amd/csrc/pgo_internal.hpp b/solve_keyframe_pose_graph_amd/csrc/pgo_internal.hpp
--- a/solve_keyframe_pose_graph_amd/csrc/pgo_internal.hpp
+++ b/solve_keyframe_pose_graph_amd/csrc/pgo_internal.hpp
@@ -156,6 +156,13 @@
     double* scal;
     int32_t* flags;
 };
+struct UpdRiderDev {
+    int32_t kind, riders, parity, first;
+    int64_t N;
+    const double* scal; const double* r; const float* Lf;
+    double* z; double* p; double* x; double* part_rz;
+};
+struct UpdSplit { int host_a = -1, host_b = -1; bool on() const { return host_a >= 0; } };
 
 void launch_k1(const GraphDev& G, const double* pose8, const double* sw, bool want_jacobian, double* partials , int* n_partials, hipStream_t st);
 void launch_prior(const GraphDev& G, const double* pose8, bool want_jacobian, double* partial_cost , hipStream_t st);
@@ -246,9 +253,13 @@
 void launch_mg_apply(const GraphDev& G, const CgDev& C, const MgDev& M, const MgLevelDev* levels, const CoarseDev& K, const double* r, double* z, double* part_rz, double scale, bool inside_iteration, hipStream_t st,
                      bool restricted = false , double prolong_scale = 0.0 ,
                      const MgLevelDev* fine = nullptr ,
-                     const MgExchangeHook* hook = nullptr , int* hook_rc = nullptr);
+                     const MgExchangeHook* hook = nullptr , int* hook_rc = nullptr,
+                     const UpdSplit* split = nullptr , int parity = 0, int first = 0,
+                     int* n_hosts = nullptr );
+int mg_rider_hosts(const CgDev& C, const MgDev& M, const MgLevelDev* levels, int* tiles );
 void launch_cg_update_mg(const GraphDev& G, const CgDev& C, const MgDev& M, const MgLevelDev* levels, const CoarseDev& K, int k, int n_pq_partials, hipStream_t st);
 void launch_cg_update_mg_sr(const GraphDev& G, const CgDev& C, const MgDev& M, const MgLevelDev* levels, const CoarseDev& K, int k, int first, int n_pq_partials, hipStream_t st);
+void launch_cg_update_mg_crit(const GraphDev& G, const CgDev& C, const MgDev& M, const MgLevelDev* levels, const CoarseDev& K, int k, int first, int n_pq_partials, hipStream_t st);
 
 double k1_algorithmic_bytes(const GraphDev& G, bool want_jacobian);
 
diff --git a/solve_keyframe_pose_graph_amd/csrc/pgo_mg_kernels.hpp b/solve_keyframe_pose_graph_amd/csrc/pgo_mg_kernels.hpp
--- a/solve_keyframe_pose_graph_amd/csrc/pgo_mg_kernels.hpp
+++ b/solve_keyframe_pose_graph_amd/csrc/pgo_mg_kernels.hpp
@@ -512,9 +512,73 @@
     __shared__ double tb[CG_BLOCK];
     mg_smooth_step_tile(A, (int)blockIdx.x + A.tile0, in_r, in_x, out_w, add1, add2, out, cs, stop, xch, tb);
 }
-__global__ __launch_bounds__(CG_BLOCK) void mg_sdown_kernel(MgLevelDev A, double* __restrict__ r_next, double* __restrict__ x_next, const double* __restrict__ Dinv_next, const int32_t* __restrict__ stop) {
-    __shared__ double xch[CG_BLOCK * 7];
+__device__ __forceinline__ void upd_rider_direction(const UpdRiderDev& U, int rb) {
+    const double alpha = U.scal[9 + 2 * U.parity], gamma = U.scal[8 + 2 * U.parity];
+    double beta = 0.0;
+    if (!U.first) { const double gamma_prev = U.scal[8 + 2 * (U.parity ^ 1)]; beta = gamma / gamma_prev; }
+    const double2* __restrict__ zv = reinterpret_cast<const double2*>(U.z);
+    double2* __restrict__ pout = reinterpret_cast<double2*>(U.p);
+    double2* __restrict__ xv = reinterpret_cast<double2*>(U.x);
+    const int64_t pairs = U.N * 3;
+    for (int64_t i = (int64_t)rb * CG_BLOCK + threadIdx.x; i < pairs; i += (int64_t)U.riders * CG_BLOCK) {
+        const double2 u0 = zv[i];
+        double2 p0 = pout[i], x0 = xv[i];
+        p0.x = u0.x + beta * p0.x; p0.y = u0.y + beta * p0.y;
+        x0.x += alpha * p0.x; x0.y += alpha * p0.y;
+        pout[i] = p0; xv[i] = x0;
+    }
+}
+__device__ __forceinline__ void upd_rider_jacobi(const UpdRiderDev& U, int rb, double* lds, double* red) {
+    constexpr int KF = CG_BLOCK / 3;
+    double2* rnew = reinterpret_cast<double2*>(lds);
+    float* lfs = reinterpret_cast<float*>(lds + 2 * CG_BLOCK);
+    const double2* __restrict__ rin = reinterpret_cast<const double2*>(U.r);
+    double2* __restrict__ zv = reinterpret_cast<double2*>(U.z);
+    const int t = threadIdx.x;
+    const int64_t pairs = U.N * 3;
+    const int64_t stride = (int64_t)U.riders * CG_BLOCK;
+    const int64_t trips = (pairs + stride - 1) / stride;
+    double acc = 0.0;
+    for (int64_t it = 0; it < trips; ++it) {
+        const int64_t base = (it * U.riders + rb) * CG_BLOCK;
+        const int64_t i = base + t;
+        const bool live = i < pairs;
+        double2 rr = make_double2(0.0, 0.0);
+        float4 lf0 = make_float4(0.f, 0.f, 0.f, 0.f), lf1 = lf0;
+        if (live) rr = rin[i];
+        const int64_t first_node = base / 3;
+        const float4* lp = reinterpret_cast<const float4*>(U.Lf + (size_t)first_node * LF_STRIDE);
+        if (first_node + t / 6 < U.N) lf0 = lp[t];
+        if (first_node + (t + CG_BLOCK) / 6 < U.N) lf1 = lp[t + CG_BLOCK];
+        reinterpret_cast<float4*>(lfs)[t] = lf0; reinterpret_cast<float4*>(lfs)[t + CG_BLOCK] = lf1;
+        rnew[t] = rr;
+        __syncthreads();
+        if (live) {
+            const int j = t % 3;
+            const double* r6 = reinterpret_cast<const double*>(rnew + (t - j));
+            const double2 z = lf_apply_pair(lfs + (t / 3) * LF_STRIDE, r6, j);
+            zv[i] = z;
+            acc += rr.x * z.x + rr.y * z.y;
+        }
+        if (it + 1 < trips) __syncthreads();
+    }
+    const double s = block_sum(acc, red);
+    if (threadIdx.x == 0) U.part_rz[rb] = s;
+    static_assert(KF * LF_STRIDE / 4 == 2 * CG_BLOCK, "two 16-B loads per lane stage a trip's factors");
+}
+__device__ __forceinline__ bool upd_riders(const UpdRiderDev& U, int own, const int32_t* __restrict__ stop, double* lds, double* red) {
+    if (U.kind == 0 || (int)blockIdx.x < own) return false;
+    const int rb = (int)blockIdx.x - own;
+    if ((stop && *stop) || rb >= U.riders) return true;
+    if (U.kind & 1) upd_rider_direction(U, rb);
+    if (U.kind & 2) upd_rider_jacobi(U, rb, lds, red);
+    return true;
+}
+__global__ __launch_bounds__(CG_BLOCK) void mg_sdown_kernel(MgLevelDev A, double* __restrict__ r_next, double* __restrict__ x_next, const double* __restrict__ Dinv_next, const int32_t* __restrict__ stop,
+                                                             UpdRiderDev U) {
+    __shared__ __attribute__((aligned(16))) double xch[CG_BLOCK * 7];
     __shared__ double tb[CG_BLOCK];
+    if (upd_riders(U, A.tiles_own + A.rT_tiles, stop, xch, tb)) return;
     if ((int)blockIdx.x < A.tiles_own) { mg_smooth_step_tile(A, (int)blockIdx.x + A.tile0, A.r, A.x, nullptr, A.x, nullptr, A.y, 1.0, stop, xch, tb); return; }
     const int stopped = stop ? *stop : 0;
     const int tile = (int)blockIdx.x - A.tiles_own;
@@ -807,10 +871,11 @@
 #define MG_TL(slot) do {} while (0)
 #endif
 __global__ __launch_bounds__(CG_BLOCK) void mg_down_kernel(MgLevelDev A, double* __restrict__ r_next, double* __restrict__ x_next, const double* __restrict__ Dinv_next,
-                                                            const int32_t* __restrict__ stop) {
-    __shared__ double xch[CG_BLOCK * 7];
+                                                            const int32_t* __restrict__ stop, UpdRiderDev U) {
+    __shared__ __attribute__((aligned(16))) double xch[CG_BLOCK * 7];
     __shared__ double tb[CG_BLOCK];
     __shared__ double cb[CG_BLOCK];
+    if (upd_riders(U, A.tiles_own, stop, xch, tb)) return;
     MG_TL(0);
     const int stopped = stop ? *stop : 0;
     const int q6 = threadIdx.x / 6, c = threadIdx.x % 6;
@@ -901,10 +966,11 @@
 template <bool FINE>
 __global__ __launch_bounds__(CG_BLOCK) void mg_up_kernel(MgLevelDev A, MgLevelDev Below, int has_below, double scale, const int32_t* __restrict__ stop,
                                                           MgDev M, const double* __restrict__ rfine, double* __restrict__ zfine, double* __restrict__ part_extra,
-                                                          const double* __restrict__ xnext = nullptr) {
-    __shared__ double xch[CG_BLOCK * 7];
+                                                          const double* __restrict__ xnext, UpdRiderDev U) {
+    __shared__ __attribute__((aligned(16))) double xch[CG_BLOCK * 7];
     __shared__ double tb[CG_BLOCK];
     __shared__ double xb[CG_BLOCK];
+    if (!FINE && upd_riders(U, A.tiles_own, stop, xch, tb)) return;
     const int stopped = stop ? *stop : 0;
     const int q6 = threadIdx.x / 6, c = threadIdx.x % 6;
     const int li = q6 & ((MG_TILE_ROWS >> A.seg_shift) - 1), sg = q6 >> (5 - A.seg_shift);
@@ -1041,9 +1107,10 @@
 #else
 #define PGO_SR_MG_WAVES 3
 #endif
-template <bool SR>
-__global__ __launch_bounds__(CG_BLOCK, SR ? PGO_SR_MG_WAVES : 1) void cg_update_mg_kernel(GraphDev G, CgDev C, MgDev M, double* __restrict__ r1_out, double* __restrict__ x1_out, const double* __restrict__ Dinv1,
-                                                                 int parity, int nparts_pq, int nparts, int first) {
+template <bool SR, bool CRIT>
+__device__ __forceinline__ void cg_update_mg_body(GraphDev G, CgDev C, MgDev M, double* __restrict__ r1_out, double* __restrict__ x1_out, const double* __restrict__ Dinv1,
+                                                  int parity, int nparts_pq, int nparts, int first) {
+    static_assert(SR || !CRIT, "the split update exists in the single-reduction form only");
     static_assert(CG_BLOCK / 3 == MG_BLOCK0, "one workgroup trip of the vector update = one run of the slot table");
     __shared__ double red[2 * (CG_BLOCK / 64) + 1];
     const double2* __restrict__ rin = reinterpret_cast<const double2*>(SR ? C.r : (parity ? C.r2 : C.r));
@@ -1072,14 +1139,17 @@
             tab1 = M.blk_tab[(size_t)run * MG_BLOCK0 + (t + CG_BLOCK) / 6];
         }
         if (i < pairs) {
-            r0 = rin[i]; q0 = qv[i]; p0 = pcur[i]; x0 = xv[i];
-            if (SR) { u0 = zv[i]; s0 = sv[i]; }
+            r0 = rin[i]; q0 = qv[i];
+            if (!CRIT) { p0 = pcur[i]; x0 = xv[i]; }
+            if (SR) { if (!CRIT) u0 = zv[i]; s0 = sv[i]; }
             const double* d = M.d0 + (size_t)(i / 3) * 3; d0 = d[0]; d1 = d[1]; d2 = d[2];
         }
         const int64_t first_node = base / 3;
-        const float4* lp = reinterpret_cast<const float4*>(C.Lf + (size_t)first_node * LF_STRIDE);
-        if (first_node + t / 6 < G.N) lf0 = lp[t];
-        if (first_node + (t + CG_BLOCK) / 6 < G.N) lf1 = lp[t + CG_BLOCK];
+        if (!CRIT) {
+            const float4* lp = reinterpret_cast<const float4*>(C.Lf + (size_t)first_node * LF_STRIDE);
+            if (first_node + t / 6 < G.N) lf0 = lp[t];
+            if (first_node + (t + CG_BLOCK) / 6 < G.N) lf1 = lp[t + CG_BLOCK];
+        }
 #pragma unroll
         for (int jj = 0; jj < 6; ++jj) { Dk0[jj] = 0.0; Dk1[jj] = 0.0; }
         if (x1_out) {
@@ -1114,18 +1184,19 @@
         double2 rr = make_double2(0.0, 0.0);
         if (live) {
             if (SR) {
-                p0.x = u0.x + beta * p0.x; p0.y = u0.y + beta * p0.y;
+                if (!CRIT) { p0.x = u0.x + beta * p0.x; p0.y = u0.y + beta * p0.y; }
                 s0.x = q0.x + beta * s0.x; s0.y = q0.y + beta * s0.y;
                 rr = make_double2(r0.x - alpha * s0.x, r0.y - alpha * s0.y);
-                x0.x += alpha * p0.x; x0.y += alpha * p0.y;
-                pout[i] = p0; sv[i] = s0;
+                if (!CRIT) { x0.x += alpha * p0.x; x0.y += alpha * p0.y; pout[i] = p0; }
+                sv[i] = s0;
             } else {
                 rr = make_double2(r0.x - alpha * q0.x, r0.y - alpha * q0.y);
                 x0.x += alpha * p0.x; x0.y += alpha * p0.y;
             }
-            rout[i] = rr; xv[i] = x0;
-        }
-        reinterpret_cast<float4*>(lfs)[t] = lf0; reinterpret_cast<float4*>(lfs)[t + CG_BLOCK] = lf1;
+            rout[i] = rr;
+            if (!CRIT) xv[i] = x0;
+        }
+        if (!CRIT) { reinterpret_cast<float4*>(lfs)[t] = lf0; reinterpret_cast<float4*>(lfs)[t + CG_BLOCK] = lf1; }
         rnew[t] = rr;
         const double e0 = d0, e1 = d1, e2 = d2;
         const int4 tb0 = tab0, tb1 = tab1;
@@ -1138,7 +1209,7 @@
             else if (j == 1) b = make_double2(r6[2] + 2.0 * (e0 * r6[4] - e1 * r6[3]), r6[3]);
             else b = make_double2(r6[4], r6[5]);
             btr[t] = b;
-            if (live) {
+            if (!CRIT && live) {
                 const double2 z = lf_apply_pair(lfs + (t / 3) * LF_STRIDE, r6, j);
                 zv[i] = z;
                 acc += rr.x * z.x + rr.y * z.y;
@@ -1180,8 +1251,21 @@
         (void)sum2;
         if (it + 1 < trips) { load_trip(run + gridDim.x); __syncthreads(); }
     }
+    if (CRIT) return;
     const double s = block_sum(acc, red);
     if (threadIdx.x == 0) C.part_rz[(parity ^ 1) * RZ_STRIDE + blockIdx.x] = s;
+}
+template <bool SR>
+__global__ __launch_bounds__(CG_BLOCK, SR ? PGO_SR_MG_WAVES : 1) void cg_update_mg_kernel(GraphDev G, CgDev C, MgDev M, double* __restrict__ r1_out, double* __restrict__ x1_out, const double* __restrict__ Dinv1,
+                                                                 int parity, int nparts_pq, int nparts, int first) {
+    cg_update_mg_body<SR, false>(G, C, M, r1_out, x1_out, Dinv1, parity, nparts_pq, nparts, first);
+}
+#ifndef PGO_SR_CRIT_WAVES
+#define PGO_SR_CRIT_WAVES 4
+#endif
+__global__ __launch_bounds__(CG_BLOCK, PGO_SR_CRIT_WAVES) void cg_update_mg_crit_kernel(GraphDev G, CgDev C, MgDev M, double* __restrict__ r1_out, double* __restrict__ x1_out, const double* __restrict__ Dinv1,
+                                                                                       int parity, int nparts_pq, int nparts, int first) {
+    cg_update_mg_body<true, true>(G, C, M, r1_out, x1_out, Dinv1, parity, nparts_pq, nparts, first);
 }
 void launch_cg_update_mg(const GraphDev& G, const CgDev& C, const MgDev& M, const MgLevelDev* levels, const CoarseDev& K, int k, int n_pq_partials, hipStream_t st) {
     const int g = cg_grid(G);
@@ -1193,9 +1277,48 @@
     if (M.n_levels == 1) hipLaunchKernelGGL(cg_update_mg_kernel<true>, dim3(g), dim3(CG_BLOCK), 0, st, G, C, M, K.rc, (double*)nullptr, (const double*)nullptr, k & 1, n_pq_partials, g, first);
     else hipLaunchKernelGGL(cg_update_mg_kernel<true>, dim3(g), dim3(CG_BLOCK), 0, st, G, C, M, levels[0].r, levels[0].x, (const double*)levels[0].Dinv, k & 1, n_pq_partials, g, first);
 }
+void launch_cg_update_mg_crit(const GraphDev& G, const CgDev& C, const MgDev& M, const MgLevelDev* levels, const CoarseDev& K, int k, int first, int n_pq_partials, hipStream_t st) {
+    const int g = cg_grid(G);
+    if (M.n_levels == 1) hipLaunchKernelGGL(cg_update_mg_crit_kernel, dim3(g), dim3(CG_BLOCK), 0, st, G, C, M, K.rc, (double*)nullptr, (const double*)nullptr, k & 1, n_pq_partials, g, first);
+    else hipLaunchKernelGGL(cg_update_mg_crit_kernel, dim3(g), dim3(CG_BLOCK), 0, st, G, C, M, levels[0].r, levels[0].x, (const double*)levels[0].Dinv, k & 1, n_pq_partials, g, first);
+}
+int mg_rider_hosts(const CgDev& C, const MgDev& M, const MgLevelDev* levels, int* tiles) {
+    const int nl = M.n_levels;
+    const bool fused = C.extra_rz > 0;
+    int n = 0;
+    for (int l = 1; l < nl; ++l) {
+        const MgLevelDev& A = levels[l - 1];
+        if (A.smoothed && A.rt_valf) { if (A.tiles_own + A.rT_tiles > 0) tiles[n++] = A.tiles_own + A.rT_tiles; }
+        else if (A.tiles_own > 0) tiles[n++] = A.tiles_own;
+    }
+    for (int l = nl - 1; l >= 1; --l) {
+        const MgLevelDev& A = levels[l - 1];
+        if (A.tiles_own == 0 || (l == 1 && fused)) continue;
+        tiles[n++] = A.tiles_own;
+    }
+    return n;
+}
 void launch_mg_apply(const GraphDev& G, const CgDev& C, const MgDev& M, const MgLevelDev* levels, const CoarseDev& K, const double* r, double* z, double* part_rz, double scale, bool inside_iteration, hipStream_t st,
                      bool restricted, double prolong_scale, const MgLevelDev* fine ,
-                     const MgExchangeHook* hook, int* hook_rc) {
+                     const MgExchangeHook* hook, int* hook_rc, const UpdSplit* split, int parity, int first, int* n_hosts) {
+    UpdRiderDev U0{}; U0.kind = 0;
+    int e_next = 0;
+    unsigned rider_wgs = 0;
+    auto rider = [&]() {
+        UpdRiderDev U = U0;
+        rider_wgs = 0;
+        if (split && split->on()) {
+            const int e = e_next;
+            U.kind = (e == split->host_a ? 1 : 0) | (e == split->host_b ? 2 : 0);
+            if (U.kind) {
+                U.riders = cg_grid(G); U.parity = parity; U.first = first; U.N = G.N;
+                U.scal = C.scal; U.r = r; U.Lf = C.Lf; U.z = z; U.p = C.p; U.x = C.x; U.part_rz = part_rz;
+                rider_wgs = (unsigned)U.riders;
+            }
+        }
+        ++e_next;
+        return U;
+    };
     const int32_t* stop = inside_iteration ? C.flags : nullptr;
     const int nl = M.n_levels;
     const unsigned g1 = (unsigned)((std::max(M.a1 - M.a0, 0) + MG_TILE_ROWS - 1) / MG_TILE_ROWS);
@@ -1204,8 +1327,8 @@
     if (restricted) {}
     else if (fine) {
         MgLevelDev T = *fine; T.tiles = 0; T.tiles_own = 0; T.r = const_cast<double*>(r);
-        if (nl == 1) hipLaunchKernelGGL(mg_sdown_kernel, dim3((unsigned)T.rT_tiles), dim3(CG_BLOCK), 0, st, T, K.rc, (double*)nullptr, (const double*)nullptr, stop);
-        else hipLaunchKernelGGL(mg_sdown_kernel, dim3((unsigned)T.rT_tiles), dim3(CG_BLOCK), 0, st, T, levels[0].r, levels[0].x, (const double*)levels[0].Dinv, stop);
+        if (nl == 1) hipLaunchKernelGGL(mg_sdown_kernel, dim3((unsigned)T.rT_tiles), dim3(CG_BLOCK), 0, st, T, K.rc, (double*)nullptr, (const double*)nullptr, stop, U0);
+        else hipLaunchKernelGGL(mg_sdown_kernel, dim3((unsigned)T.rT_tiles), dim3(CG_BLOCK), 0, st, T, levels[0].r, levels[0].x, (const double*)levels[0].Dinv, stop, U0);
     }
     else if (g1 == 0) {}
     else if (nl == 1) hipLaunchKernelGGL(mg_restrict0_kernel, dim3(g1), dim3(CG_BLOCK), 0, st, M, r, K.rc, (double*)nullptr, (const double*)nullptr, stop);
@@ -1217,8 +1340,9 @@
         if (A.smoothed && A.rt_valf) {
             const unsigned g = (unsigned)(A.tiles_own + A.rT_tiles);
             if (g == 0) continue;
-            if (l + 1 == nl) hipLaunchKernelGGL(mg_sdown_kernel, dim3(g), dim3(CG_BLOCK), 0, st, A, K.rc, (double*)nullptr, (const double*)nullptr, stop);
-            else hipLaunchKernelGGL(mg_sdown_kernel, dim3(g), dim3(CG_BLOCK), 0, st, A, levels[l].r, levels[l].x, (const double*)levels[l].Dinv, stop);
+            const UpdRiderDev U = rider();
+            if (l + 1 == nl) hipLaunchKernelGGL(mg_sdown_kernel, dim3(g + rider_wgs), dim3(CG_BLOCK), 0, st, A, K.rc, (double*)nullptr, (const double*)nullptr, stop, U);
+            else hipLaunchKernelGGL(mg_sdown_kernel, dim3(g + rider_wgs), dim3(CG_BLOCK), 0, st, A, levels[l].r, levels[l].x, (const double*)levels[l].Dinv, stop, U);
             continue;
         }
         if (A.tiles_own == 0) continue;
@@ -1226,8 +1350,9 @@
             hipLaunchKernelGGL(mg_smooth_step_kernel, dim3((unsigned)A.tiles_own), dim3(CG_BLOCK), 0, st, A, (const double*)A.r, (const double*)A.x, A.t, (const double*)nullptr, (const double*)nullptr, A.u, prolong_scale, stop);
             A.r = A.t; A.x = A.u;
         }
-        if (l + 1 == nl) hipLaunchKernelGGL(mg_down_kernel, dim3((unsigned)A.tiles_own), dim3(CG_BLOCK), 0, st, A, K.rc, (double*)nullptr, (const double*)nullptr, stop);
-        else hipLaunchKernelGGL(mg_down_kernel, dim3((unsigned)A.tiles_own), dim3(CG_BLOCK), 0, st, A, levels[l].r, levels[l].x, (const double*)levels[l].Dinv, stop);
+        const UpdRiderDev U = rider();
+        if (l + 1 == nl) hipLaunchKernelGGL(mg_down_kernel, dim3((unsigned)A.tiles_own + rider_wgs), dim3(CG_BLOCK), 0, st, A, K.rc, (double*)nullptr, (const double*)nullptr, stop, U);
+        else hipLaunchKernelGGL(mg_down_kernel, dim3((unsigned)A.tiles_own + rider_wgs), dim3(CG_BLOCK), 0, st, A, levels[l].r, levels[l].x, (const double*)levels[l].Dinv, stop, U);
     }
     auto below_of = [&](int idx) { MgLevelDev B = levels[idx]; if (B.smoothed) B.x = const_cast<double*>(B.zero); return B; };
     auto expl_at = [&](int idx) { return idx >= 0 && levels[idx].smoothed && levels[idx].rt_valf != nullptr; };
@@ -1243,19 +1368,26 @@
         if (A.tiles_own == 0) continue;
         if (expl_at(l - 1)) {
             const double* xn = l + 1 == nl ? (const double*)K.yc : (const double*)levels[l].xf;
-            if (l == 1 && fused) hipLaunchKernelGGL(mg_up_kernel<true>, dim3((unsigned)(A.tiles_own < MAX_PARTIALS ? A.tiles_own : MAX_PARTIALS)), dim3(CG_BLOCK), 0, st, A, A, 0, scale, stop, M, r, z, part_rz + g0, xn);
-            else hipLaunchKernelGGL(mg_up_kernel<false>, dim3((unsigned)A.tiles_own), dim3(CG_BLOCK), 0, st, A, l >= 2 ? below_of(l - 2) : levels[0], l >= 2 && !expl_at(l - 2) ? 1 : 0, scale, stop, M, r, z, part_rz, xn);
+            if (l == 1 && fused) hipLaunchKernelGGL(mg_up_kernel<true>, dim3((unsigned)(A.tiles_own < MAX_PARTIALS ? A.tiles_own : MAX_PARTIALS)), dim3(CG_BLOCK), 0, st, A, A, 0, scale, stop, M, r, z, part_rz + g0, xn, U0);
+            else {
+                const UpdRiderDev U = rider();
+                hipLaunchKernelGGL(mg_up_kernel<false>, dim3((unsigned)A.tiles_own + rider_wgs), dim3(CG_BLOCK), 0, st, A, l >= 2 ? below_of(l - 2) : levels[0], l >= 2 && !expl_at(l - 2) ? 1 : 0, scale, stop, M, r, z, part_rz, xn, U);
+            }
             continue;
         }
         if (A.smoothed) {
             hipLaunchKernelGGL(mg_smooth_step_kernel, dim3((unsigned)A.tiles_own), dim3(CG_BLOCK), 0, st, A, (const double*)nullptr, (const double*)A.xt, (double*)nullptr, (const double*)A.x, (const double*)A.xt, A.y, prolong_scale, stop);
             A.xt = A.y;
         }
-        if (l == 1 && fused) hipLaunchKernelGGL(mg_up_kernel<true>, dim3((unsigned)(A.tiles_own < MAX_PARTIALS ? A.tiles_own : MAX_PARTIALS)), dim3(CG_BLOCK), 0, st, A, A, 0, scale, stop, M, r, z, part_rz + g0, (const double*)nullptr);
-        else hipLaunchKernelGGL(mg_up_kernel<false>, dim3((unsigned)A.tiles_own), dim3(CG_BLOCK), 0, st, A, l >= 2 ? below_of(l - 2) : levels[0], l >= 2 && !expl_at(l - 2) ? 1 : 0, scale, stop, M, r, z, part_rz, (const double*)nullptr);
+        if (l == 1 && fused) hipLaunchKernelGGL(mg_up_kernel<true>, dim3((unsigned)(A.tiles_own < MAX_PARTIALS ? A.tiles_own : MAX_PARTIALS)), dim3(CG_BLOCK), 0, st, A, A, 0, scale, stop, M, r, z, part_rz + g0, (const double*)nullptr, U0);
+        else {
+            const UpdRiderDev U = rider();
+            hipLaunchKernelGGL(mg_up_kernel<false>, dim3((unsigned)A.tiles_own + rider_wgs), dim3(CG_BLOCK), 0, st, A, l >= 2 ? below_of(l - 2) : levels[0], l >= 2 && !expl_at(l - 2) ? 1 : 0, scale, stop, M, r, z, part_rz, (const double*)nullptr, U);
+        }
     }
     xchg(2, 1);
     if (hook_failed) return;
     if (fine) hipLaunchKernelGGL(mg_prolong0s_kernel, dim3(g0), dim3(CG_BLOCK), 0, st, G, *fine, (const double*)(nl == 1 ? K.yc : levels[0].xf), r, z, part_rz, scale, stop);
     else if (!fused) hipLaunchKernelGGL(mg_prolong0_kernel, dim3(g0), dim3(CG_BLOCK), 0, st, G, M, (const double*)(nl == 1 ? K.yc : levels[0].xf), r, z, part_rz, scale, stop);
-}
+    if (n_hosts) *n_hosts = e_next;
+}
diff --git a/solve_keyframe_pose_graph_amd/csrc/pgo_pcg.hip b/solve_keyframe_pose_graph_amd/csrc/pgo_pcg.hip
--- a/solve_keyframe_pose_graph_amd/csrc/pgo_pcg.hip
+++ b/solve_keyframe_pose_graph_amd/csrc/pgo_pcg.hip
@@ -141,6 +141,21 @@
     return p->opt.cg_single_reduction != 0 && !p->local_ids && p->built_mf && p->opt.cg_rel_tolerance >= 1e-11 && p->N_global <= SINGLE_REDUCTION_MAX_KEYFRAMES &&
            (!two_level || coarse_group_keyframes(p->coarse.K) > 0);
 }
+static UpdSplit choose_split(const pgo_problem* p) {
+    UpdSplit sp;
+    if (debug_no_split_update() || mg_fine_view(p)) return sp;
+    int tiles[2 * MG_MAX_LEVELS];
+    const int n = mg_rider_hosts(p->C, p->mg.M, p->mg.levels, tiles);
+    if (n < 2) return sp;
+    int a = 0;
+    for (int e = 1; e < n; ++e) if (tiles[e] < tiles[a]) a = e;
+    int b = a == 0 ? 1 : 0;
+    for (int e = 0; e < n; ++e) if (e != a && tiles[e] < tiles[b]) b = e;
+    sp.host_a = std::min(a, b); sp.host_b = std::max(a, b);
+    int da, db;
+    if (debug_split_hosts(&da, &db) && db < n) { sp.host_a = da; sp.host_b = db; }
+    return sp;
+}
 PcgForm choose_form(const pgo_problem* p, bool this_rank_only) {
     PcgForm f{PcgForm::classic_csr, PcgForm::none, 0};
     const bool mg = p->mg.active, two_level = p->coarse.active && !mg;
@@ -152,6 +167,7 @@
     if (fused_coarse) f.fused_parts = coarse_update_grid(p->G, p->coarse.K);
     else if (mg) f.post = f.rec != PcgForm::ranks && p->mg.M.blk_tab != nullptr ? PcgForm::mg_restricted : PcgForm::mg_cycle;
     else if (two_level) f.post = PcgForm::two_level;
+    if (f.rec == PcgForm::sr && f.post == PcgForm::mg_restricted) f.split = choose_split(p);
     return f;
 }
 void pcg_matvec(pgo_problem* p, const PcgForm& f, int k, double tol2) {
@@ -175,6 +191,7 @@
         ++p->st_pcg_iterations;
     } else if (f.rec == PcgForm::sr_coarse) launch_cg_update_restrict_sr(p->G, p->C, p->coarse.K, k, first, k > 0 ? 1 : 0, n_pq, p->st);
     else if (f.rec == PcgForm::classic_coarse) launch_cg_update_restrict(p->G, p->C, p->coarse.K, k, n_pq, p->st);
+    else if (f.rec == PcgForm::sr && restricted && f.split.on()) launch_cg_update_mg_crit(p->G, p->C, m.M, m.levels, p->coarse.K, k, first, n_pq, p->st);
     else if (f.rec == PcgForm::sr && restricted) launch_cg_update_mg_sr(p->G, p->C, m.M, m.levels, p->coarse.K, k, first, n_pq, p->st);
     else if (f.rec == PcgForm::sr) launch_cg_update_sr(p->G, p->C, k, first, n_pq, p->st);
     else if (restricted) launch_cg_update_mg(p->G, p->C, m.M, m.levels, p->coarse.K, k, n_pq, p->st);
@@ -186,7 +203,16 @@
     const double* const r = f.single_red() || (k & 1) ? p->C.r : p->C.r2;
     if (f.fused_coarse()) launch_coarse_solve_dot(p->coarse.K, p->C.flags, part_rz + f.fused_parts, p->st);
     else if (f.mg() && f.rec == PcgForm::ranks) return mg_apply_ranks(p, true);
-    else if (f.mg()) launch_mg_apply(p->G, p->C, p->mg.M, p->mg.levels, p->coarse.K, r, p->C.z, part_rz, mg_scale(p), true, p->st, f.post == PcgForm::mg_restricted, mg_cs(p), mg_fine_view(p));
+    else if (f.mg()) {
+        const bool split = f.rec == PcgForm::sr && f.post == PcgForm::mg_restricted && f.split.on();
+        int hosts = 0;
+        launch_mg_apply(p->G, p->C, p->mg.M, p->mg.levels, p->coarse.K, r, p->C.z, part_rz, mg_scale(p), true, p->st, f.post == PcgForm::mg_restricted, mg_cs(p), mg_fine_view(p), nullptr, nullptr,
+                        split ? &f.split : nullptr, k & 1, k == 0 ? 1 : 0, &hosts);
+        if (split) {
+            int tiles[2 * MG_MAX_LEVELS];
+            if (hosts != mg_rider_hosts(p->C, p->mg.M, p->mg.levels, tiles) || f.split.host_b >= hosts) { p->err = "split update: the cycle's launches differ from mg_rider_hosts' list"; return PGO_ERR_STATE; }
+        }
+    }
     else if (f.post == PcgForm::two_level) launch_coarse_apply(p->G, p->C, p->coarse.K, r, p->C.z, part_rz, true, p->st);
     return PGO_OK;
 }
diff --git a/solve_keyframe_pose_graph_amd/csrc/pgo_solver.hip b/solve_keyframe_pose_graph_amd/csrc/pgo_solver.hip
--- a/solve_keyframe_pose_graph_amd/csrc/pgo_solver.hip
+++ b/solve_keyframe_pose_graph_amd/csrc/pgo_solver.hip
@@ -1447,7 +1447,7 @@
                           PcgForm f = choose_form(p);
                           const bool sr = f.single_red();
                           if (which == 6) { pcg_matvec(p, f, kk, 0.0); if ((rc = pcg_update(p, f, kk)) != PGO_OK) return rc; }
-                          else f.post = PcgForm::mg_cycle;
+                          else { f.post = PcgForm::mg_cycle; f.split = UpdSplit{}; }
                           if ((rc = pcg_precond(p, f, kk)) != PGO_OK) return rc;
                           const double lanes_rel = (double)(p->mf_pair_lanes + p->mf_rel_side_lanes), lanes_sw = (double)p->mf_sw_lanes;
                           const double fine = lanes_rel * (128.0 + 12.0) + lanes_sw * (128.0 + 12.0 + 8.0) + N * ((sr ? 2.0 : 4.0) * 48.0 + 48.0 + 13.0) + N * ((sr ? 11.0 : 7.0) * 48.0 + 96.0);
@@ -1460,6 +1460,7 @@
                               cyc += (A.smoothed ? 4.0 : 2.0) * (double)A.nnzb * (144.0 + 4.0) + (double)A.n * ((A.smoothed ? 4.0 : 2.0) * 288.0  + 24.0 + (A.smoothed ? 18.0 : 10.0) * 48.0 + 16.0);
                           }
                           cyc += (double)p->coarse.K.nc * (double)p->coarse.K.nc * 4.0 + (double)p->coarse.K.nc * 16.0;
+                          if (f.split.on()) cyc += N * 48.0;
                           bytes = which == 6 ? fine + cyc : cyc;
                           break; }
                 case 8: {
```

After: 117.6 (median of 6 runs). +4.9%, better.
